# jfkirk/tensorrec

Hardware: AMD Instinct MI355X
Metric: user-item predictions/sec (higher is better)
Workload: dtype i8/bf16/fp32; 1 GPU; synthetic 1000000 users x 1000000 items, identity features, d=128, LinearRepresentation + DotProduct, biased, fused top-10 (BASELINE.json configs[2]); users=1000000, items=1000000, n_components=128, top_k=10, parallelism=items sharded x1, users replicated, topk_method=two_stage

## Files before the change

### include/tensorrec_hip.h

```cpp
#ifndef TENSORREC_HIP_H
#define TENSORREC_HIP_H
#include <stdint.h>

#ifdef __cplusplus
extern "C" {
#endif

#define TREC_OK 0
#define TREC_ERR_INVALID 1
#define TREC_ERR_LAUNCH 2
#define TREC_ERR_UNSUPPORTED 3

#define TREC_DTYPE_F32 0
#define TREC_DTYPE_BF16 1
#define TREC_MODE_DOT 0
#define TREC_MODE_EUCLIDEAN 1

int trec_abi_version(void);
const char* trec_last_error(void);
int trec_device_cu_count(void);
int trec_set_tuning(const char* name, int32_t value);
int trec_get_tuning(const char* name, int dflt);
int trec_clear_tuning(const char* name);

// ... 15 lines not shown
                        const void* packed_entries, int64_t n_rows, int64_t nnz, const float* W, int32_t d,
                        const float* own, int32_t accumulate, float* out, float* out_rowsum, void* workspace,
                        int64_t workspace_bytes, void* stream);
int trec_spmv_csr_split(const int64_t* indptr, const int32_t* indices, const float* values, const int32_t* val_perm,
                        int64_t n_rows, int64_t nnz, const float* beta, float* out, void* workspace,
                        int64_t workspace_bytes, void* stream);
int trec_csr_to_dense(const int64_t* indptr, const int32_t* indices, const float* values, int64_t n_rows,
                      int32_t n_cols, float* out, void* stream);
int trec_row_l2norm_fwd(const float* x, int64_t n_rows, int32_t d, float* y, float* inv_norm, void* stream);
int trec_row_l2norm_bwd(const float* y, const float* inv_norm, const float* dy, int64_t n_rows, int32_t d, float* dx,
                        void* stream);
int trec_relu_bwd(const float* out, const float* dout, int64_t n, float* dpre, void* stream);
int trec_colsum(const float* x, int64_t n_rows, int32_t d, float* out, float* workspace, int32_t n_slices, void* stream);
int trec_gemm_f32(int32_t trans_a, int32_t trans_b, int64_t M, int64_t N, int64_t K, const float* A, int64_t lda,
                  const float* B, int64_t ldb, float* C, int64_t ldc, int32_t accumulate, float* workspace,
                  int32_t splits, void* stream);
int trec_gemm_f32_split_bf16(int32_t trans_a, int32_t trans_b, int64_t M, int64_t N, int64_t K, const float* A, int64_t lda,
                             const float* B, int64_t ldb, float* C, int64_t ldc, int32_t accumulate, float* workspace,
                             int32_t splits, float* a_colsum_parts, void* stream);

int trec_score_kpad(int32_t d);
int trec_score_rows_per_workgroup(int32_t dtype, int32_t kpad);
int trec_score_tile_rows(int32_t dtype, int32_t kpad);
int trec_score_topk_capacity(int32_t k);
int trec_score_prep(const float* repr, int64_t n, int32_t d, int32_t kpad, int32_t normalize, int32_t dtype, void* out,
                    float* out_sqnorm, void* stream);
int trec_score_gemm_store(const void* users, const void* items, int32_t dtype, int32_t kpad, int64_t n_users,
                          int64_t n_items, const float* user_bias, const float* item_bias, int32_t mode,
                          const float* user_sqnorm, const float* item_sqnorm, float* out, int64_t ld_out,
                          int32_t variant, void* stream);
int trec_score_topk_parts(int32_t dtype, int32_t kpad, int64_t n_items, int32_t n_chunks);
int trec_score_gemm_topk(const void* users, const void* items, int32_t dtype, int32_t kpad, int64_t n_users,
                         int64_t n_items, int32_t item_index_base, const float* user_bias, const float* item_bias,
                         int32_t mode, const float* user_sqnorm, const float* item_sqnorm, int32_t n_chunks,
                         int32_t capacity, float* part_vals, int32_t* part_idx, int32_t variant, void* stream);
int trec_score_gemm_blockmax(const void* users, const void* items, int32_t dtype, int32_t kpad, int64_t n_users,
                             int64_t n_items, const float* user_bias, const float* item_bias, int32_t mode,
                             const float* user_sqnorm, const float* item_sqnorm, int32_t sb_rows, int32_t n_chunks,
                             float* blockmax, int64_t bm_stride, int32_t variant, void* stream);
int trec_topk_select_blocks(const float* blockmax, int32_t n_sb, int64_t n_users, int64_t stride, int32_t k, int32_t* sel,
                            float* sel_max, float* tau, void* stream);
int trec_topk_group_keys(const int32_t* sel, const float* sel_max, const float* floor, int64_t n, int32_t k, int32_t n_sb,
                         int32_t* keys, void* stream);
int trec_topk_pad_counts(const int64_t* indptr_t, int32_t n_sb, int32_t rows_wg, int32_t* cnt_pad, void* stream);
int trec_exclusive_scan_i32(const int32_t* counts, int64_t n, int64_t* workspace_i64, int64_t* out, void* stream);
int trec_topk_fill_groups(const int64_t* pstart, const int64_t* indptr_t, const int32_t* users_t, const int32_t* perm_t,
                          int32_t n_sb, int32_t rows_wg, int64_t max_rows, const void* users_op, int32_t row_bytes,
                          const float* user_bias, const float* user_sq, const float* user_tau, void* G, float* g_bias,
                          float* g_sq, float* g_tau, int32_t* row_pair, int32_t* rblock_chunk, void* stream);
int trec_score_gemm_topk_grouped(const void* users_g, const void* items, int32_t dtype, int32_t kpad, int64_t n_rows_g,
                                 int64_t n_items, int32_t item_index_base, const float* user_bias_g,
                                 const float* item_bias, int32_t mode, const float* user_sqnorm_g,
                                 const float* item_sqnorm, int32_t sb_rows, const int32_t* rblock_chunk,
                                 const int32_t* row_pair, const float* row_floor, int32_t capacity, float* part_vals,
                                 int32_t* part_idx, int32_t variant, const int32_t* row_index, void* stream);
int trec_topk_fill_groups_index(const int64_t* pstart, const int64_t* indptr_t, const int32_t* users_t,
                                const int32_t* perm_t, int32_t n_sb, int32_t rows_wg, int64_t max_rows, int32_t* row_user,
                                int32_t* row_pair, int32_t* rblock_chunk, void* stream);

int trec_topk_select_blocks_ex(const float* blockmax, int32_t n_sb, int64_t n_users, int64_t stride, int32_t k,
                               int32_t k_tau, int32_t* sel, float* sel_max, float* tau, void* stream);

int trec_score_prep_filter(const float* repr, int64_t n, int32_t d, int32_t kpad, int32_t normalize, const float* bias,
                           float* out_f32, void* out_bf16, float* row_stats, float* gstats, void* stream);
int trec_score_prep_i8(const float* repr, int64_t n, int32_t d, int32_t kpad, int32_t side, float clip_sigmas,
                       int32_t sb_rows, const float* bias, float* scales, double* workspace, void* out_q,
                       float* row_stats, int32_t* bias_q, float* sb_stats, float* gstats, void* stream);
int trec_score_row_scale_i8(const float* repr, int64_t n, int32_t d, float* nat, float* gmax, void* stream);
int trec_score_prep_i8_users(const float* repr, int64_t n, int32_t d, int32_t kpad, const float* wg_scale, int32_t wg_rows,
                             void* out_q, float* row_stats, void* stream);
int trec_score_bias_i8_classes(const float* bias, int64_t n, int32_t sb_rows, const float* ladder, const int32_t* class_used,
                               int32_t n_classes, float* sb_stats, int32_t* bias_q, float* gstats, void* stream);
int32_t trec_score_blockmax_i8_rows_per_workgroup(int32_t top_k);
int trec_score_user_err_i8(const float* user_stats, const float* user_bias, const float* gstats, int32_t kdim,
                           int64_t n_users, const float* scales, const float* wg_scale, int32_t wg_rows, float* r_err,
                           void* stream);
int trec_score_gemm_blockmax_i8(const void* users_q, const void* items_q, int32_t kpad, int64_t n_users, int64_t n_items,
                                const float* user_bias, const int32_t* item_bias_q, const float* scales,
                                const float* sb_stats, int32_t sb_rows, int32_t n_chunks, float* blockmax,
                                int64_t bm_stride, const float* user_err, float* chunk_top, int32_t top_k,
                                const float* wg_scale, const int32_t* wg_class, int32_t wg_rows, void* stream);
int64_t trec_user_prep_alloc_rows(int64_t n, int32_t wg_rows);
int64_t trec_user_prep_workspace_bytes(int64_t n);
int trec_user_prep_sorted(const float* repr, int64_t n, int32_t d, int32_t kpad, int32_t normalize, const float* user_bias,
                          int32_t wg_rows, int64_t n_alloc, void* workspace, int64_t workspace_bytes, int32_t* src,
                          int32_t* pos, float* wg_scale, int32_t* wg_class, float* ladder, int32_t* class_used, float* gmax,
                          int32_t* meta, float* out_f32, void* out_bf16, float* row_stats, void* out_q, float* row_stats8,
                          float* bias_sorted, void* stream);
int trec_fill_zero(void* p, int64_t nbytes, void* stream);
int trec_topk_rows_collect(const float* table, int32_t n_sb, int64_t n_users, int64_t stride, const float* thr,
                           const float* user_err, const float* sb_stats, int32_t kdim, int32_t rcap, int32_t* row_count,
                           int32_t* row_user, int64_t* status, void* stream);
int trec_score_gemm_blockmax_grouped(const void* users_bf16, const void* items_bf16, int32_t kpad, int64_t n_rows_g,
                                     int64_t n_items, const float* user_bias, const float* item_bias, int32_t sb_rows,
                                     const int32_t* rblock_chunk, const int32_t* row_user, float* blockmax,
                                     int64_t bm_stride, int32_t wgs_per_row, void* stream);
int trec_topk_rows_hot(int32_t* row_count, int32_t n_sb, int32_t rcap, int64_t n_users, int32_t* hot_list, int32_t hot_cap,
                       int64_t max_pairs, int64_t* status, void* stream);
int trec_score_gemm_blockmax_hot(const void* users_bf16, const void* items_bf16, int32_t kpad, int64_t n_users,
                                 int64_t n_items, const float* user_bias, const float* item_bias, int32_t sb_rows,
                                 const int32_t* hot_list, int32_t hot_cap, float* blockmax, int64_t bm_stride, void* stream);
int trec_topk_dense_users(const float* table, int32_t n_sb, int64_t n_users, int64_t stride, const float* thr,
                          const float* user_err, const float* sb_stats, int32_t kdim, int32_t limit, float* cand_floor,
                          int32_t* flag, int32_t* n_flagged, void* stream);
int trec_score_gemm_refine_candidates(const void* users_bf16, const void* items_bf16, int32_t kpad, int64_t n_rows_g,
                                      int64_t n_items, const float* user_bias, const float* item_bias, int32_t sb_rows,
                                      const int32_t* row_count, const int32_t* row_user, float* blockmax, int64_t bm_stride,
                                      int32_t wgs_per_row, const float* cand_floor, int32_t* cand_n, void* cand,
                                      int32_t cand_cap, int32_t item_index_base, const int32_t* wg_map, int32_t n_wgs,
                                      void* stream);
int trec_topk_rows_wg_map(const int32_t* row_count, int32_t n_sb, int32_t wgs_per_row, int32_t* wg_start, int32_t* wg_map,
                          int64_t map_cap, void* stream);
int trec_score_gemm_refine_candidates_hot(const void* users_bf16, const void* items_bf16, int32_t kpad, int64_t n_users,
                                          int64_t n_items, const float* user_bias, const float* item_bias, int32_t sb_rows,
                                          const int32_t* hot_list, int32_t hot_cap, float* blockmax, int64_t bm_stride,
                                          const float* cand_floor, int32_t* cand_n, void* cand, int32_t cand_cap,
                                          int32_t item_index_base, void* stream);
int trec_topk_candidates_finish(const int32_t* cand_n, const void* cand, int32_t cand_cap, const float* cand_floor,
                                const float* user_stats, const float* item_gstats, const float* users_f32,
                                const float* items_f32, int64_t ld_users, int64_t ld_items, int32_t kdim,
                                const float* user_bias, const float* item_bias, int32_t item_index_base, int64_t n_users,
                                int32_t k, float* out_vals, int32_t* out_idx, int32_t* flag, int32_t* n_flagged,
                                const int32_t* out_index, int32_t lanes_per_user, void* stream);
int trec_topk_candidates_finish_mixed(const int32_t* cand_n, const void* cand, int32_t cand_cap, const float* cand_floor,
                                      const float* user_stats, const float* item_gstats, const float* users_f32,
                                      const float* items_f32, int64_t ld_users, int64_t ld_items, int32_t kdim,
                                      const float* user_bias, const float* item_bias, int32_t item_index_base, int64_t n_users,
                                      int32_t k, float* out_vals, int32_t* out_idx, int32_t* flag, int32_t* n_flagged,
                                      const int32_t* out_index, int32_t cands_per_lane, int32_t* over_list, int32_t* over_count,
                                      void* stream);
int trec_topk_candidates_finish_wide(const int32_t* cand_n, const void* cand, int32_t cand_cap, const float* cand_floor,
                                     const float* users_f32, const float* items_f32, int64_t ld_users, int64_t ld_items,
                                     int32_t kdim, const float* user_bias, const float* item_bias, int32_t item_index_base,
                                     int64_t n_users, int32_t k, float* out_vals, int32_t* out_idx, int32_t* flag, int32_t* n_flagged,
                                     const int32_t* out_index, void* stream);
int trec_topk_cascade_floor(float* tau, const int32_t* src, const float* user_stats, const float* user_bias,
                            const float* item_gstats, int32_t kdim, int64_t n_users, float* floor0, int32_t* flag,
                            int32_t* n_flagged, int32_t* cand_n, void* stream);

int32_t trec_topk_prerefine_max_superblocks(void);
int trec_topk_prerefine_rows_pos(const int32_t* sel, const float* sel_val, int32_t k, int32_t top_k, int32_t sb_per_chunk,
                                 int32_t n_sb, int64_t n_users, const int32_t* src, int32_t rcap, int32_t* sel_sb,
                                 int32_t* row_count, int32_t* row_user, int32_t* ok, int32_t* sel_pos, void* stream);
int trec_topk_prerefine_tau_listed(const int32_t* sel_sb, const int32_t* sel_pos, const int32_t* ok, int32_t k, const float* pre_max,
                                   int32_t rcap, int64_t n_users, const int32_t* src, const float* user_stats,
                                   const float* user_bias, const float* item_gstats, int32_t kdim, float* tau, float* vals,
                                   float* cand_floor, void* stream);
int trec_score_gemm_refine_candidates_marked(const void* users_bf16, const void* items_bf16, int32_t kpad, int64_t n_rows_g,
                                             int64_t n_items, const float* user_bias, const float* item_bias, int32_t sb_rows,
                                             const int32_t* row_count, const int32_t* row_user, float* blockmax, int64_t bm_stride,
                                             int32_t wgs_per_row, const float* cand_floor, int32_t* cand_n, void* cand,
                                             int32_t cand_cap, int32_t item_index_base, const int32_t* wg_map, int32_t n_wgs,
                                             float* pre_max, void* stream);
int trec_topk_euclid_certify(const int32_t* cand_idx, const float* cand_g, const float* exact, int32_t kc, int32_t k,
                             const float* user_sq, const float* user_bias, const float* item_gstats, const float* bias_max,
                             int32_t kdim, int64_t n_users, float* out_vals, int32_t* out_idx, int32_t* flag,
                             int32_t* n_flagged, const float* lambda_, const float* bias_min, void* stream);
int trec_topk_filter_floor(const float* tau, const float* user_stats, const float* user_bias, const float* item_gstats,
                           int32_t kdim, int64_t n_users, float* floor, int32_t* flag, int32_t* n_flagged, void* stream);
int trec_topk_collect_blocks(const float* blockmax, int32_t n_sb, int64_t n_users, int64_t stride, const float* floor,
                             int32_t ksel, int32_t* keys, int32_t* count, int32_t* flag, int32_t* n_flagged, void* stream);
int trec_topk_filter_floor_ex(const float* tau, const float* user_stats, const float* user_bias, const float* item_gstats,
                              int32_t kdim, int64_t n_users, float mult, float* floor, int32_t* flag, int32_t* n_flagged,
                              void* stream);
int trec_topk_scan_blocks(const float* blockmax, int32_t n_sb, int64_t n_users, int64_t stride, int32_t k, const float* floor0,
                          int32_t cand_cap, float* sel_max, float* tau, int32_t* cand_s, float* cand_v, int32_t* cand_n,
                          void* stream);
int trec_topk_prune_candidates(const int32_t* cand_s, const float* cand_v, const int32_t* cand_n, int32_t cand_cap,
                               const float* floor, int32_t ksel, int64_t n_users, int32_t* keys, int32_t* count, int32_t* flag,
                               int32_t* n_flagged, int32_t* redo, void* stream);
int trec_topk_collect_blocks_masked(const float* blockmax, int32_t n_sb, int64_t n_users, int64_t stride, const float* floor,
                                    int32_t ksel, int32_t* keys, int32_t* count, int32_t* flag, int32_t* n_flagged,
                                    const int32_t* redo, void* stream);
int trec_topk_filter_finish(const int32_t* part_idx, int32_t capacity, int32_t ksel, const int32_t* count,
                            const float* users_f32, const float* items_f32, int64_t ld_users, int64_t ld_items,
                            int32_t kdim, const float* user_bias, const float* item_bias, int32_t item_index_base,
                            int64_t n_users, int32_t k, float* out_vals, int32_t* out_idx, int32_t* flag,
                            int32_t* n_flagged, void* stream);
int trec_topk_filter_finish_wide(const int32_t* part_idx, int32_t capacity, int32_t ksel, const int32_t* count,
                                 const float* users_f32, const float* items_f32, int64_t ld_users, int64_t ld_items,
                                 int32_t kdim, const float* user_bias, const float* item_bias, int32_t item_index_base,
                                 int64_t n_users, int32_t k, float* out_vals, int32_t* out_idx, int32_t* flag,
                                 int32_t* n_flagged, void* stream);

int trec_topk_merge(const float* part_vals, const int32_t* part_idx, int64_t n_users, int32_t n_cand, int32_t k,
                    float* out_vals, int32_t* out_idx, void* stream);

int trec_pair_score_fwd(const float* U, const float* V, const int32_t* xu, const int32_t* xi, int64_t n_pairs,
                        int32_t pairs_per_user, int32_t d, int32_t mode, const float* user_bias,
                        const float* item_bias, float* out, float* out_sqdist, void* stream);
int trec_pair_score_bwd(const float* U, const float* V, const int32_t* xu, const int32_t* xi, const float* grad,
                        int64_t n_pairs, int32_t pairs_per_user, int32_t d, int32_t mode, float* dU, float* dV,
                        float* d_user_bias, float* d_item_bias, void* stream);

int trec_pair_euclid_coef(const float* U, const float* V, const int32_t* xu, const int32_t* xi, const float* grad,
                          const float* sqdist, int64_t n_pairs, int32_t pairs_per_user, int32_t d, float* coef,
                          void* stream);

int trec_group_pairs_by_item(const int32_t* xu, const int32_t* xi, int64_t n_pairs, int32_t pairs_per_user,
                             int64_t n_items, int32_t* workspace_i32, int64_t* workspace_i64, int64_t* indptr_t,
                             int32_t* users_t, int32_t* perm_t, int32_t counts_given, const int32_t* ranks,
                             const float* values_in, float* values_out, void* stream);
int32_t trec_group_pairs_lds_runs(int64_t n_pairs, int64_t n_items);
int trec_group_pairs_by_item_lds(const int32_t* xu, const int32_t* xi, int64_t n_pairs, int32_t pairs_per_user, int64_t n_items,
                                 int32_t* workspace_i32, int64_t* workspace_i64, int32_t* run_counts, int64_t* indptr_t,
                                 int32_t* users_t, int32_t* perm_t, void* stream);
int64_t trec_group_pairs_staged_bytes(int64_t n_pairs, int32_t window_log2);
int trec_group_pairs_by_item_staged(const int32_t* xu, const int32_t* xi, int64_t n_pairs, int32_t pairs_per_user, int64_t n_items,
                                    int32_t* workspace_i32, int64_t* workspace_i64, int64_t* indptr_t, int32_t* entries,
                                    const int32_t* ranks, const float* values_in, void* staging, int64_t staging_bytes,
                                    int32_t window_log2, void* stream);

int64_t trec_group_pairs_binned_bytes(int64_t n_pairs, int64_t n_items);
int trec_group_pairs_by_item_binned(const int32_t* xu, const int32_t* xi, const float* values, int64_t n_pairs, int32_t pairs_per_user,
                                    int64_t n_items, int32_t drop_zero_values, void* workspace, int64_t workspace_bytes,
                                    int64_t* indptr_t, int32_t* entries, void* stream);

int trec_rank_rows(const float* scores, int64_t n_users, int64_t n_items, int64_t ld_scores, int32_t* ranks,
                   int64_t ld_ranks, void* stream);
int64_t trec_rank_rows_workspace_bytes(int64_t n_users, int64_t n_items);
int trec_rank_rows_chunked(const float* scores, int64_t n_users, int64_t n_items, int64_t ld_scores, int32_t* ranks,
                           int64_t ld_ranks, void* workspace, int64_t workspace_bytes, void* stream);
int trec_score_rankcount_max_targets(void);
int trec_pair_score_exact(const float* users_f32, const float* items_f32, int64_t ld, int32_t kdim, const int32_t* xu,
                          const int32_t* xi, int64_t n_pairs, const float* user_bias, const float* item_bias,
                          int32_t mode, const float* user_sqnorm, const float* item_sqnorm, int32_t item_index_base,
                          float* out, void* stream);
int trec_score_gemm_rankcount(const float* users_f32, const float* items_f32, int32_t kpad, int64_t n_rows,
                              int64_t n_items, int32_t item_index_base, const float* user_bias, const float* item_bias,
                              int32_t mode, const float* user_sqnorm, const float* item_sqnorm, const int32_t* row_user,
                              const int32_t* row_t0, const int32_t* row_tn, const int32_t* tgt_item,
                              const float* tgt_score, int32_t n_chunks, int32_t* counts, void* stream);
int trec_rank_of_pairs(const float* scores, int64_t ld_scores, int64_t col_offset, int64_t begin, int64_t end,
                       const int32_t* xu, const int32_t* xi, const float* target_scores, int64_t n_pairs,
                       int32_t add_one, int32_t* out, void* stream);
int trec_rank_of_pairs_by_user(const float* scores, int64_t ld_scores, int64_t col_offset, int64_t begin, int64_t end,
                               const int64_t* pair_indptr, const int32_t* xi, const float* target_scores,
                               int64_t n_users, int64_t n_pairs, int32_t add_one, int32_t* out, void* stream);

int trec_wmrb_fwd(const int64_t* indptr, const int32_t* pos_slot, const float* pos_weight, const float* pred_serial,
                  const float* sample_pred, int64_t n_users, int64_t n_items, int32_t n_sampled, float* loss,
                  float* smr, void* stream);
int trec_wmrb_bwd(const int64_t* indptr, const int32_t* pos_slot, const float* pos_weight, const float* pred_serial,
                  const float* sample_pred, const float* smr, const float* grad_loss, int64_t n_users,
                  int64_t n_items, int32_t n_sampled, float* d_pred_serial, float* d_sample_pred, void* stream);
int trec_sampled_softmax_fwd(const int64_t* indptr, const int32_t* pos_slot, const float* pred_serial,
                             const float* sample_pred, int64_t n_users, int32_t n_sampled, float inv_temperature,
                             float* loss, float* row_max, float* row_sum, void* stream);
int trec_sampled_softmax_bwd(const int64_t* indptr, const int32_t* pos_slot, const float* pred_serial,
                             const float* sample_pred, const float* row_max, const float* row_sum,
                             const float* grad_loss, int64_t n_users, int32_t n_sampled, float inv_temperature,
                             float* d_pred_serial, float* d_sample_pred, void* stream);
int trec_bpr_fwd(const int64_t* indptr, const int32_t* pos_slot, const float* pred_serial, const float* sample_pred,
                 int64_t n_users, int32_t n_sampled, float* loss, void* stream);
int trec_bpr_bwd(const int64_t* indptr, const int32_t* pos_slot, const float* pred_serial, const float* sample_pred,
                 const float* grad_loss, int64_t n_users, int32_t n_sampled, float* d_pred_serial,
                 float* d_sample_pred, void* stream);
int trec_sampled_softmax_adj_fwd(const int64_t* indptr, const int32_t* x_item, const int32_t* pos_slot,
                                 const float* pred_serial, const float* sample_pred, const int32_t* samples, const float* log_q,
                                 float log_q_uniform, int64_t n_users, int64_t n_items, int32_t n_sampled, float inv_temperature,
                                 int32_t log_q_correction, int32_t remove_hits, float* loss, float* row_ref, float* row_max,
                                 float* row_sum, void* stream);
int trec_sampled_softmax_adj_bwd(const int64_t* indptr, const int32_t* x_item, const int32_t* pos_slot,
                                 const float* pred_serial, const float* sample_pred, const int32_t* samples, const float* log_q,
                                 float log_q_uniform, const float* row_ref, const float* row_max, const float* row_sum,
                                 const float* grad_loss, int64_t n_users, int64_t n_items, int32_t n_sampled,
                                 float inv_temperature, int32_t log_q_correction, int32_t remove_hits, float* d_pred_serial,
                                 float* d_sample_pred, void* stream);
int trec_bpr_adj_fwd(const int64_t* indptr, const int32_t* x_item, const int32_t* pos_slot, const float* pred_serial,
                     const float* sample_pred, const int32_t* samples, int64_t n_users, int32_t n_sampled, int32_t remove_hits,
                     float* loss, void* stream);
int trec_bpr_adj_bwd(const int64_t* indptr, const int32_t* x_item, const int32_t* pos_slot, const float* pred_serial,
                     const float* sample_pred, const int32_t* samples, const float* grad_loss, int64_t n_users, int32_t n_sampled,
                     int32_t remove_hits, float* d_pred_serial, float* d_sample_pred, void* stream);
int trec_warp_fwd(const int64_t* indptr, const int32_t* x_item, const int32_t* pos_slot, const float* pred_serial,
                  const float* sample_pred, const int32_t* samples, int64_t n_users, int64_t n_items, int32_t n_sampled,
                  int32_t remove_hits, float* loss, int32_t* first, float* weight, void* stream);
int trec_warp_bwd(const int64_t* indptr, const int32_t* pos_slot, const int32_t* first, const float* weight,
                  const float* grad_loss, int64_t n_users, int32_t n_sampled, float* d_pred_serial, float* d_sample_pred,
                  void* stream);
int trec_wmrb_fused_lds_bytes(int32_t n_sampled, int32_t max_interactions_per_user, int32_t d);
int trec_wmrb_fused_step(const float* U, const float* V, const float* user_bias, const float* item_bias,
                         const int64_t* indptr, const int32_t* x_item, const int32_t* pos_slot, const float* pos_weight,
                         const int32_t* samples, int64_t n_users, int64_t n_items, int32_t n_sampled, int32_t d,
                         int32_t max_interactions_per_user, float* loss, float* pred_serial, float* dU,
                         float* d_user_bias, float* coef_samples, float* coef_pairs, int32_t* sample_hist,
                         int32_t* sample_rank, void* stream);
int trec_softmax_fused_lds_bytes(int32_t n_sampled, int32_t max_interactions_per_user, int32_t d);
int trec_softmax_fused_step(const float* U, const float* V, const float* user_bias, const float* item_bias,
                            const int64_t* indptr, const int32_t* x_item, const int32_t* pos_slot, const int32_t* samples,
                            int64_t n_users, int64_t n_items, int32_t n_sampled, int32_t d,
                            int32_t max_interactions_per_user, float inv_temperature, const float* log_q, float log_uniform,
                            int32_t log_q_correction, int32_t remove_hits, float* loss, float* pred_serial, float* dU,
                            float* d_user_bias, float* coef_samples, float* coef_pairs, int32_t* sample_hist,
                            int32_t* sample_rank, void* stream);
int trec_warp_fused_lds_bytes(int32_t n_sampled, int32_t max_interactions_per_user, int32_t d);
int trec_warp_fused_step(const float* U, const float* V, const float* user_bias, const float* item_bias,
                         const int64_t* indptr, const int32_t* x_item, const int32_t* pos_slot, const int32_t* samples,
                         int64_t n_users, int64_t n_items, int32_t n_sampled, int32_t d, int32_t max_interactions_per_user,
                         int32_t remove_hits, float* loss, float* pred_serial, float* dU, float* d_user_bias,
                         float* coef_samples, float* coef_pairs, int32_t* first, int32_t* sample_hist, int32_t* sample_rank,
                         void* stream);
int trec_softmax_shared_supported(int32_t n_sampled, int32_t d);
int trec_softmax_shared_slices(int64_t n_users, int32_t n_sampled, int32_t d);
int trec_softmax_shared_stats(const float* U, const float* Vs, const float* user_bias, const float* sample_bias,
                              const float* sample_c, int64_t n_users, int32_t n_sampled, int32_t d, float inv_temperature,
// ... 116 lines not shown
```

### tensorrec_amd/_native.py

```python
from __future__ import annotations

import ctypes
import os

import torch

_HERE = os.path.dirname(os.path.abspath(__file__))
LIB_PATH = os.environ.get("TREC_HIP_LIB") or os.path.join(_HERE, "libtensorrec_hip.so")

_vp, _i32, _i64, _u32, _u64, _f = (ctypes.c_void_p, ctypes.c_int32, ctypes.c_int64, ctypes.c_uint32,
                                   ctypes.c_uint64, ctypes.c_float)

_RETURNS_I64 = ("trec_csr_split_workspace_bytes", "trec_rank_rows_workspace_bytes", "trec_user_prep_alloc_rows",
                "trec_user_prep_workspace_bytes", "trec_group_pairs_staged_bytes", "trec_group_pairs_binned_bytes",
                "trec_fit_step_coop_workspace_floats")

SIGNATURES = {
    "trec_abi_version": [],
    "trec_device_cu_count": [],
    "trec_set_tuning": [ctypes.c_char_p, _i32],
    "trec_get_tuning": [ctypes.c_char_p, ctypes.c_int],
    "trec_clear_tuning": [ctypes.c_char_p],
    "trec_spmm_csr": [_vp, _vp, _vp, _vp, _i64, _i64, _vp, _i32, _vp, _i32, _i32, _vp, _vp, _vp],
    "trec_spmm_one_per_row": [_vp, _vp, _i64, _vp, _i32, _vp, _vp],
    "trec_spmm_csr_filter": [_vp, _vp, _vp, _i64, _i64, _vp, _i32, _vp, _vp, _vp, _vp, _vp],
    "trec_absmax": [_vp, _i64, _vp, _vp],
    "trec_spmm_csr_packed": [_vp, _vp, _i64, _vp, _i32, _i32, _i32, _vp, _vp, _vp],
    "trec_spmv_csr": [_vp, _vp, _vp, _vp, _i64, _vp, _vp, _vp],
    "trec_csr_split_workspace_bytes": [_i64, _i32],
    "trec_spmm_csr_split": [_vp, _vp, _vp, _vp, _vp, _i64, _i64, _vp, _i32, _vp, _i32, _vp, _vp, _vp, _i64, _vp],
    "trec_spmv_csr_split": [_vp, _vp, _vp, _vp, _i64, _i64, _vp, _vp, _vp, _i64, _vp],
    "trec_pair_euclid_coef": [_vp, _vp, _vp, _vp, _vp, _vp, _i64, _i32, _i32, _vp, _vp],
    "trec_csr_to_dense": [_vp, _vp, _vp, _i64, _i32, _vp, _vp],
    "trec_row_l2norm_fwd": [_vp, _i64, _i32, _vp, _vp, _vp],
    "trec_row_l2norm_bwd": [_vp, _vp, _vp, _i64, _i32, _vp, _vp],
    "trec_relu_bwd": [_vp, _vp, _i64, _vp, _vp],
    "trec_colsum": [_vp, _i64, _i32, _vp, _vp, _i32, _vp],
    "trec_gemm_f32": [_i32, _i32, _i64, _i64, _i64, _vp, _i64, _vp, _i64, _vp, _i64, _i32, _vp, _i32, _vp],
    "trec_gemm_f32_split_bf16": [_i32, _i32, _i64, _i64, _i64, _vp, _i64, _vp, _i64, _vp, _i64, _i32, _vp, _i32, _vp, _vp],
    "trec_score_kpad": [_i32],
    "trec_score_rows_per_workgroup": [_i32, _i32],
    "trec_score_tile_rows": [_i32, _i32],
    "trec_score_topk_capacity": [_i32],
    "trec_score_prep": [_vp, _i64, _i32, _i32, _i32, _i32, _vp, _vp, _vp],
    "trec_score_gemm_store": [_vp, _vp, _i32, _i32, _i64, _i64, _vp, _vp, _i32, _vp, _vp, _vp, _i64, _i32, _vp],
    "trec_score_topk_parts": [_i32, _i32, _i64, _i32],
    "trec_score_gemm_topk": [_vp, _vp, _i32, _i32, _i64, _i64, _i32, _vp, _vp, _i32, _vp, _vp, _i32, _i32, _vp, _vp,
                             _i32, _vp],
    "trec_score_gemm_blockmax": [_vp, _vp, _i32, _i32, _i64, _i64, _vp, _vp, _i32, _vp, _vp, _i32, _i32, _vp, _i64, _i32,
                                 _vp],
    "trec_topk_select_blocks": [_vp, _i32, _i64, _i64, _i32, _vp, _vp, _vp, _vp],
    "trec_topk_select_blocks_ex": [_vp, _i32, _i64, _i64, _i32, _i32, _vp, _vp, _vp, _vp],
    "trec_score_prep_filter": [_vp, _i64, _i32, _i32, _i32, _vp, _vp, _vp, _vp, _vp, _vp],
    "trec_score_prep_i8": [_vp, _i64, _i32, _i32, _i32, _f, _i32, _vp, _vp, _vp, _vp, _vp, _vp, _vp, _vp, _vp],
    "trec_score_row_scale_i8": [_vp, _i64, _i32, _vp, _vp, _vp],
    "trec_score_prep_i8_users": [_vp, _i64, _i32, _i32, _vp, _i32, _vp, _vp, _vp],
    "trec_score_bias_i8_classes": [_vp, _i64, _i32, _vp, _vp, _i32, _vp, _vp, _vp, _vp],
    "trec_score_blockmax_i8_rows_per_workgroup": [_i32],
    "trec_score_user_err_i8": [_vp, _vp, _vp, _i32, _i64, _vp, _vp, _i32, _vp, _vp],
    "trec_score_gemm_blockmax_i8": [_vp, _vp, _i32, _i64, _i64, _vp, _vp, _vp, _vp, _i32, _i32, _vp, _i64, _vp, _vp, _i32,
                                    _vp, _vp, _i32, _vp],
    "trec_user_prep_alloc_rows": [_i64, _i32],
    "trec_user_prep_workspace_bytes": [_i64],
    "trec_user_prep_sorted": [_vp, _i64, _i32, _i32, _i32, _vp, _i32, _i64, _vp, _i64, _vp, _vp, _vp, _vp, _vp, _vp, _vp, _vp,
                              _vp, _vp, _vp, _vp, _vp, _vp, _vp],
    "trec_fill_zero": [_vp, _i64, _vp],
    "trec_topk_cascade_floor": [_vp, _vp, _vp, _vp, _vp, _i32, _i64, _vp, _vp, _vp, _vp, _vp],
    "trec_topk_prerefine_max_superblocks": [],
    "trec_topk_prerefine_rows_pos": [_vp, _vp, _i32, _i32, _i32, _i32, _i64, _vp, _i32, _vp, _vp, _vp, _vp, _vp, _vp],
    "trec_topk_prerefine_tau_listed": [_vp, _vp, _vp, _i32, _vp, _i32, _i64, _vp, _vp, _vp, _vp, _i32, _vp, _vp, _vp, _vp],
    "trec_score_gemm_refine_candidates_marked": [_vp, _vp, _i32, _i64, _i64, _vp, _vp, _i32, _vp, _vp, _vp, _i64, _i32, _vp, _vp, _vp,
                                                 _i32, _i32, _vp, _i32, _vp, _vp],
    "trec_topk_rows_collect": [_vp, _i32, _i64, _i64, _vp, _vp, _vp, _i32, _i32, _vp, _vp, _vp, _vp],
    "trec_score_gemm_blockmax_grouped": [_vp, _vp, _i32, _i64, _i64, _vp, _vp, _i32, _vp, _vp, _vp, _i64, _i32, _vp],
    "trec_topk_rows_hot": [_vp, _i32, _i32, _i64, _vp, _i32, _i64, _vp, _vp],
    "trec_score_gemm_blockmax_hot": [_vp, _vp, _i32, _i64, _i64, _vp, _vp, _i32, _vp, _i32, _vp, _i64, _vp],
    "trec_topk_dense_users": [_vp, _i32, _i64, _i64, _vp, _vp, _vp, _i32, _i32, _vp, _vp, _vp, _vp],
    "trec_score_gemm_refine_candidates": [_vp, _vp, _i32, _i64, _i64, _vp, _vp, _i32, _vp, _vp, _vp, _i64, _i32, _vp, _vp, _vp,
                                          _i32, _i32, _vp, _i32, _vp],
    "trec_topk_rows_wg_map": [_vp, _i32, _i32, _vp, _vp, _i64, _vp],
    "trec_score_gemm_refine_candidates_hot": [_vp, _vp, _i32, _i64, _i64, _vp, _vp, _i32, _vp, _i32, _vp, _i64, _vp, _vp, _vp,
                                              _i32, _i32, _vp],
    "trec_topk_candidates_finish": [_vp, _vp, _i32, _vp, _vp, _vp, _vp, _vp, _i64, _i64, _i32, _vp, _vp, _i32, _i64, _i32, _vp,
                                    _vp, _vp, _vp, _vp, _i32, _vp],
    "trec_topk_candidates_finish_mixed": [_vp, _vp, _i32, _vp, _vp, _vp, _vp, _vp, _i64, _i64, _i32, _vp, _vp, _i32, _i64, _i32,
                                          _vp, _vp, _vp, _vp, _vp, _i32, _vp, _vp, _vp],
    "trec_topk_candidates_finish_wide": [_vp, _vp, _i32, _vp, _vp, _vp, _i64, _i64, _i32, _vp, _vp, _i32, _i64, _i32, _vp, _vp, _vp, _vp,
                                         _vp, _vp],
    "trec_topk_euclid_certify": [_vp, _vp, _vp, _i32, _i32, _vp, _vp, _vp, _vp, _i32, _i64, _vp, _vp, _vp, _vp, _vp, _vp, _vp],
    "trec_topk_filter_floor": [_vp, _vp, _vp, _vp, _i32, _i64, _vp, _vp, _vp, _vp],
    "trec_topk_collect_blocks": [_vp, _i32, _i64, _i64, _vp, _i32, _vp, _vp, _vp, _vp, _vp],
    "trec_topk_filter_floor_ex": [_vp, _vp, _vp, _vp, _i32, _i64, _f, _vp, _vp, _vp, _vp],
    "trec_topk_scan_blocks": [_vp, _i32, _i64, _i64, _i32, _vp, _i32, _vp, _vp, _vp, _vp, _vp, _vp],
    "trec_topk_prune_candidates": [_vp, _vp, _vp, _i32, _vp, _i32, _i64, _vp, _vp, _vp, _vp, _vp, _vp],
    "trec_topk_collect_blocks_masked": [_vp, _i32, _i64, _i64, _vp, _i32, _vp, _vp, _vp, _vp, _vp, _vp],
    "trec_topk_filter_finish": [_vp, _i32, _i32, _vp, _vp, _vp, _i64, _i64, _i32, _vp, _vp, _i32, _i64, _i32, _vp, _vp,
                                _vp, _vp, _vp],
    "trec_topk_filter_finish_wide": [_vp, _i32, _i32, _vp, _vp, _vp, _i64, _i64, _i32, _vp, _vp, _i32, _i64, _i32, _vp, _vp,
                                     _vp, _vp, _vp],
    "trec_topk_group_keys": [_vp, _vp, _vp, _i64, _i32, _i32, _vp, _vp],
    "trec_topk_pad_counts": [_vp, _i32, _i32, _vp, _vp],
    "trec_exclusive_scan_i32": [_vp, _i64, _vp, _vp, _vp],
    "trec_topk_fill_groups": [_vp, _vp, _vp, _vp, _i32, _i32, _i64, _vp, _i32, _vp, _vp, _vp, _vp, _vp, _vp, _vp, _vp, _vp,
                              _vp],
    "trec_score_gemm_topk_grouped": [_vp, _vp, _i32, _i32, _i64, _i64, _i32, _vp, _vp, _i32, _vp, _vp, _i32, _vp, _vp,
                                     _vp, _i32, _vp, _vp, _i32, _vp, _vp],
    "trec_topk_fill_groups_index": [_vp, _vp, _vp, _vp, _i32, _i32, _i64, _vp, _vp, _vp, _vp],
    "trec_topk_merge": [_vp, _vp, _i64, _i32, _i32, _vp, _vp, _vp],
    "trec_pair_score_fwd": [_vp, _vp, _vp, _vp, _i64, _i32, _i32, _i32, _vp, _vp, _vp, _vp, _vp],
    "trec_pair_score_bwd": [_vp, _vp, _vp, _vp, _vp, _i64, _i32, _i32, _i32, _vp, _vp, _vp, _vp, _vp],
    "trec_group_pairs_by_item": [_vp, _vp, _i64, _i32, _i64, _vp, _vp, _vp, _vp, _vp, _i32, _vp, _vp, _vp, _vp],
    "trec_group_pairs_lds_runs": [_i64, _i64],
    "trec_group_pairs_by_item_lds": [_vp, _vp, _i64, _i32, _i64, _vp, _vp, _vp, _vp, _vp, _vp, _vp],
    "trec_group_pairs_staged_bytes": [_i64, _i32],
    "trec_group_pairs_binned_bytes": [_i64, _i64],
    "trec_group_pairs_by_item_binned": [_vp, _vp, _vp, _i64, _i32, _i64, _i32, _vp, _i64, _vp, _vp, _vp],
    "trec_group_pairs_by_item_staged": [_vp, _vp, _i64, _i32, _i64, _vp, _vp, _vp, _vp, _vp, _vp, _vp, _i64, _i32, _vp],
    "trec_rank_rows": [_vp, _i64, _i64, _i64, _vp, _i64, _vp],
    "trec_rank_rows_workspace_bytes": [_i64, _i64],
    "trec_rank_rows_chunked": [_vp, _i64, _i64, _i64, _vp, _i64, _vp, _i64, _vp],
    "trec_score_rankcount_max_targets": [],
    "trec_pair_score_exact": [_vp, _vp, _i64, _i32, _vp, _vp, _i64, _vp, _vp, _i32, _vp, _vp, _i32, _vp, _vp],
    "trec_score_gemm_rankcount": [_vp, _vp, _i32, _i64, _i64, _i32, _vp, _vp, _i32, _vp, _vp, _vp, _vp, _vp, _vp, _vp,
                                  _i32, _vp, _vp],
    "trec_rank_of_pairs": [_vp, _i64, _i64, _i64, _i64, _vp, _vp, _vp, _i64, _i32, _vp, _vp],
    "trec_rank_of_pairs_by_user": [_vp, _i64, _i64, _i64, _i64, _vp, _vp, _vp, _i64, _i64, _i32, _vp, _vp],
    "trec_wmrb_fwd": [_vp, _vp, _vp, _vp, _vp, _i64, _i64, _i32, _vp, _vp, _vp],
    "trec_wmrb_bwd": [_vp, _vp, _vp, _vp, _vp, _vp, _vp, _i64, _i64, _i32, _vp, _vp, _vp],
    "trec_sampled_softmax_fwd": [_vp, _vp, _vp, _vp, _i64, _i32, _f, _vp, _vp, _vp, _vp],
    "trec_sampled_softmax_bwd": [_vp, _vp, _vp, _vp, _vp, _vp, _vp, _i64, _i32, _f, _vp, _vp, _vp],
    "trec_bpr_fwd": [_vp, _vp, _vp, _vp, _i64, _i32, _vp, _vp],
    "trec_bpr_bwd": [_vp, _vp, _vp, _vp, _vp, _i64, _i32, _vp, _vp, _vp],
    "trec_sampled_softmax_adj_fwd": [_vp, _vp, _vp, _vp, _vp, _vp, _vp, _f, _i64, _i64, _i32, _f, _i32, _i32, _vp, _vp, _vp, _vp, _vp],
    "trec_sampled_softmax_adj_bwd": [_vp, _vp, _vp, _vp, _vp, _vp, _vp, _f, _vp, _vp, _vp, _vp, _i64, _i64, _i32, _f, _i32, _i32,
                                     _vp, _vp, _vp],
    "trec_bpr_adj_fwd": [_vp, _vp, _vp, _vp, _vp, _vp, _i64, _i32, _i32, _vp, _vp],
    "trec_bpr_adj_bwd": [_vp, _vp, _vp, _vp, _vp, _vp, _vp, _i64, _i32, _i32, _vp, _vp, _vp],
    "trec_warp_fwd": [_vp, _vp, _vp, _vp, _vp, _vp, _i64, _i64, _i32, _i32, _vp, _vp, _vp, _vp],
    "trec_warp_bwd": [_vp, _vp, _vp, _vp, _vp, _i64, _i32, _vp, _vp, _vp],
    "trec_wmrb_fused_lds_bytes": [_i32, _i32, _i32],
    "trec_wmrb_fused_step": [_vp, _vp, _vp, _vp, _vp, _vp, _vp, _vp, _vp, _i64, _i64, _i32, _i32, _i32, _vp, _vp, _vp, _vp,
                             _vp, _vp, _vp, _vp, _vp],
    "trec_warp_fused_lds_bytes": [_i32, _i32, _i32],
    "trec_warp_fused_step": [_vp, _vp, _vp, _vp, _vp, _vp, _vp, _vp, _i64, _i64, _i32, _i32, _i32, _i32, _vp, _vp, _vp, _vp, _vp, _vp,
                             _vp, _vp, _vp, _vp],
    "trec_softmax_fused_lds_bytes": [_i32, _i32, _i32],
    "trec_softmax_fused_step": [_vp, _vp, _vp, _vp, _vp, _vp, _vp, _vp, _i64, _i64, _i32, _i32, _i32, _f, _vp, _f, _i32, _i32,
                                _vp, _vp, _vp, _vp, _vp, _vp, _vp, _vp, _vp],
    "trec_softmax_shared_supported": [_i32, _i32],
    "trec_softmax_shared_slices": [_i64, _i32, _i32],
    "trec_softmax_shared_stats": [_vp, _vp, _vp, _vp, _vp, _i64, _i32, _i32, _f, _vp, _vp, _vp],
    "trec_softmax_shared_positives": [_vp, _vp, _vp, _vp, _vp, _i64, _f, _vp, _vp, _vp, _vp, _vp],
    "trec_softmax_shared_grads": [_vp, _vp, _vp, _vp, _vp, _vp, _vp, _i64, _i32, _i32, _f, _i32, _vp, _vp, _vp, _vp, _vp],
    "trec_softmax_shared_scatter": [_vp, _vp, _vp, _vp, _i32, _i32, _i64, _vp, _vp, _vp],
    "trec_softmax_full_positives": [_vp, _vp, _vp, _vp, _vp, _i64, _f, _vp, _vp, _vp, _vp, _vp],
    "trec_wmrb_tiled_lds_bytes": [_i32, _i32, _i32],
    "trec_wmrb_tiled_step": [_vp, _vp, _vp, _vp, _vp, _vp, _vp, _vp, _vp, _i64, _i64, _i32, _i32, _i32, _i32, _vp, _vp, _vp,
                             _vp, _vp, _vp, _vp, _vp, _vp, _i64, _vp, _vp],
    "trec_softmax_tiled_lds_bytes": [_i32, _i32, _i32],
    "trec_softmax_tiled_step": [_vp, _vp, _vp, _vp, _vp, _vp, _vp, _vp, _i64, _i64, _i32, _i32, _i32, _i32, _f, _vp, _f, _i32, _i32,
                                _vp, _vp, _vp, _vp, _vp, _vp, _vp, _vp, _vp, _i64, _vp, _vp],
    "trec_fit_step_coop_workspace_floats": [_i64, _i64, _i32, _i32, _i32],
    "trec_fit_step_coop": [_vp] * 12 + [_vp] * 6 + [_vp] * 5 + [_i64, _i64, _i64, _i32, _i32, _i32, _i64, _u64, _u32, _f, _f, _f, _f, _f,
                                                            _vp, _i64, _vp, _vp, _vp],
    "trec_item_weighted_hist": [_vp, _vp, _i64, _vp, _vp, _i64, _i32, _vp, _vp],
    "trec_dense_loss_fwd": [_i32, _vp, _i64, _i64, _vp, _vp, _vp, _i64, _vp, _vp, _vp],
    "trec_dense_loss_fwd_phase": [_i32, _i32, _vp, _i64, _i64, _vp, _vp, _vp, _i64, _i64, _vp, _vp, _vp],
    "trec_dense_loss_bwd": [_i32, _vp, _i64, _i64, _vp, _vp, _vp, _i64, _vp, _vp, _vp, _vp],
    "trec_softmax_dense_fwd": [_vp, _i64, _vp, _vp, _vp, _i64, _i64, _f, _vp, _vp, _vp, _vp],
    "trec_softmax_dense_bwd": [_vp, _i64, _vp, _vp, _vp, _vp, _vp, _vp, _i64, _i64, _f, _vp, _vp],
    "trec_gram_f64": [_vp, _i64, _i32, _i64, _vp, _vp],
    "trec_dense_loss_factored_phase": [_i32, _i32, _vp, _vp, _vp, _i64, _i64, _i64, _vp, _vp, _vp],
    "trec_dense_loss_factored_bwd": [_i32, _vp, _vp, _i64, _vp, _vp, _vp, _vp, _vp],
    "trec_rmse_fwd": [_vp, _vp, _i64, _vp, _i32, _vp, _vp],
    "trec_rmse_bwd": [_vp, _vp, _vp, _vp, _i64, _vp, _vp],
    "trec_sample_items": [_i64, _i64, _i32, _i32, _i32, _u64, _u32, _vp, _vp],
    "trec_sample_items_alias": [_i64, _i64, _i32, _i32, _vp, _vp, _u64, _u32, _vp, _vp],
    "trec_hard_negatives_supported": [_i32, _i32, _i32],
    "trec_select_hard_negatives": [_vp, _vp, _vp, _vp, _vp, _vp, _vp, _i64, _i64, _i32, _i32, _i32, _i32, _i32, _vp, _vp, _vp],
    "trec_crc32c": [_vp, _u64, _u32],
    "trec_collapse_tastes_fwd": [_vp, _vp, _i32, _i64, _i32, _vp, _vp, _vp, _vp, _i64, _vp, _vp],
    "trec_collapse_tastes_bwd": [_vp, _vp, _vp, _i32, _i64, _vp, _vp, _vp],
    "trec_adam_tf_step": [_vp, _vp, _vp, _vp, _i64, _f, _f, _f, _f, _f, _vp],
    "trec_adam_schedule_advance": [_vp, _f, _f, _f, _i32, _vp],
    "trec_adam_tf_step_dev": [_vp, _vp, _vp, _vp, _i64, _vp, _f, _f, _f, _f, _vp],
    "trec_sample_items_dev": [_i64, _i64, _i32, _i32, _i32, _u64, _vp, _vp, _vp],
    "trec_exclude_filter_topk": [_vp, _vp, _i32, _i64, _i32, _vp, _vp, _vp, _vp, _vp, _vp, _vp, _vp],
    "trec_topk_rows_excluded": [_vp, _i64, _i64, _i64, _i32, _vp, _vp, _vp, _vp, _vp, _vp],
    "trec_exclude_rank_adjust": [_vp, _vp, _vp, _vp, _vp, _vp, _i64, _vp, _vp],
    "trec_topk_drop_self": [_vp, _vp, _i32, _i64, _vp, _vp, _vp, _vp],
    "trec_candset_scores": [_vp, _vp, _i64, _i32, _vp, _vp, _vp, _i64, _i64, _i64, _vp, _vp, _i32, _vp, _vp, _vp, _vp],
    "trec_candset_topk": [_vp, _vp, _vp, _vp, _i64, _i32, _vp, _i64, _vp, _vp, _vp],
    "trec_candset_rank_count": [_vp, _vp, _vp, _vp, _vp, _vp, _i64, _vp, _vp],
}

_lib = None


class NativeLibraryError(RuntimeError):
    pass


def load():
    global _lib
    if _lib is not None:
        return _lib
    if not os.path.exists(LIB_PATH):
        raise NativeLibraryError(
            "%s not found: build it with `python -c 'import __graft_entry__ as g; g.build()'` or "
            "`make -C tensorrec_amd/csrc`.  tensorrec_amd has no CPU fallback." % LIB_PATH)
    try:
        lib = ctypes.CDLL(LIB_PATH)
    except OSError as exc:
        raise NativeLibraryError("cannot load %s: %s" % (LIB_PATH, exc))
    for name, argtypes in SIGNATURES.items():
        try:
            fn = getattr(lib, name)
        except AttributeError:
            raise NativeLibraryError("%s does not export %s (stale build?)" % (LIB_PATH, name))
        fn.argtypes = argtypes
        fn.restype = ctypes.c_int64 if name in _RETURNS_I64 else ctypes.c_int
    lib.trec_last_error.argtypes = []
    lib.trec_last_error.restype = ctypes.c_char_p
    _lib = lib
    return lib
# ... 44 lines not shown
```

### tensorrec_amd/csrc/score_blockmax.hip

```cpp
#include "score_common.hpp"
#include <math.h>
#include <type_traits>

namespace {

constexpr int BN = 64;

__device__ __forceinline__ int swz16(int row, int ch) {
    return ch >= 16 ? (row & 15) : ((row >> 1) & 7);
}

template <int KT, bool BIAS>
__global__ __launch_bounds__(256, 2) void blockmax_pipe_kernel(ScoreParams p)
{
    constexpr int NCB = 4;
    constexpr int NBUF = 2;
    constexpr int RB = KT * 2;
    constexpr int CH = RB / 16;
    constexpr int KS = KT / 16;
    constexpr int TILE_BYTES = BN * RB;
    constexpr int NSLOT = BN * CH / 256;
    constexpr int NSTEP = 2 * KS;
    static_assert(KT == 64 || KT == 128, "pipelined BLOCKMAX covers K = 64 / 128");

// ... 366 lines not shown
    float bm[NUB];
#pragma unroll
    for (int ub = 0; ub < NUB; ++ub) bm[ub] = -INFINITY;

    int tile_now = 0;
    int64_t sb_first = t_begin;
    auto queue_entry = [&](int i, int n) __attribute__((always_inline)) {
        const bool in = i < n;
        const int32_t code = in ? qc[i] : 0;
        const f32x4 a = in ? qv[i] : (f32x4){0.f, 0.f, 0.f, 0.f};
        const int ul = code >> 16;
        const int32_t uid = in ? q_id[ul] : -1;
        const float fl = q_fl[ul], bu = q_bu[ul];
        const int64_t item0 = sb_first + (int64_t)(code & 0xffff) * 4;
        float v[4];
        int32_t slot[4];
#pragma unroll
        for (int e = 0; e < 4; ++e) {
            v[e] = BIAS ? a[e] + bu : a[e];
            slot[e] = 0x7fffffff;
            if (uid >= 0 && v[e] >= fl && item0 + e < p.n_t) slot[e] = atomicAdd(p.cand_n + uid, 1);
        }
#pragma unroll
        for (int e = 0; e < 4; ++e) {
#ifdef TREC_CAND_DIAG
            if ((p.cand_diag & 3) == 2) continue;
#endif
            if (slot[e] < p.cand_cap)
                p.cand[(int64_t)uid * p.cand_cap + slot[e]] = make_int2((int32_t)(item0 + e) + p.t_index_base, __float_as_int(v[e]));
        }
    };
    auto queue_flush = [&](auto unrc) __attribute__((always_inline)) {
        constexpr int UNR = decltype(unrc)::value;
#ifdef TREC_CAND_DIAG
        const int n = (p.cand_diag & 3) == 1 ? 0 : qn;
#else
        const int n = qn;
#endif
#pragma unroll 1
        for (int i0 = 0; i0 < n; i0 += 64 * UNR) {
#pragma unroll
            for (int j = 0; j < UNR; ++j) queue_entry(i0 + j * 64 + lane, n);
        }
        qn = 0;
    };

    auto tile_body = [&](auto bufc) __attribute__((always_inline)) {
        constexpr int buf = decltype(bufc)::value;
        const char* tb = smem + buf * TILE_BYTES;
        const float* sd = side + buf * BN + 4 * g;
        bf16x8 tf[3];
        f32x4 c0 = {0.f, 0.f, 0.f, 0.f};
        if (BIAS) c0 = *(const f32x4*)sd;
        tf[0] = *(const bf16x8*)(tb + koff[0]);
        tf[1] = *(const bf16x8*)(tb + koff[1 % KS]);
        __builtin_amdgcn_sched_barrier(0);
#pragma unroll
        for (int s = 0; s < NSTEP; ++s) {
            const int blk = s / KS, ks = s % KS;
            if (s + 2 < NSTEP)
                tf[(s + 2) % 3] = *(const bf16x8*)(tb + ((s + 2) / KS) * 16 * RB + koff[(s + 2) % KS]);
            if (ks == 0) {
#pragma unroll
                for (int ub = 0; ub < NUB; ++ub)
                    acc[ub] = __builtin_amdgcn_mfma_f32_16x16x32_bf16(tf[s % 3], rfb[ub][0], c0, 0, 0, 0);
                if (BIAS && blk + 1 < NBLK) c0 = *(const f32x4*)(sd + 16 * (blk + 1));
            } else {
#pragma unroll
                for (int ub = 0; ub < NUB; ++ub)
                    acc[ub] = __builtin_amdgcn_mfma_f32_16x16x32_bf16(tf[s % 3], rfb[ub][ks], acc[ub], 0, 0, 0);
            }
            if (ks == KS - 1 && !LIST) {
#pragma unroll
                for (int ub = 0; ub < NUB; ++ub) {
                    bm[ub] = fmaxf(fmaxf(bm[ub], acc[ub][0]), acc[ub][1]);
                    bm[ub] = fmaxf(fmaxf(bm[ub], acc[ub][2]), acc[ub][3]);
                }
            }
            if (ks == KS - 1 && LIST) {
#pragma unroll
                for (int ub = 0; ub < NUB; ++ub) {
                    if ((ub % (NUB / 2)) == 0 && __builtin_expect(qn > LQ_FLUSH, 0)) queue_flush(std::integral_constant<int, 1>{});
                    const float m4 = fmaxf(fmaxf(fmaxf(acc[ub][0], acc[ub][1]), acc[ub][2]), acc[ub][3]);
                    bm[ub] = fmaxf(bm[ub], m4);
                    const bool hit = m4 >= thr_a[ub];
                    const unsigned long long hm = __builtin_amdgcn_ballot_w64(hit);
                    if (hm != 0ull) {
                        const int pos = qn + (int)__builtin_amdgcn_mbcnt_hi((unsigned int)(hm >> 32),
                                                                            __builtin_amdgcn_mbcnt_lo((unsigned int)hm, 0u));
                        if (hit) {
                            int lo = lane;
                            asm volatile("" : "+v"(lo));
                            qv[pos] = acc[ub];
                            qc[pos] = (((ub * 16) + (lo & 15)) << 16) | (((tile_now + blk) << 2) + (lo >> 4));
                        }
                        qn += __builtin_popcountll(hm);
                    }
                }
            }
            __builtin_amdgcn_sched_barrier(0);
        }
    };

    if (!GRP) stage_issue(0, 0);
    asm volatile("s_waitcnt vmcnt(0)" ::: "memory");
    __syncthreads();
#ifdef TREC_CAND_DIAG
    dg_t1 = wall_clock64();
#endif

    for (int t = 0; t < n_tiles; ++t) {
        const int buf = t & 1;
        if (t + 1 < n_tiles) stage_issue(t + 1, buf ^ 1);
        if (LIST) tile_now = (t % p.sb_tiles) * NBLK;
        if (buf == 0) tile_body(std::integral_constant<int, 0>{});
        else tile_body(std::integral_constant<int, 1>{});

        if (((t + 1) % p.sb_tiles) == 0 || t + 1 == n_tiles) {
#ifdef TREC_CAND_DIAG
            const unsigned long long dg_b = wall_clock64();
#endif
            if (LIST) { queue_flush(std::integral_constant<int, 3>{}); sb_first = t_begin + (int64_t)(t + 1) * BN; }
            const int64_t sb = GRP ? (int64_t)chunk : t_begin / ((int64_t)p.sb_tiles * BN) + t / p.sb_tiles;
            float m[NUB];
#pragma unroll
            for (int ub = 0; ub < NUB; ++ub) {
                float x = bm[ub];
                x = fmaxf(x, __shfl_xor(x, 16, 64));
                m[ub] = fmaxf(x, __shfl_xor(x, 32, 64));
                bm[ub] = -INFINITY;
            }
            if (LIST) {
                if (g == 0) {
#pragma unroll
                    for (int ub = 0; ub < NUB; ++ub) q_ta[ub * 16 + lu] = m[ub];
                }
                __builtin_amdgcn_fence(__ATOMIC_RELEASE, "wavefront");
                __builtin_amdgcn_wave_barrier();
                __builtin_amdgcn_fence(__ATOMIC_ACQUIRE, "wavefront");
#pragma unroll
                for (int o = 0; o < OW; ++o) {
                    const int slot = (OW * g + o) * 16 + lu;
                    float v = q_ta[slot];
                    const int32_t ou = q_id[slot];
                    if (BIAS) v = v + q_bu[slot];
#ifdef TREC_CAND_DIAG
                    if (p.cand_diag & 8) continue;
#endif
                    if (GRP && p.pre_max) {
                        if (ou >= 0) {
                            const int64_t rb = ((int64_t)__builtin_amdgcn_readfirstlane(rblock) * 4 + wave) * (NUB * 16);
                            p.pre_max[rb + slot] = v;
                            p.blockmax[sb * p.bm_stride + ou] = -INFINITY;
                        }
                    } else if (ou >= 0) p.blockmax[sb * p.bm_stride + ou] = v;
                }
                __builtin_amdgcn_fence(__ATOMIC_RELEASE, "wavefront");
                __builtin_amdgcn_wave_barrier();
            } else {
#pragma unroll
                for (int o = 0; o < OW; ++o) {
                    float v = g == 0 ? m[o] : (g == 1 ? m[OW + o] : (g == 2 ? m[2 * OW + o] : m[3 * OW + o]));
                    if (BIAS) v = v + own_bias[o];
                    if (own_u[o] >= 0) p.blockmax[sb * p.bm_stride + own_u[o]] = v;
                }
            }
#ifdef TREC_CAND_DIAG
            dg_flush += wall_clock64() - dg_b;
#endif
        }
        if (t + 1 < n_tiles) asm volatile("s_waitcnt vmcnt(0)" ::: "memory");
        __syncthreads();
    }
#ifdef TREC_CAND_DIAG
    if (GRP && LIST && tid == 0 && blockIdx.x < REFINE_DIAG_WGS) {
        const unsigned long long dg_e = wall_clock64();
        unsigned long long* row = g_refine_clk + (size_t)blockIdx.x * 4;
        row[0] = dg_t1 - dg_t0;
        row[1] = dg_e - dg_t1 - dg_flush;
        row[2] = dg_flush;
        row[3] = dg_e - dg_t0;
    }
#endif
}

template <int KT, bool BIAS, bool GRP, bool LIST = false>
int launch_bf16x16(ScoreParams p, hipStream_t st)
{
    constexpr int LDS = 2 * BN * KT * 2 + 2 * BN * 4 + (LIST ? 4 * LQ_CAP * 20 + 4 * 4 * NUB * 16 * 4 : 0);
    constexpr int RW = 4 * NUB * 16;
    auto kern = blockmax_bf16x16_kernel<KT, BIAS, GRP, LIST>;
    static bool attr_set = false;
    if (!attr_set && LDS > 32 * 1024) {
        (void)hipFuncSetAttribute((const void*)kern, hipFuncAttributeMaxDynamicSharedMemorySize, LDS);
        attr_set = true;
    }
    if (GRP && p.capacity > 0) p.capacity = p.capacity * 512 / RW;
    p.n_rblocks = GRP ? (int)(p.n_r / RW) : (int)ceil_div64(p.n_r, RW);
    const unsigned blocks = GRP ? (p.wg_map ? (unsigned)p.n_wgs : (unsigned)p.n_rblocks) : (unsigned)p.n_rblocks * (unsigned)p.n_chunks;
    if (blocks == 0) return TREC_OK;
    hipLaunchKernelGGL(kern, dim3(blocks), dim3(256), LDS, st, p);
    return trec_check_launch(GRP ? "trec_score_gemm_blockmax_grouped (16x16x32)" : "trec_score_gemm_blockmax (16x16x32)");
}

template <int KT, bool BIAS>
__global__ __launch_bounds__(256, 2) void blockmax_pipe_f32_kernel(ScoreParams p)
{
    constexpr int NCB = 2;
    constexpr int RB = KT * 4;
    constexpr int CH = RB / 16;
    constexpr int KS = KT / 2;
    constexpr int G = 8;
    constexpr int TILE_BYTES = BN * RB;
    constexpr int NSLOT = BN * CH / 256;
    static_assert(KT == 64 || KT == 128, "pipelined fp32 BLOCKMAX covers K = 64 / 128");

    extern __shared__ __attribute__((aligned(16))) char smem[];
    float* side = (float*)(smem + 2 * TILE_BYTES);

    const int tid = threadIdx.x;
    const int lane = tid & 63;
    const int wave = __builtin_amdgcn_readfirstlane(tid >> 6);
    const int half = lane >> 5, l31 = lane & 31;
    const int rblock = blockIdx.x % p.n_rblocks;
    const int chunk = blockIdx.x / p.n_rblocks;
    const int64_t r_base = ((int64_t)rblock * 4 + wave) * (NCB * 32);
    const int64_t t_begin = (int64_t)chunk * p.chunk_len;
    const int64_t t_end = (t_begin + p.chunk_len < p.n_t) ? t_begin + p.chunk_len : p.n_t;
    const int n_tiles = (int)((t_end - t_begin + BN - 1) / BN);

    float rff[NCB][KS];
    float r_bias[NCB];
#pragma unroll
    for (int cb = 0; cb < NCB; ++cb) {
        int64_t row = r_base + cb * 32 + l31;
        if (row >= p.n_r) row = p.n_r - 1;
        const float* src = (const float*)p.R + row * (int64_t)KT;
#pragma unroll
        for (int ks = 0; ks < KS; ++ks) rff[cb][ks] = src[2 * ks + half];
        r_bias[cb] = (BIAS && p.r_bias) ? p.r_bias[row] : 0.f;
    }

    int slot_off[NSLOT];
#pragma unroll
    for (int i = 0; i < NSLOT; ++i) {
        const int q = i * 256 + tid;
        const int row = q / CH, pc = q % CH;
        slot_off[i] = row * RB + ((pc ^ (row & 15)) * 16);
    }
    const char* t_chunk = (const char*)p.T + t_begin * (int64_t)RB;
    float side_b = 0.f;
    auto stage_issue = [&](int tile, int buf) {
        const int64_t row0 = t_begin + (int64_t)tile * BN;
        const bool clamp = row0 + BN > p.n_t;
        if (BIAS && tid < BN) {
            int64_t g = row0 + tid;
            if (g >= p.n_t) g = p.n_t - 1;
            side_b = p.t_bias ? p.t_bias[g] : 0.f;
        }
        const char* tile_base = t_chunk + (int64_t)tile * (BN * RB);
#pragma unroll
        for (int i = 0; i < NSLOT; ++i) {
            int off = slot_off[i];
            if (clamp) {
                const int last = (int)(p.n_t - 1 - row0);
                const int row = (i * 256 + tid) / CH;
                if (row > last) off -= (row - last) * RB;
            }
            char* dst = smem + buf * TILE_BYTES + (i * 256 + wave * 64) * 16;
            __builtin_amdgcn_global_load_lds((const __attribute__((address_space(1))) void*)(tile_base + off),
                                             (__attribute__((address_space(3))) void*)dst, 16, 0, 0);
        }
    };
    auto stage_commit = [&](int buf) {
        if (BIAS && tid < BN) side[buf * BN + tid] = side_b;
        asm volatile("s_waitcnt vmcnt(0)" ::: "memory");
    };

    const int sw = l31 & 15;
    const int row_off = l31 * RB + half * 4;
    auto tf_addr = [&](int ks) { return row_off + (((ks >> 1) ^ sw) * 16) + (ks & 1) * 8; };

    float bm[NCB];
#pragma unroll
    for (int cb = 0; cb < NCB; ++cb) bm[cb] = -INFINITY;

    stage_issue(0, 0);
    stage_commit(0);
    __syncthreads();

    for (int t = 0; t < n_tiles; ++t) {
        const int buf = t & 1;
        if (t + 1 < n_tiles) stage_issue(t + 1, buf ^ 1);
        const char* tb = smem + buf * TILE_BYTES;
        const float* sd = side + buf * BN + 4 * half;
#pragma unroll 1
        for (int rb = 0; rb < BN / 32; ++rb) {
            const char* blk = tb + rb * 32 * RB;
            f32x16 acc[NCB];
#pragma unroll
            for (int cb = 0; cb < NCB; ++cb)
#pragma unroll
                for (int r = 0; r < 16; ++r) acc[cb][r] = 0.f;
            float cur[G], nxt[G];
#pragma unroll
            for (int g = 0; g < G; ++g) cur[g] = *(const float*)(blk + tf_addr(g));
// ... 135 lines not shown
```

### tensorrec_amd/csrc/score_blockmax_i8.hip

```cpp
#include "score_common.hpp"
#include <math.h>
#include <limits.h>
#include <type_traits>

namespace {

typedef int v4i32 __attribute__((ext_vector_type(4)));

constexpr int BNQ = 128;
constexpr int NWQ = 4;

template <int KT, bool BIAS, int TK, int NUB>
__global__ __launch_bounds__(NWQ * 64, 8 / NWQ) void blockmax_i8x16_kernel(ScoreParams p)
{
    constexpr int NT = NWQ * 64;
    constexpr int OW = NUB / 4;
    static_assert(NUB % 4 == 0, "user blocks per wave must split over the four row-groups");
    constexpr int RB = KT;
    constexpr int CH = RB / 16;
    constexpr int KS = KT / 64;
    constexpr int TILE_BYTES = BNQ * RB;
    constexpr int NSLOT = BNQ * CH / NT;
    constexpr int NBLK = BNQ / 16;
    constexpr int NSTEP = NBLK * KS;
    static_assert(KT == 64 || KT == 128, "int8 16x16x64 BLOCKMAX covers K = 64 / 128");

    extern __shared__ __attribute__((aligned(16))) char smem[];
    int* side = (int*)(smem + 2 * TILE_BYTES);

    const int tid = threadIdx.x;
    const int lane = tid & 63;
    const int wave = __builtin_amdgcn_readfirstlane(tid >> 6);
    const int g = lane >> 4, lu = lane & 15;
    const int rblock = blockIdx.x % p.n_rblocks;
    const int chunk = blockIdx.x / p.n_rblocks;
    if (p.wg_scale && p.wg_scale[rblock] == 0.f) return;
    const int64_t r_base = ((int64_t)rblock * NWQ + wave) * (NUB * 16);
    const int64_t t_begin = (int64_t)chunk * p.chunk_len;
    const int64_t t_end = (t_begin + p.chunk_len < p.n_t) ? t_begin + p.chunk_len : p.n_t;
    const int n_tiles = (int)((t_end - t_begin + BNQ - 1) / BNQ);
    auto swz = [](int row) { return CH == 8 ? (row & 7) : ((row >> 1) & 3); };

    v4i32 rfq[NUB][KS];
#pragma unroll
    for (int ub = 0; ub < NUB; ++ub) {
        int64_t row = r_base + ub * 16 + lu;
        if (row >= p.n_r) row = p.n_r - 1;
        const char* src = (const char*)p.R + row * (int64_t)RB;
#pragma unroll
        for (int ks = 0; ks < KS; ++ks) rfq[ub][ks] = *(const v4i32*)(src + (ks * 4 + g) * 16);
    }
    int64_t own_u[OW];
    float own_bias[OW], e_nx[OW], e_ex[OW], e_cu[OW];
    float top[TK ? OW : 1][TK ? TK : 1];
#pragma unroll
    for (int o = 0; o < OW; ++o) {
        own_u[o] = r_base + (OW * g + o) * 16 + lu;
        const int64_t row = own_u[o] < p.n_r ? own_u[o] : p.n_r - 1;
        own_bias[o] = (BIAS && p.r_bias) ? p.r_bias[row] : 0.f;
        if (TK) {
            e_nx[o] = p.r_err[row * 4]; e_ex[o] = p.r_err[row * 4 + 1]; e_cu[o] = p.r_err[row * 4 + 2];
#pragma unroll
            for (int j = 0; j < TK; ++j) top[o][j] = -INFINITY;
        }
    }

    int slot_off[NSLOT];
#pragma unroll
    for (int i = 0; i < NSLOT; ++i) {
        const int q = i * NT + tid;
        const int row = q / CH, pc = q % CH;
        slot_off[i] = row * RB + ((pc ^ swz(row)) * 16);
    }
    const char* t_chunk = (const char*)p.T + t_begin * (int64_t)RB;
    const int* t_bias_q = p.t_bias ? (const int*)p.t_bias + (p.wg_class ? (int64_t)p.wg_class[rblock] * p.bias_stride : 0) : nullptr;
    auto stage_issue = [&](int tile, int buf) {
        const int64_t row0 = t_begin + (int64_t)tile * BNQ;
        const bool clamp = row0 + BNQ > p.n_t;
        if (BIAS && wave < BNQ / 64) {
            int64_t gi = row0 + wave * 64 + lane;
            if (gi >= p.n_t) gi = p.n_t - 1;
            if (t_bias_q) {
                __builtin_amdgcn_global_load_lds((const __attribute__((address_space(1))) void*)(t_bias_q + gi),
                                                 (__attribute__((address_space(3))) void*)(side + buf * BNQ + wave * 64), 4, 0, 0);
            } else {
                side[buf * BNQ + wave * 64 + lane] = 0;
            }
        }
        const char* tile_base = t_chunk + (int64_t)tile * (BNQ * RB);
#pragma unroll
        for (int i = 0; i < NSLOT; ++i) {
            int off = slot_off[i];
            if (clamp) {
                const int last = (int)(p.n_t - 1 - row0);
                const int row = (i * NT + tid) / CH;
                if (row > last) off -= (row - last) * RB;
            }
            char* dst = smem + buf * TILE_BYTES + (i * NT + wave * 64) * 16;
            __builtin_amdgcn_global_load_lds((const __attribute__((address_space(1))) void*)(tile_base + off),
                                             (__attribute__((address_space(3))) void*)dst, 16, 0, 0);
        }
    };

    int koff[KS];
#pragma unroll
    for (int ks = 0; ks < KS; ++ks) koff[ks] = lu * RB + (((ks * 4 + g) ^ swz(lu)) * 16);

    v4i32 acc[NUB];
    int bm[NUB];
#pragma unroll
    for (int ub = 0; ub < NUB; ++ub) bm[ub] = INT_MIN;

    auto tile_body = [&](auto bufc) __attribute__((always_inline)) {
        constexpr int buf = decltype(bufc)::value;
        const char* tb = smem + buf * TILE_BYTES;
        const int* sd = side + buf * BNQ + 4 * g;
        v4i32 tf[3];
        v4i32 c0 = {0, 0, 0, 0};
        if (BIAS) c0 = *(const v4i32*)sd;
        tf[0] = *(const v4i32*)(tb + koff[0]);
        tf[1] = *(const v4i32*)(tb + (KS > 1 ? koff[1 % KS] : 16 * RB + koff[0]));
        __builtin_amdgcn_sched_barrier(0);
#pragma unroll
        for (int s = 0; s < NSTEP; ++s) {
            const int blk = s / KS, ks = s % KS;
            if (ks == 0) {
#pragma unroll
                for (int ub = 0; ub < NUB; ++ub)
                    acc[ub] = __builtin_amdgcn_mfma_i32_16x16x64_i8(tf[s % 3], rfq[ub][0], c0, 0, 0, 0);
                __builtin_amdgcn_sched_barrier(0);
                if (BIAS && blk + 1 < NBLK) c0 = *(const v4i32*)(sd + 16 * (blk + 1));
            } else {
#pragma unroll
                for (int ub = 0; ub < NUB; ++ub)
                    acc[ub] = __builtin_amdgcn_mfma_i32_16x16x64_i8(tf[s % 3], rfq[ub][ks], acc[ub], 0, 0, 0);
                __builtin_amdgcn_sched_barrier(0);
            }
            if (s + 2 < NSTEP) tf[(s + 2) % 3] = *(const v4i32*)(tb + ((s + 2) / KS) * 16 * RB + koff[(s + 2) % KS]);
            if (ks == KS - 1) {
#pragma unroll
                for (int ub = 0; ub < NUB; ++ub) {
                    bm[ub] = max(max(bm[ub], acc[ub][0]), acc[ub][1]);
                    bm[ub] = max(max(bm[ub], acc[ub][2]), acc[ub][3]);
                }
            }
            __builtin_amdgcn_sched_barrier(0);
        }
    };

    stage_issue(0, 0);
    asm volatile("s_waitcnt vmcnt(0)" ::: "memory");
    __syncthreads();

    const float a_user = p.wg_scale ? p.wg_scale[rblock] : p.scales[0];
    const int64_t sb0 = t_begin / ((int64_t)p.sb_tiles * BNQ);
    f32x4 ss_cur = *(const f32x4*)(p.sb_stats + sb0 * 4), ss_next = ss_cur;
    for (int t = 0; t < n_tiles; ++t) {
        const int buf = t & 1;
        if (t + 1 < n_tiles) stage_issue(t + 1, buf ^ 1);
        if ((t % p.sb_tiles) == 0 && t + p.sb_tiles < n_tiles)
            ss_next = *(const f32x4*)(p.sb_stats + (sb0 + t / p.sb_tiles + 1) * 4);
        if (buf == 0) tile_body(std::integral_constant<int, 0>{});
        else tile_body(std::integral_constant<int, 1>{});

        if (((t + 1) % p.sb_tiles) == 0 || t + 1 == n_tiles) {
            const int64_t sb = sb0 + t / p.sb_tiles;
            const float scale = a_user * ss_cur[0];
            const float yh = TK ? ss_cur[1] : 0.f, dy = TK ? ss_cur[2] : 0.f, db = TK ? a_user * ss_cur[3] : 0.f;
            ss_cur = ss_next;
            int m[NUB];
#pragma unroll
            for (int ub = 0; ub < NUB; ++ub) {
                int x = bm[ub];
                const int o1 = __shfl_xor(x, 16, 64);
                x = x > o1 ? x : o1;
                const int o2 = __shfl_xor(x, 32, 64);
                m[ub] = x > o2 ? x : o2;
                bm[ub] = INT_MIN;
            }
#pragma unroll
            for (int o = 0; o < OW; ++o) {
                const int mo = g == 0 ? m[o] : (g == 1 ? m[OW + o] : (g == 2 ? m[2 * OW + o] : m[3 * OW + o]));
                float v = (float)mo * scale;
                if (BIAS) v = v + own_bias[o];
                if (own_u[o] < p.n_r) p.blockmax[sb * p.bm_stride + own_u[o]] = v;
                if (TK) {
                    float lb = v - i8_pair_err(e_nx[o], e_ex[o], e_cu[o], yh, dy, db, KT);
                    lb = (lb == lb) ? lb : -INFINITY;
                    if (p.top_tag) lb = lb_tag(lb, t / p.sb_tiles);
#pragma unroll
                    for (int j = TK - 1; j >= 1; --j) top[o][j] = __builtin_amdgcn_fmed3f(top[o][j], top[o][j - 1], lb);
                    top[o][0] = fmaxf(top[o][0], lb);
                }
            }
        }
        if (t + 1 < n_tiles) asm volatile("s_waitcnt vmcnt(0)" ::: "memory");
        __syncthreads();
    }
    if (TK) {
#pragma unroll
        for (int o = 0; o < OW; ++o)
            if (own_u[o] < p.n_r) {
#pragma unroll
                for (int j = 0; j < TK; ++j) p.chunk_top[((int64_t)chunk * TK + j) * p.bm_stride + own_u[o]] = top[o][j];
            }
    }
}

template <int KT, bool BIAS, int TK, int NUB>
int launch_i8x16(ScoreParams p, int sb_rows, hipStream_t st)
{
    constexpr int LDS = 2 * BNQ * KT + 2 * BNQ * 4;
    auto kern = blockmax_i8x16_kernel<KT, BIAS, TK, NUB>;
    static bool attr_set = false;
    if (!attr_set && LDS > 32 * 1024) {
        (void)hipFuncSetAttribute((const void*)kern, hipFuncAttributeMaxDynamicSharedMemorySize, LDS);
        attr_set = true;
    }
    p.n_rblocks = (int)ceil_div64(p.n_r, NWQ * NUB * 16);
    p.sb_tiles = sb_rows / BNQ;
    const unsigned blocks = (unsigned)p.n_rblocks * (unsigned)p.n_chunks;
    hipLaunchKernelGGL(kern, dim3(blocks), dim3(NWQ * 64), LDS, st, p);
    return trec_check_launch("trec_score_gemm_blockmax_i8 (16x16x64)");
}

template <int KT, bool BIAS>
int launch_i8x16_lists(const ScoreParams& p, int sb_rows, hipStream_t st)
{
    if (p.top_k == 0) return launch_i8x16<KT, BIAS, 0, 12>(p, sb_rows, st);
    if (p.top_k == 10) return launch_i8x16<KT, BIAS, 10, 12>(p, sb_rows, st);
    return launch_i8x16<KT, BIAS, 16, 8>(p, sb_rows, st);
}

template <int G>
__global__ __launch_bounds__(256) void prep_i8_kernel(const float* __restrict__ x, int64_t n, int d, int kt,
                                                     const float* __restrict__ scale_ptr, int sb_rows,
                                                     float* __restrict__ sb_stats, signed char* __restrict__ out_q,
                                                     float2* __restrict__ row_stats, int wg_rows)
{
    const int64_t row = ((int64_t)blockIdx.x * blockDim.x + threadIdx.x) / G;
    const bool ok = row < n;
    const int sub = threadIdx.x % G;
    const int64_t sb = sb_rows ? (ok ? row : n - 1) / sb_rows : 0;
    const float scale = sb_rows ? sb_stats[sb * 4] : (wg_rows > 0 ? scale_ptr[(ok ? row : n - 1) / wg_rows] : *scale_ptr);
    const float inv = 1.0f / scale;
    const float* xr = x + (ok ? row : 0) * (int64_t)d;
    float sw = 0.f, se = 0.f;
#pragma unroll
    for (int it = 0; it < 2; ++it) {
        const int c = (it * G + sub) * 4;
        f32x4 v = {0.f, 0.f, 0.f, 0.f};
        if (ok && c < d) {
            if ((d & 3) == 0) v = *(const f32x4*)(xr + c);
            else {
#pragma unroll
                for (int e = 0; e < 4; ++e) if (c + e < d) v[e] = xr[c + e];
            }
        }
        unsigned int pk = 0;
#pragma unroll
        for (int e = 0; e < 4; ++e) {
            float q = rintf(v[e] * inv);
            if (!(q == q)) q = 0.f;
            q = fminf(fmaxf(q, -127.f), 127.f);
            const float err = v[e] - q * scale;
            sw = fmaf(v[e], v[e], sw);
            se = fmaf(err, err, se);
            pk |= ((unsigned int)(int)q & 0xffu) << (8 * e);
        }
        if (ok && c < kt) *(unsigned int*)(out_q + row * (int64_t)kt + c) = pk;
    }
    for (int off = G / 2; off > 0; off >>= 1) { sw += __shfl_xor(sw, off, 64); se += __shfl_xor(se, off, 64); }
    float nw = sqrtf(sw), ne = sqrtf(se);
    if (sub == 0 && ok) row_stats[row] = make_float2(nw, ne);
}

__global__ __launch_bounds__(256) void sb_reduce_kernel(const float2* __restrict__ row_stats, int64_t n, int sb_rows,
                                                       float* __restrict__ sb_stats)
{
    const int64_t s = blockIdx.x;
    const int64_t r0 = s * sb_rows, r1 = (r0 + sb_rows < n) ? r0 + sb_rows : n;
    float g0 = 0.f, g1 = 0.f;
    for (int64_t r = r0 + threadIdx.x; r < r1; r += 256) {
        const float2 st = row_stats[r];
        float a = st.x + st.y, b = st.y;
        if (a != a) a = INFINITY;
        if (b != b) b = INFINITY;
        g0 = fmaxf(g0, a); g1 = fmaxf(g1, b);
    }
    for (int off = 32; off > 0; off >>= 1) { g0 = fmaxf(g0, __shfl_xor(g0, off, 64)); g1 = fmaxf(g1, __shfl_xor(g1, off, 64)); }
    __shared__ float w0[4], w1[4];
    if ((threadIdx.x & 63) == 0) { w0[threadIdx.x >> 6] = g0; w1[threadIdx.x >> 6] = g1; }
    __syncthreads();
    if (threadIdx.x == 0) {
        sb_stats[s * 4 + 1] = fmaxf(fmaxf(w0[0], w0[1]), fmaxf(w0[2], w0[3]));
        sb_stats[s * 4 + 2] = fmaxf(fmaxf(w1[0], w1[1]), fmaxf(w1[2], w1[3]));
    }
}

__global__ __launch_bounds__(1024) void sb_scale_kernel(const float* __restrict__ x, int64_t n, int d, int sb_rows,
                                                       float* __restrict__ sb_stats)
{
    const int64_t s = blockIdx.x;
    const int64_t r0 = s * sb_rows;
    const int64_t r1 = (r0 + sb_rows < n) ? r0 + sb_rows : n;
    const int64_t n_elem = (r1 - r0) * d;
    const float* xs = x + r0 * (int64_t)d;
    float am = 0.f;
    if ((d & 3) == 0) {
        for (int64_t i = (int64_t)threadIdx.x * 4; i < n_elem; i += 4096) {
            const f32x4 v = *(const f32x4*)(xs + i);
#pragma unroll
            for (int e = 0; e < 4; ++e) { const float a = fabsf(v[e]); am = (a > am || a != a) ? a : am; }
        }
    } else {
        for (int64_t i = threadIdx.x; i < n_elem; i += 1024) { const float a = fabsf(xs[i]); am = (a > am || a != a) ? a : am; }
    }
    if (am != am) am = INFINITY;
    for (int off = 32; off > 0; off >>= 1) am = fmaxf(am, __shfl_xor(am, off, 64));
    __shared__ float wmax[16];
    if ((threadIdx.x & 63) == 0) wmax[threadIdx.x >> 6] = am;
    __syncthreads();
    if (threadIdx.x == 0) {
        am = 0.f;
        for (int w = 0; w < 16; ++w) am = fmaxf(am, wmax[w]);
        float sc = am / 127.0f;
        if (!(sc > 0.f) || !(sc < INFINITY)) sc = 1.0f;
        sb_stats[s * 4] = sc;
    }
}

__global__ __launch_bounds__(256) void bias_i8_kernel(const float* __restrict__ bias, int64_t n, const float* __restrict__ ladder,
                                                     const int32_t* __restrict__ class_used, int sb_rows,
                                                     float* __restrict__ sb_stats, int* __restrict__ bias_q,
                                                     float* __restrict__ gstats)
{
    const int64_t s = blockIdx.x;
    const int c = blockIdx.y;
    if (class_used && class_used[c] == 0) return;
    const int64_t r0 = s * sb_rows, r1 = (r0 + sb_rows < n) ? r0 + sb_rows : n;
// ... 90 lines not shown
    if (u >= n_users) return;
    const float2 st = ustats[u];
    const float bu = user_bias ? fabsf(user_bias[u]) : 0.f;
    const float ck = (float)(kdim + 6) * 2.98023224e-07f;
    *(f32x4*)(r_err + u * 4) = (f32x4){st.x, st.y, ck * (bu + gstats[2]), wg_scale ? wg_scale[u / wg_rows] : scales[0]};
}

__global__ __launch_bounds__(256) void sumsq_absmax_kernel(const float* __restrict__ x, int64_t n_elem, double* __restrict__ ws)
{
    double acc = 0.0;
    float am = 0.f;
    for (int64_t i = ((int64_t)blockIdx.x * 256 + threadIdx.x) * 4; i + 3 < n_elem; i += (int64_t)gridDim.x * 1024) {
        const f32x4 v = *(const f32x4*)(x + i);
        acc += (double)v[0] * v[0] + (double)v[1] * v[1] + (double)v[2] * v[2] + (double)v[3] * v[3];
#pragma unroll
        for (int e = 0; e < 4; ++e) { const float a = fabsf(v[e]); am = (a > am || a != a) ? a : am; }
    }
    if (blockIdx.x == 0 && threadIdx.x == 0)
        for (int64_t i = n_elem & ~(int64_t)3; i < n_elem; ++i) {
            acc += (double)x[i] * x[i];
            const float a = fabsf(x[i]);
            am = (a > am || a != a) ? a : am;
        }
    if (am != am) am = INFINITY;
    for (int off = 32; off > 0; off >>= 1) { acc += __shfl_xor(acc, off, 64); am = fmaxf(am, __shfl_xor(am, off, 64)); }
    if ((threadIdx.x & 63) == 0) {
        atomicAdd(ws, acc);
        atomicMax((unsigned int*)(ws + 1), __float_as_uint(am));
    }
}

__global__ void scale_from_stats_kernel(const double* __restrict__ ws, double n_elem, float clip_sigmas, float* __restrict__ scales)
{
    const double rms = sqrt(ws[0] / n_elem);
    const float am = __uint_as_float(*(const unsigned int*)(ws + 1));
    float top = am;
    if (clip_sigmas > 0.f && (float)(clip_sigmas * rms) < top) top = (float)(clip_sigmas * rms);
    float s = top / 127.0f;
    if (!(s > 0.f) || !(s < INFINITY)) s = 1.0f;
    scales[0] = s;
}

}

extern "C" int trec_score_prep_i8(const float* repr, int64_t n, int32_t d, int32_t kpad, int32_t side, float clip_sigmas,
                                  int32_t sb_rows, const float* bias, float* scales, double* workspace, void* out_q,
                                  float* row_stats, int32_t* bias_q, float* sb_stats, float* gstats, void* stream)
{
    TREC_REQUIRE(scales && (side == 0 || side == 1 || side == 2), "trec_score_prep_i8: side must be 0 (users), 1 (items) or 2 (item biases)");
    TREC_REQUIRE(!bias || (bias_q && gstats && side >= 1), "trec_score_prep_i8: a bias needs bias_q, gstats and side 1 / 2");
    TREC_REQUIRE(side == 0 || (sb_stats && sb_rows >= 1), "trec_score_prep_i8: the item side needs sb_stats and sb_rows");
    if (n == 0) return TREC_OK;
    hipStream_t st = (hipStream_t)stream;
    if (side != 2) {
        TREC_REQUIRE(repr && out_q && row_stats, "trec_score_prep_i8: null pointer");
        TREC_REQUIRE(d >= 1 && kpad >= d && kpad % 4 == 0 && (kpad <= 64 || kpad == 128),
                     "trec_score_prep_i8: need d <= kpad, kpad % 4 == 0, kpad <= 64 or kpad == 128");
        TREC_REQUIRE(((uintptr_t)repr % 16) == 0, "trec_score_prep_i8: repr must be 16-byte aligned");
        if (side == 0) {
            TREC_REQUIRE(workspace, "trec_score_prep_i8: the user side needs the 16-byte workspace");
            if (hipMemsetAsync(workspace, 0, 2 * sizeof(double), st) != hipSuccess) {
                trec_set_last_error("trec_score_prep_i8: memset failed");
                return TREC_ERR_LAUNCH;
            }
            const int64_t n_elem = n * (int64_t)d;
            unsigned sb = (unsigned)ceil_div64(n_elem, 1024 * 8);
            if (sb > 4096) sb = 4096;
            if (sb < 1) sb = 1;
            hipLaunchKernelGGL(sumsq_absmax_kernel, dim3(sb), dim3(256), 0, st, repr, n_elem, workspace);
            hipLaunchKernelGGL(scale_from_stats_kernel, dim3(1), dim3(1), 0, st, workspace, (double)n_elem, clip_sigmas, scales);
        } else {
            hipLaunchKernelGGL(sb_scale_kernel, dim3((unsigned)ceil_div64(n, sb_rows)), dim3(1024), 0, st, repr, n, d, sb_rows, sb_stats);
        }
        const int g = kpad == 128 ? 32 : (kpad == 64 ? 16 : 8);
        const unsigned blocks = (unsigned)ceil_div64(n * g, 256);
#define TREC_PQ(GV) hipLaunchKernelGGL(prep_i8_kernel<GV>, dim3(blocks), dim3(256), 0, st, repr, n, d, kpad, scales, side == 1 ? sb_rows : 0, sb_stats, (signed char*)out_q, (float2*)row_stats, 0)
        if (g == 32) TREC_PQ(32);
        else if (g == 16) TREC_PQ(16);
        else TREC_PQ(8);
#undef TREC_PQ
        if (side == 1)
            hipLaunchKernelGGL(sb_reduce_kernel, dim3((unsigned)ceil_div64(n, sb_rows)), dim3(256), 0, st, (const float2*)row_stats, n, sb_rows, sb_stats);
    }
    if (side >= 1 && bias)
        hipLaunchKernelGGL(bias_i8_kernel, dim3((unsigned)ceil_div64(n, sb_rows), 1), dim3(256), 0, st, bias, n, scales, (const int32_t*)nullptr, sb_rows, sb_stats, bias_q, gstats);
    return trec_check_launch("trec_score_prep_i8");
}


extern "C" int trec_score_row_scale_i8(const float* repr, int64_t n, int32_t d, float* nat, float* gmax, void* stream)
{
    TREC_REQUIRE(repr && nat && gmax, "trec_score_row_scale_i8: null pointer");
    TREC_REQUIRE(d >= 1 && d <= 256 && ((uintptr_t)repr % 16) == 0, "trec_score_row_scale_i8: need d <= 256 and 16-byte aligned rows");
    if (n == 0) return TREC_OK;
    const int kp = (d + 3) / 4 * 4;
    const int g = kp > 64 ? 32 : (kp > 32 ? 16 : 8);
    const unsigned blocks = (unsigned)ceil_div64(n * g, 256);
    hipStream_t st = (hipStream_t)stream;
    if (g == 32) hipLaunchKernelGGL(row_natscale_kernel<32>, dim3(blocks), dim3(256), 0, st, repr, n, d, nat, gmax);
    else if (g == 16) hipLaunchKernelGGL(row_natscale_kernel<16>, dim3(blocks), dim3(256), 0, st, repr, n, d, nat, gmax);
    else hipLaunchKernelGGL(row_natscale_kernel<8>, dim3(blocks), dim3(256), 0, st, repr, n, d, nat, gmax);
    return trec_check_launch("trec_score_row_scale_i8");
}

extern "C" int trec_score_prep_i8_users(const float* repr, int64_t n, int32_t d, int32_t kpad, const float* wg_scale,
                                        int32_t wg_rows, void* out_q, float* row_stats, void* stream)
{
    TREC_REQUIRE(repr && wg_scale && out_q && row_stats && wg_rows >= 1, "trec_score_prep_i8_users: bad arguments");
    TREC_REQUIRE(d >= 1 && kpad >= d && kpad % 4 == 0 && (kpad <= 64 || kpad == 128),
                 "trec_score_prep_i8_users: need d <= kpad, kpad % 4 == 0, kpad <= 64 or kpad == 128");
    TREC_REQUIRE(((uintptr_t)repr % 16) == 0, "trec_score_prep_i8_users: repr must be 16-byte aligned");
    if (n == 0) return TREC_OK;
    hipStream_t st = (hipStream_t)stream;
    const int g = kpad == 128 ? 32 : (kpad == 64 ? 16 : 8);
    const unsigned blocks = (unsigned)ceil_div64(n * g, 256);
#define TREC_PQU(GV) hipLaunchKernelGGL(prep_i8_kernel<GV>, dim3(blocks), dim3(256), 0, st, repr, n, d, kpad, wg_scale, 0, (float*)nullptr, (signed char*)out_q, (float2*)row_stats, wg_rows)
    if (g == 32) TREC_PQU(32);
    else if (g == 16) TREC_PQU(16);
    else TREC_PQU(8);
#undef TREC_PQU
    return trec_check_launch("trec_score_prep_i8_users");
}

extern "C" int trec_score_bias_i8_classes(const float* bias, int64_t n, int32_t sb_rows, const float* ladder,
                                          const int32_t* class_used, int32_t n_classes, float* sb_stats, int32_t* bias_q,
                                          float* gstats, void* stream)
{
    TREC_REQUIRE(bias && ladder && sb_stats && bias_q && gstats, "trec_score_bias_i8_classes: null pointer");
    TREC_REQUIRE(sb_rows >= 1 && n_classes >= 1 && n_classes <= 65535, "trec_score_bias_i8_classes: bad sizes");
    if (n == 0) return TREC_OK;
    hipLaunchKernelGGL(bias_i8_kernel, dim3((unsigned)ceil_div64(n, sb_rows), (unsigned)n_classes), dim3(256), 0, (hipStream_t)stream,
                       bias, n, ladder, class_used, sb_rows, sb_stats, bias_q, gstats);
    return trec_check_launch("trec_score_bias_i8_classes");
}

extern "C" int32_t trec_score_blockmax_i8_rows_per_workgroup(int32_t top_k)
{
    return top_k <= 10 ? NWQ * 12 * 16 : NWQ * 8 * 16;
}

extern "C" int trec_score_user_err_i8(const float* user_stats, const float* user_bias, const float* gstats, int32_t kdim,
                                      int64_t n_users, const float* scales, const float* wg_scale, int32_t wg_rows,
                                      float* r_err, void* stream)
{
    TREC_REQUIRE(user_stats && gstats && r_err && kdim >= 1, "trec_score_user_err_i8: bad arguments");
    TREC_REQUIRE((wg_scale && wg_rows >= 1) || scales, "trec_score_user_err_i8: need wg_scale + wg_rows or scales");
    TREC_REQUIRE(((uintptr_t)r_err % 16) == 0, "trec_score_user_err_i8: r_err must be 16-byte aligned");
    if (n_users == 0) return TREC_OK;
    hipLaunchKernelGGL(user_err_i8_kernel, dim3((unsigned)ceil_div64(n_users, 256)), dim3(256), 0, (hipStream_t)stream,
                       (const float2*)user_stats, user_bias, gstats, kdim, n_users, scales, wg_scale, wg_rows, r_err);
    return trec_check_launch("trec_score_user_err_i8");
}

extern "C" int trec_score_gemm_blockmax_i8(const void* users_q, const void* items_q, int32_t kpad, int64_t n_users,
                                           int64_t n_items, const float* user_bias, const int32_t* item_bias_q,
                                           const float* scales, const float* sb_stats, int32_t sb_rows, int32_t n_chunks,
                                           float* blockmax, int64_t bm_stride, const float* user_err, float* chunk_top,
                                           int32_t top_k, const float* wg_scale, const int32_t* wg_class, int32_t wg_rows,
                                           void* stream)
{
    const int top_tag = (top_k & 0x100) ? 1 : 0;
    top_k &= 0xff;
    TREC_REQUIRE(!wg_scale || wg_rows == trec_score_blockmax_i8_rows_per_workgroup(top_k),
                 "trec_score_gemm_blockmax_i8: the user operand was laid out for another workgroup height (prepared for the other top_k?)");
    TREC_REQUIRE(users_q && items_q && (scales || wg_scale) && sb_stats && blockmax && bm_stride >= n_users, "trec_score_gemm_blockmax_i8: bad arguments");
    TREC_REQUIRE(!wg_class || wg_scale, "trec_score_gemm_blockmax_i8: wg_class comes with wg_scale");
    TREC_REQUIRE(kpad == 64 || kpad == 128, "trec_score_gemm_blockmax_i8: kpad must be 64 or 128");
    TREC_REQUIRE(sb_rows >= BNQ && sb_rows % BNQ == 0, "trec_score_gemm_blockmax_i8: sb_rows must be a multiple of 128");
    TREC_REQUIRE(n_users >= 1 && n_items >= 1 && n_chunks >= 1, "trec_score_gemm_blockmax_i8: empty operand");
    TREC_REQUIRE(n_items < (int64_t)1 << 31 && n_users < (int64_t)1 << 31, "trec_score_gemm_blockmax_i8: sizes must fit int32");
    TREC_REQUIRE((chunk_top != nullptr) == (user_err != nullptr) && (chunk_top ? (top_k == 10 || top_k == 16) : top_k == 0),
                 "trec_score_gemm_blockmax_i8: user_err, chunk_top and top_k (10 or 16) come together");
    ScoreParams p = {};
    p.R = users_q; p.T = items_q; p.n_r = n_users; p.n_t = n_items;
    p.chunk_len = ceil_div64(ceil_div64(n_items, n_chunks), sb_rows) * sb_rows;
    p.n_chunks = (int)ceil_div64(n_items, p.chunk_len);
    p.r_bias = user_bias; p.t_bias = (const float*)item_bias_q;
    p.blockmax = blockmax; p.bm_stride = bm_stride;
    p.scales = scales; p.sb_stats = sb_stats; p.r_err = user_err; p.chunk_top = chunk_top; p.top_k = top_k;
    p.top_tag = top_tag;
    TREC_REQUIRE(!top_tag || (top_k && p.chunk_len / sb_rows <= (1 << TREC_LB_TAG_BITS)),
                 "trec_score_gemm_blockmax_i8: tagged lower bounds need the lists and chunks of at most 4096 superblocks");
    p.wg_scale = wg_scale; p.wg_class = item_bias_q ? wg_class : nullptr; p.bias_stride = n_items;
    hipStream_t st = (hipStream_t)stream;
    const bool bias = user_bias || item_bias_q;
    if (kpad == 128) return bias ? launch_i8x16_lists<128, true>(p, sb_rows, st) : launch_i8x16_lists<128, false>(p, sb_rows, st);
    return bias ? launch_i8x16_lists<64, true>(p, sb_rows, st) : launch_i8x16_lists<64, false>(p, sb_rows, st);
}
```

### tensorrec_amd/csrc/score_common.hpp

```cpp
#pragma once
#include "common.hpp"

struct ScoreParams {
    const void* R;
    const void* T;
    int64_t n_r, n_t;
    int64_t chunk_len;
    int n_chunks;
    int n_rblocks;
    const float* r_bias;
    const float* t_bias;
    const float* r_sqnorm;
    const float* t_sqnorm;
    int euclid;
    float* out;
    int64_t ld_out;
    float* part_vals;
    int32_t* part_idx;
    int capacity;
    int n_parts;
    int32_t t_index_base;
    float* blockmax;
    int64_t bm_stride;
    int sb_tiles;
    const int32_t* rblock_chunk;
    const int32_t* row_pair;
    const float* row_floor;
    const int32_t* row_index;
    int independent_lists;
    const float* scales;
    const float* sb_stats;
    const float* r_err;
    const float* wg_scale;
    const int32_t* wg_class;
    int64_t bias_stride;
    int grp_band_major;
    const float* cand_floor;
    int32_t* cand_n;
    int2* cand;
    int32_t cand_cap;
    const int32_t* wg_map;
    int32_t n_wgs;
    float* pre_max;
    int cand_diag;
    float* chunk_top;
    int top_k;
    int top_tag;
};

#define TREC_LB_TAG_BITS 12
__device__ __forceinline__ int lb_key(float x)
{
    const int b = __float_as_int(x);
    return b >= 0 ? b : (int)(0x80000000u - (unsigned int)b);
}
__device__ __forceinline__ float lb_tag(float lb, int idx)
{
    if (!(fabsf(lb) < 1e37f)) return -INFINITY;
    const int k2 = ((lb_key(lb) >> TREC_LB_TAG_BITS) - 1) * (1 << TREC_LB_TAG_BITS) + idx;
    const int b2 = k2 >= 0 ? k2 : (int)(0x80000000u - (unsigned int)k2);
    return __int_as_float(b2);
}
__device__ __forceinline__ int lb_tag_index(float tagged) { return lb_key(tagged) & ((1 << TREC_LB_TAG_BITS) - 1); }

__device__ __forceinline__ float i8_pair_err(float nx, float ex, float cu, float yh, float dy, float db, int kdim)
{
    const float ck = (float)(kdim + 6) * 2.98023224e-07f;
    const float e = nx * (dy + ck * yh) + ex * yh + db + cu;
    return e * 1.001953125f + 1e-30f;
}

int launch_blockmax_pipelined(const ScoreParams& p, int kt, hipStream_t stream);
int launch_blockmax_filter16(const ScoreParams& p, int kt, hipStream_t stream);
int launch_blockmax_pipelined_grouped(const ScoreParams& p, int kt, hipStream_t stream);
int launch_blockmax_pipelined_f32(const ScoreParams& p, int kt, int sb_rows, hipStream_t stream);
```

### tensorrec_amd/csrc/topk_cascade.hip

```cpp
#include "score_common.hpp"
#include "topk_common.hpp"

namespace {

constexpr int CROWS = 8;
constexpr int CGROUPS = 4;
constexpr int CUSERS = 1024;
constexpr int GROUP_ROWS = 512;

struct UserConsts { float f[4], nx[4], ex[4], au[4]; unsigned int valid; };

__device__ __forceinline__ UserConsts load_user_consts(const float* __restrict__ thr, const float* __restrict__ user_err,
                                                       int64_t n_users, int64_t u)
{
    const float infl = 1.0029296875f;
    UserConsts c;
    c.valid = 0u;
    float thv[4];
    f32x4 uvv[4];
#pragma unroll
    for (int e = 0; e < 4; ++e) {
        const int64_t ue_i = u + e < n_users ? u + e : n_users - 1;
        thv[e] = thr[ue_i];
        uvv[e] = *(const f32x4*)(user_err + ue_i * 4);
// ... 23 lines not shown
{
    const float infl = 1.0029296875f;
    const float ck = (float)(kdim + 6) * 2.98023224e-07f;
    const bool vec = (stride % 4 == 0) && (((uintptr_t)table % 16) == 0) && (u + 3 < stride);
    unsigned int bits = 0;
    f32x4 v[CROWS], ss[CROWS];
#pragma unroll
    for (int r = 0; r < CROWS; ++r) {
        const int32_t s = s0 + r < n_sb ? s0 + r : n_sb - 1;
        const float* src = table + (int64_t)s * stride + u;
        if (vec) v[r] = __builtin_nontemporal_load((const f32x4*)src);
        else {
            v[r] = (f32x4){-INFINITY, -INFINITY, -INFINITY, -INFINITY};
#pragma unroll
            for (int e = 0; e < 4; ++e) if (u + e < n_users) v[r][e] = src[e];
        }
        ss[r] = *(const f32x4*)(sb_stats + (int64_t)s * 4);
    }
#pragma unroll
    for (int r = 0; r < CROWS; ++r) {
        const int32_t s = s0 + r;
        const float A = (ss[r][2] + ck * ss[r][1]) * infl, B = ss[r][1] * infl, C = ss[r][3] * infl;
#pragma unroll
        for (int e = 0; e < 4; ++e)
            if (s < n_sb && ((c.valid >> e) & 1u) && !(__fmaf_rn(c.nx[e], A, __fmaf_rn(c.ex[e], B, __fmaf_rn(c.au[e], C, v[r][e]))) < c.f[e]))
                bits |= 1u << (4 * r + e);
    }
    return bits;
}

__global__ __launch_bounds__(256) void rows_collect_kernel(const float* __restrict__ table, int32_t n_sb, int64_t n_users,
                                                          int64_t stride, const float* __restrict__ thr,
                                                          const float* __restrict__ user_err,
                                                          const float* __restrict__ sb_stats, int kdim, int32_t rcap,
                                                          int32_t* __restrict__ row_count, int32_t* __restrict__ row_user, int rows_fast)
{
    __shared__ int wsum[2][CROWS][4];
    __shared__ int base_s[2][CROWS];
    const unsigned ublk = rows_fast ? blockIdx.y : blockIdx.x, rgrp = rows_fast ? blockIdx.x : blockIdx.y;
    const int64_t u = (int64_t)ublk * CUSERS + threadIdx.x * 4;
    const int lane = threadIdx.x & 63, wave = threadIdx.x >> 6;
    const UserConsts c = load_user_consts(thr, user_err, n_users, u);
    for (int g = 0; g < CGROUPS; ++g) {
        const int32_t s0 = (rgrp * CGROUPS + g) * CROWS;
        if (s0 >= n_sb) break;
        const unsigned int bits = tile_bits(table, n_sb, n_users, stride, c, sb_stats, kdim, s0, u);
        int pre[CROWS];
#pragma unroll
        for (int r = 0; r < CROWS; ++r) {
            const int k = __builtin_popcount((bits >> (4 * r)) & 15u);
            int inc = k;
            for (int off = 1; off < 64; off <<= 1) {
                const int t = __shfl_up(inc, off, 64);
                if (lane >= off) inc += t;
            }
            pre[r] = inc - k;
            if (lane == 63) wsum[g & 1][r][wave] = inc;
        }
        __syncthreads();
        if (threadIdx.x < CROWS && s0 + threadIdx.x < n_sb) {
            const int total = wsum[g & 1][threadIdx.x][0] + wsum[g & 1][threadIdx.x][1] + wsum[g & 1][threadIdx.x][2] +
                              wsum[g & 1][threadIdx.x][3];
            base_s[g & 1][threadIdx.x] = total ? atomicAdd(&row_count[s0 + threadIdx.x], total) : 0;
        }
        __syncthreads();
#pragma unroll
        for (int r = 0; r < CROWS; ++r) {
            const int32_t s = s0 + r;
            if (s >= n_sb) break;
            const unsigned int m = (bits >> (4 * r)) & 15u;
            if (m) {
                int idx = base_s[g & 1][r] + pre[r];
                for (int w = 0; w < wave; ++w) idx += wsum[g & 1][r][w];
#pragma unroll
                for (int e = 0; e < 4; ++e)
                    if ((m >> e) & 1u) {
                        if (idx < rcap) row_user[(int64_t)s * rcap + idx] = (int32_t)(u + e);
                        ++idx;
                    }
            }
        }
    }
}

__global__ __launch_bounds__(256) void rows_collect_wave_kernel(const float* __restrict__ table, int32_t n_sb, int64_t n_users,
                                                               int64_t stride, const float* __restrict__ thr,
                                                               const float* __restrict__ user_err,
                                                               const float* __restrict__ sb_stats, int kdim, int32_t rcap,
                                                               int32_t* __restrict__ row_count, int32_t* __restrict__ row_user)
{
    const int64_t u = (int64_t)blockIdx.y * CUSERS + threadIdx.x * 4;
    const int lane = threadIdx.x & 63;
    const UserConsts c = load_user_consts(thr, user_err, n_users, u);
    for (int g = 0; g < CGROUPS; ++g) {
        const int32_t s0 = (blockIdx.x * CGROUPS + g) * CROWS;
        if (s0 >= n_sb) break;
        const unsigned int bits = tile_bits(table, n_sb, n_users, stride, c, sb_stats, kdim, s0, u);
        if (__builtin_amdgcn_ballot_w64(bits != 0u) == 0ull) continue;
        int pre[CROWS];
        int mine = 0;
#pragma unroll
        for (int r = 0; r < CROWS; ++r) {
            const int k = __builtin_popcount((bits >> (4 * r)) & 15u);
            int inc = k;
            for (int off = 1; off < 64; off <<= 1) {
                const int t = __shfl_up(inc, off, 64);
                if (lane >= off) inc += t;
            }
            pre[r] = inc - k;
            const int tot = __shfl(inc, 63, 64);
            if (lane == r) mine = tot;
        }
        int base = 0;
        if (lane < CROWS && mine > 0 && s0 + lane < n_sb) base = atomicAdd(&row_count[s0 + lane], mine);
#pragma unroll
        for (int r = 0; r < CROWS; ++r) {
            const int32_t s = s0 + r;
            const int b = __shfl(base, r, 64);
            if (s >= n_sb) break;
            const unsigned int m = (bits >> (4 * r)) & 15u;
            if (m) {
                int idx = b + pre[r];
#pragma unroll
                for (int e = 0; e < 4; ++e)
                    if ((m >> e) & 1u) {
                        if (idx < rcap) row_user[(int64_t)s * rcap + idx] = (int32_t)(u + e);
                        ++idx;
                    }
            }
        }
    }
}

__global__ __launch_bounds__(256) void dense_users_kernel(const float* __restrict__ table, int32_t n_sb, int64_t n_users,
                                                         int64_t stride, const float* __restrict__ thr,
                                                         const float* __restrict__ user_err,
                                                         const float* __restrict__ sb_stats, int kdim, int32_t limit,
                                                         float* __restrict__ cand_floor, int32_t* __restrict__ flag,
                                                         int32_t* __restrict__ n_flagged)
{
    const int64_t u = ((int64_t)blockIdx.x * 256 + threadIdx.x) * 4;
    if (u >= n_users) return;
    const UserConsts c = load_user_consts(thr, user_err, n_users, u);
    int cnt[4] = {0, 0, 0, 0};
    const int32_t groups = n_sb / CROWS;
    for (int j = 0; j < 4; ++j) {
        const int32_t s0 = (int32_t)(((int64_t)groups * j) / 4) * CROWS;
        const unsigned int bits = tile_bits(table, n_sb, n_users, stride, c, sb_stats, kdim, s0, u);
#pragma unroll
        for (int e = 0; e < 4; ++e) cnt[e] += __builtin_popcount(bits & (0x11111111u << e));
    }
#pragma unroll
    for (int e = 0; e < 4; ++e)
        if (u + e < n_users && cnt[e] >= limit && cand_floor[u + e] < INFINITY) {
            cand_floor[u + e] = INFINITY;
            if (flag[u + e] == 0) { flag[u + e] = 1; atomicAdd(n_flagged, 1); }
        }
}

__global__ __launch_bounds__(256) void rows_status_kernel(const int32_t* __restrict__ row_count, int32_t n_sb, int32_t rcap,
                                                         int64_t* __restrict__ status)
{
    __shared__ long long tot[4];
    __shared__ int over[4];
    long long t = 0;
    int o = 0;
    for (int s = threadIdx.x; s < n_sb; s += 256) {
        const int c = row_count[s];
        o |= c > rcap;
        t += ((c < rcap ? c : rcap) + GROUP_ROWS - 1) / GROUP_ROWS * GROUP_ROWS;
    }
    for (int off = 32; off > 0; off >>= 1) { t += __shfl_xor(t, off, 64); o |= __shfl_xor(o, off, 64); }
    if ((threadIdx.x & 63) == 0) { tot[threadIdx.x >> 6] = t; over[threadIdx.x >> 6] = o; }
    __syncthreads();
    if (threadIdx.x == 0) {
        status[0] = tot[0] + tot[1] + tot[2] + tot[3];
        status[1] = (over[0] | over[1] | over[2] | over[3]) ? 1 : 0;
    }
}

__global__ __launch_bounds__(256) void rows_hot_kernel(int32_t* __restrict__ row_count, int32_t n_sb, int32_t rcap,
                                                      int64_t n_users, int32_t* __restrict__ hot_list, int32_t hot_cap,
                                                      int64_t max_pairs, int64_t* __restrict__ status)
{
    __shared__ int wcnt[4];
    __shared__ int base_s;
    __shared__ long long tot[4], totp[4];
    if (threadIdx.x == 0) base_s = 0;
    long long t = 0, tp = 0;
    __syncthreads();
    for (int s0 = 0; s0 < n_sb; s0 += 256) {
        const int s = s0 + threadIdx.x;
        const int c = s < n_sb ? row_count[s] : 0;
        const bool hot = c > rcap;
        const unsigned long long m = __builtin_amdgcn_ballot_w64(hot);
        const int lane = threadIdx.x & 63, wave = threadIdx.x >> 6;
        if (lane == 0) wcnt[wave] = __builtin_popcountll(m);
        __syncthreads();
        int idx = base_s + __builtin_popcountll(m & ((1ull << lane) - 1ull));
        for (int w = 0; w < wave; ++w) idx += wcnt[w];
        if (hot) {
            if (idx < hot_cap) hot_list[idx] = s;
            row_count[s] = 0;
        } else {
            t += (c + GROUP_ROWS - 1) / GROUP_ROWS * GROUP_ROWS;
            tp += c;
        }
        __syncthreads();
        if (threadIdx.x == 0) base_s += wcnt[0] + wcnt[1] + wcnt[2] + wcnt[3];
        __syncthreads();
    }
    for (int off = 32; off > 0; off >>= 1) { t += __shfl_xor(t, off, 64); tp += __shfl_xor(tp, off, 64); }
    if ((threadIdx.x & 63) == 0) { tot[threadIdx.x >> 6] = t; totp[threadIdx.x >> 6] = tp; }
    __syncthreads();
    const int n_hot = base_s;
    for (int j = n_hot + threadIdx.x; j < hot_cap; j += 256) hot_list[j] = -1;
    if (threadIdx.x == 0) {
        const long long per_hot = (n_users + GROUP_ROWS - 1) / GROUP_ROWS * GROUP_ROWS;
        const long long nh = n_hot < hot_cap ? n_hot : hot_cap;
        status[0] = tot[0] + tot[1] + tot[2] + tot[3] + nh * per_hot;
        const long long pairs = totp[0] + totp[1] + totp[2] + totp[3] + (long long)n_hot * n_users;
        status[1] = (n_hot > hot_cap || pairs > max_pairs) ? 1 : 0;
        status[2] = n_hot;
    }
}

}

extern "C" int trec_topk_rows_collect(const float* table, int32_t n_sb, int64_t n_users, int64_t stride, const float* thr,
                                      const float* user_err, const float* sb_stats, int32_t kdim, int32_t rcap,
                                      int32_t* row_count, int32_t* row_user, int64_t* status, void* stream)
{
    TREC_REQUIRE(table && thr && user_err && sb_stats && row_count && row_user && status, "trec_topk_rows_collect: null pointer");
    TREC_REQUIRE(n_sb >= 1 && n_users >= 1 && stride >= n_users, "trec_topk_rows_collect: bad sizes");
    TREC_REQUIRE(rcap >= GROUP_ROWS && rcap % GROUP_ROWS == 0, "trec_topk_rows_collect: rcap must be a multiple of 512");
    hipStream_t st = (hipStream_t)stream;
    const int n_ublk = (int)ceil_div64(n_users, CUSERS);
    const unsigned n_rgrp = (unsigned)((n_sb + CROWS * CGROUPS - 1) / (CROWS * CGROUPS));
    const int rows_fast = trec_get_tuning("rows_collect_rows_fast", 1) != 0 && n_ublk <= 65535;
    if (rows_fast && trec_get_tuning("rows_collect_per_wave", 1) != 0)
        hipLaunchKernelGGL(rows_collect_wave_kernel, dim3(n_rgrp, (unsigned)n_ublk), dim3(256), 0, st, table, n_sb, n_users, stride, thr,
                           user_err, sb_stats, kdim, rcap, row_count, row_user);
    else
    hipLaunchKernelGGL(rows_collect_kernel, rows_fast ? dim3(n_rgrp, (unsigned)n_ublk) : dim3((unsigned)n_ublk, n_rgrp),
                       dim3(256), 0, st, table, n_sb, n_users, stride, thr, user_err, sb_stats, kdim, rcap, row_count, row_user, rows_fast);
    hipLaunchKernelGGL(rows_status_kernel, dim3(1), dim3(256), 0, st, row_count, n_sb, rcap, status);
    return trec_check_launch("trec_topk_rows_collect");
}

extern "C" int trec_topk_rows_hot(int32_t* row_count, int32_t n_sb, int32_t rcap, int64_t n_users, int32_t* hot_list,
                                  int32_t hot_cap, int64_t max_pairs, int64_t* status, void* stream)
{
    TREC_REQUIRE(row_count && hot_list && status, "trec_topk_rows_hot: null pointer");
    TREC_REQUIRE(n_sb >= 1 && rcap >= 1 && hot_cap >= 1 && n_users >= 1, "trec_topk_rows_hot: bad sizes");
    hipLaunchKernelGGL(rows_hot_kernel, dim3(1), dim3(256), 0, (hipStream_t)stream, row_count, n_sb, rcap, n_users, hot_list,
                       hot_cap, max_pairs, status);
    return trec_check_launch("trec_topk_rows_hot");
}

extern "C" int trec_score_gemm_blockmax_hot(const void* users_bf16, const void* items_bf16, int32_t kpad, int64_t n_users,
                                            int64_t n_items, const float* user_bias, const float* item_bias, int32_t sb_rows,
                                            const int32_t* hot_list, int32_t hot_cap, float* blockmax, int64_t bm_stride,
                                            void* stream)
{
    TREC_REQUIRE(users_bf16 && items_bf16 && hot_list && blockmax, "trec_score_gemm_blockmax_hot: null pointer");
    TREC_REQUIRE(kpad == 64 || kpad == 128, "trec_score_gemm_blockmax_hot: kpad must be 64 or 128");
    TREC_REQUIRE(sb_rows >= 64 && sb_rows % 64 == 0 && hot_cap >= 1 && bm_stride >= n_users, "trec_score_gemm_blockmax_hot: bad sizes");
    if (n_users == 0 || n_items == 0) return TREC_OK;
    ScoreParams p = {};
    p.R = users_bf16; p.T = items_bf16; p.n_r = n_users; p.n_t = n_items;
    p.chunk_len = sb_rows; p.n_chunks = hot_cap;
    p.r_bias = user_bias; p.t_bias = item_bias;
    p.blockmax = blockmax; p.bm_stride = bm_stride; p.sb_tiles = sb_rows / 64;
    p.rblock_chunk = hot_list;
    return launch_blockmax_filter16(p, kpad, (hipStream_t)stream);
}

extern "C" int trec_score_gemm_blockmax_grouped(const void* users_bf16, const void* items_bf16, int32_t kpad, int64_t n_rows_g,
                                                int64_t n_items, const float* user_bias, const float* item_bias,
                                                int32_t sb_rows, const int32_t* rblock_chunk, const int32_t* row_user,
                                                float* blockmax, int64_t bm_stride, int32_t wgs_per_row, void* stream)
{
    TREC_REQUIRE(wgs_per_row >= 0, "trec_score_gemm_blockmax_grouped: wgs_per_row < 0");
    TREC_REQUIRE(users_bf16 && items_bf16 && rblock_chunk && row_user && blockmax, "trec_score_gemm_blockmax_grouped: null pointer");
    TREC_REQUIRE(kpad == 64 || kpad == 128, "trec_score_gemm_blockmax_grouped: kpad must be 64 or 128");
    TREC_REQUIRE(n_rows_g % GROUP_ROWS == 0 && n_rows_g < ((int64_t)1 << 40), "trec_score_gemm_blockmax_grouped: n_rows_g % 512 != 0");
    TREC_REQUIRE(sb_rows >= 64 && sb_rows % 64 == 0, "trec_score_gemm_blockmax_grouped: sb_rows must be a multiple of 64");
    if (n_rows_g == 0) return TREC_OK;
    TREC_REQUIRE(n_rows_g / GROUP_ROWS < ((int64_t)1 << 31), "trec_score_gemm_blockmax_grouped: too many workgroups");
    ScoreParams p = {};
    p.R = users_bf16; p.T = items_bf16; p.n_r = n_rows_g; p.n_t = n_items;
    p.chunk_len = sb_rows; p.n_chunks = 1;
    p.r_bias = user_bias; p.t_bias = item_bias;
    p.blockmax = blockmax; p.bm_stride = bm_stride; p.sb_tiles = sb_rows / 64;
    p.rblock_chunk = rblock_chunk; p.row_index = row_user; p.capacity = wgs_per_row;
    p.grp_band_major = trec_get_tuning("cascade_band_major", 0);
    return launch_blockmax_pipelined_grouped(p, kpad, (hipStream_t)stream);
}

extern "C" int trec_score_gemm_refine_candidates(const void* users_bf16, const void* items_bf16, int32_t kpad, int64_t n_rows_g,
                                                 int64_t n_items, const float* user_bias, const float* item_bias,
                                                 int32_t sb_rows, const int32_t* row_count, const int32_t* row_user,
                                                 float* blockmax, int64_t bm_stride, int32_t wgs_per_row,
                                                 const float* cand_floor, int32_t* cand_n, void* cand, int32_t cand_cap,
                                                 int32_t item_index_base, const int32_t* wg_map, int32_t n_wgs, void* stream)
{
    TREC_REQUIRE(users_bf16 && items_bf16 && row_count && row_user && blockmax && cand_floor && cand_n && cand,
                 "trec_score_gemm_refine_candidates: null pointer");
    TREC_REQUIRE(n_wgs >= 0 && (wg_map || n_wgs == 0), "trec_score_gemm_refine_candidates: n_wgs without wg_map");
    if (wg_map && n_wgs == 0) return TREC_OK;
    TREC_REQUIRE(wgs_per_row > 0 && cand_cap >= 1, "trec_score_gemm_refine_candidates: needs the fixed-capacity layout (wgs_per_row > 0)");
    TREC_REQUIRE(kpad == 64 || kpad == 128, "trec_score_gemm_refine_candidates: kpad must be 64 or 128");
    TREC_REQUIRE(n_rows_g % GROUP_ROWS == 0 && n_rows_g < ((int64_t)1 << 40), "trec_score_gemm_refine_candidates: n_rows_g % 512 != 0");
    TREC_REQUIRE(sb_rows >= 64 && sb_rows % 64 == 0 && sb_rows <= 65536, "trec_score_gemm_refine_candidates: sb_rows must be a multiple of 64, <= 65536");
    if (n_rows_g == 0) return TREC_OK;
    TREC_REQUIRE(n_rows_g / GROUP_ROWS < ((int64_t)1 << 31), "trec_score_gemm_refine_candidates: too many workgroups");
    ScoreParams p = {};
    p.R = users_bf16; p.T = items_bf16; p.n_r = n_rows_g; p.n_t = n_items;
    p.chunk_len = sb_rows; p.n_chunks = 1;
    p.r_bias = user_bias; p.t_bias = item_bias;
    p.blockmax = blockmax; p.bm_stride = bm_stride; p.sb_tiles = sb_rows / 64;
    p.rblock_chunk = row_count; p.row_index = row_user; p.capacity = wgs_per_row;
    p.cand_floor = cand_floor; p.cand_n = cand_n; p.cand = (int2*)cand; p.cand_cap = cand_cap; p.t_index_base = item_index_base;
    p.cand_diag = trec_get_tuning("cascade_cand_diag", 0);
    p.wg_map = wg_map; p.n_wgs = n_wgs;
    return launch_blockmax_pipelined_grouped(p, kpad, (hipStream_t)stream);
}

extern "C" int trec_score_gemm_refine_candidates_marked(const void* users_bf16, const void* items_bf16, int32_t kpad, int64_t n_rows_g,
                                                        int64_t n_items, const float* user_bias, const float* item_bias,
                                                        int32_t sb_rows, const int32_t* row_count, const int32_t* row_user,
                                                        float* blockmax, int64_t bm_stride, int32_t wgs_per_row,
                                                        const float* cand_floor, int32_t* cand_n, void* cand, int32_t cand_cap,
                                                        int32_t item_index_base, const int32_t* wg_map, int32_t n_wgs, float* pre_max,
                                                        void* stream)
{
    TREC_REQUIRE(users_bf16 && items_bf16 && row_count && row_user && blockmax && cand_floor && cand_n && cand && pre_max,
                 "trec_score_gemm_refine_candidates_marked: null pointer");
    TREC_REQUIRE(n_wgs >= 0 && (wg_map || n_wgs == 0), "trec_score_gemm_refine_candidates_marked: n_wgs without wg_map");
    if (wg_map && n_wgs == 0) return TREC_OK;
    TREC_REQUIRE(wgs_per_row > 0 && cand_cap >= 1, "trec_score_gemm_refine_candidates_marked: needs the fixed-capacity layout (wgs_per_row > 0)");
    TREC_REQUIRE(kpad == 64 || kpad == 128, "trec_score_gemm_refine_candidates_marked: kpad must be 64 or 128");
    TREC_REQUIRE(n_rows_g % GROUP_ROWS == 0 && n_rows_g < ((int64_t)1 << 40), "trec_score_gemm_refine_candidates_marked: n_rows_g % 512 != 0");
    TREC_REQUIRE(sb_rows >= 64 && sb_rows % 64 == 0 && sb_rows <= 65536, "trec_score_gemm_refine_candidates_marked: sb_rows must be a multiple of 64, <= 65536");
    if (n_rows_g == 0) return TREC_OK;
    TREC_REQUIRE(n_rows_g / GROUP_ROWS < ((int64_t)1 << 31), "trec_score_gemm_refine_candidates_marked: too many workgroups");
    ScoreParams p = {};
    p.R = users_bf16; p.T = items_bf16; p.n_r = n_rows_g; p.n_t = n_items;
    p.chunk_len = sb_rows; p.n_chunks = 1;
    p.r_bias = user_bias; p.t_bias = item_bias;
    p.blockmax = blockmax; p.bm_stride = bm_stride; p.sb_tiles = sb_rows / 64;
    p.rblock_chunk = row_count; p.row_index = row_user; p.capacity = wgs_per_row;
    p.cand_floor = cand_floor; p.cand_n = cand_n; p.cand = (int2*)cand; p.cand_cap = cand_cap; p.t_index_base = item_index_base;
    p.cand_diag = trec_get_tuning("cascade_cand_diag", 0);
    p.wg_map = wg_map; p.n_wgs = n_wgs;
    p.pre_max = pre_max;
    return launch_blockmax_pipelined_grouped(p, kpad, (hipStream_t)stream);
}

extern "C" int trec_score_gemm_refine_candidates_hot(const void* users_bf16, const void* items_bf16, int32_t kpad, int64_t n_users,
                                                     int64_t n_items, const float* user_bias, const float* item_bias,
                                                     int32_t sb_rows, const int32_t* hot_list, int32_t hot_cap, float* blockmax,
                                                     int64_t bm_stride, const float* cand_floor, int32_t* cand_n, void* cand,
                                                     int32_t cand_cap, int32_t item_index_base, void* stream)
{
    TREC_REQUIRE(users_bf16 && items_bf16 && hot_list && blockmax && cand_floor && cand_n && cand,
                 "trec_score_gemm_refine_candidates_hot: null pointer");
    TREC_REQUIRE(kpad == 64 || kpad == 128, "trec_score_gemm_refine_candidates_hot: kpad must be 64 or 128");
    TREC_REQUIRE(sb_rows >= 64 && sb_rows % 64 == 0 && sb_rows <= 65536 && hot_cap >= 1 && bm_stride >= n_users && cand_cap >= 1,
                 "trec_score_gemm_refine_candidates_hot: bad sizes");
    if (n_users == 0 || n_items == 0) return TREC_OK;
    ScoreParams p = {};
    p.R = users_bf16; p.T = items_bf16; p.n_r = n_users; p.n_t = n_items;
    p.chunk_len = sb_rows; p.n_chunks = hot_cap;
    p.r_bias = user_bias; p.t_bias = item_bias;
    p.blockmax = blockmax; p.bm_stride = bm_stride; p.sb_tiles = sb_rows / 64;
    p.rblock_chunk = hot_list;
    p.cand_floor = cand_floor; p.cand_n = cand_n; p.cand = (int2*)cand; p.cand_cap = cand_cap; p.t_index_base = item_index_base;
    return launch_blockmax_filter16(p, kpad, (hipStream_t)stream);
}

extern "C" int trec_topk_dense_users(const float* table, int32_t n_sb, int64_t n_users, int64_t stride, const float* thr,
                                     const float* user_err, const float* sb_stats, int32_t kdim, int32_t limit,
                                     float* cand_floor, int32_t* flag, int32_t* n_flagged, void* stream)
{
    TREC_REQUIRE(table && thr && user_err && sb_stats && cand_floor && flag && n_flagged, "trec_topk_dense_users: null pointer");
    TREC_REQUIRE(n_sb >= 32 && stride >= n_users && limit >= 1 && limit <= 32, "trec_topk_dense_users: need n_sb >= 32, 1 <= limit <= 32");
    if (n_users == 0) return TREC_OK;
    hipLaunchKernelGGL(dense_users_kernel, dim3((unsigned)ceil_div64(n_users, 1024)), dim3(256), 0, (hipStream_t)stream, table, n_sb,
                       n_users, stride, thr, user_err, sb_stats, kdim, limit, cand_floor, flag, n_flagged);
    return trec_check_launch("trec_topk_dense_users");
}

namespace {
__global__ __launch_bounds__(256) void wg_start_kernel(const int32_t* __restrict__ row_count, int32_t n_sb, int32_t wgs_per_row,
                                                      int32_t* __restrict__ wg_start, int32_t group_rows)
{
    __shared__ int wsum[4];
    __shared__ int base_s;
    if (threadIdx.x == 0) base_s = 0;
    __syncthreads();
    const int lane = threadIdx.x & 63, wave = threadIdx.x >> 6;
    for (int s0 = 0; s0 < n_sb; s0 += 256) {
        const int s = s0 + threadIdx.x;
        int c = s < n_sb ? (row_count[s] + group_rows - 1) / group_rows : 0;
        if (c > wgs_per_row) c = wgs_per_row;
        int inc = c;
        for (int off = 1; off < 64; off <<= 1) {
            const int t = __shfl_up(inc, off, 64);
            if (lane >= off) inc += t;
        }
        if (lane == 63) wsum[wave] = inc;
        __syncthreads();
        int excl = base_s + inc - c;
        for (int w = 0; w < wave; ++w) excl += wsum[w];
        if (s < n_sb) wg_start[s] = excl;
        __syncthreads();
        if (threadIdx.x == 0) base_s += wsum[0] + wsum[1] + wsum[2] + wsum[3];
        __syncthreads();
    }
    if (threadIdx.x == 0) wg_start[n_sb] = base_s;
}

__global__ __launch_bounds__(256) void wg_map_kernel(const int32_t* __restrict__ wg_start, int32_t wgs_per_row, int64_t map_cap,
                                                    int32_t* __restrict__ wg_map)
{
    const int s = blockIdx.x;
    const int b = wg_start[s], e = wg_start[s + 1];
    for (int j = threadIdx.x; j < e - b; j += 256)
        if ((int64_t)b + j < map_cap) wg_map[b + j] = s * wgs_per_row + j;
}
}

extern "C" int trec_topk_rows_wg_map(const int32_t* row_count, int32_t n_sb, int32_t wgs_per_row, int32_t* wg_start,
                                     int32_t* wg_map, int64_t map_cap, void* stream)
{
    TREC_REQUIRE(row_count && wg_start && wg_map, "trec_topk_rows_wg_map: null pointer");
    TREC_REQUIRE(n_sb >= 1 && wgs_per_row >= 1 && map_cap >= 0 && (int64_t)n_sb * wgs_per_row < ((int64_t)1 << 31),
                 "trec_topk_rows_wg_map: bad sizes");
    hipStream_t st = (hipStream_t)stream;
    hipLaunchKernelGGL(wg_start_kernel, dim3(1), dim3(256), 0, st, row_count, n_sb, wgs_per_row, wg_start, GROUP_ROWS);
    hipLaunchKernelGGL(wg_map_kernel, dim3((unsigned)n_sb), dim3(256), 0, st, wg_start, wgs_per_row, map_cap, wg_map);
    return trec_check_launch("trec_topk_rows_wg_map");
}
```

### tensorrec_amd/ops_topk.py

```python
from .ops_base import (DTYPE_BF16, DTYPE_F32, MODE_DOT, MODE_EUCLIDEAN, N, _f32c, _timed, gemm_raw, group_pairs_by_item,
                       l2_normalize_rows, pair_scores_exact, rank_rows, torch)

def score_kpad(d):
    k = N.query("trec_score_kpad", int(d))
    if k < 0:
        raise ValueError("n_components = %d is beyond the MFMA score kernel's limit of 256" % d)
    return k


def score_prep(repr_, dtype=DTYPE_F32, normalize=False, want_sqnorm=False):
    x = _f32c(repr_.detach())
    n, d = x.shape
    kpad = score_kpad(d)
    if dtype == DTYPE_F32 and kpad == d and not normalize and not want_sqnorm:
        return x, None, kpad
    out = torch.empty((n, kpad), dtype=torch.float32 if dtype == DTYPE_F32 else torch.bfloat16, device=x.device)
    sq = torch.empty((n,), dtype=torch.float32, device=x.device) if want_sqnorm else None
    N.call("trec_score_prep", N.ptr(x), n, d, kpad, 1 if normalize else 0, dtype, N.ptr(out), N.ptr(sq))
    return out, sq, kpad


SCORE_KMAX = 256


# ... 303 lines not shown
def score_prep_filter(repr_, normalize=False, bias=None, want_gstats=False, sort_users=False, k=10, user_bias=None):
    x = _f32c(repr_.detach())
    n, d = x.shape
    kpad = score_kpad(d)
    if sort_users and kpad <= 128 and n > 0 and i8_user_classes_enabled():
        return _prep_users_sorted(x, normalize, k, user_bias)
    op = FilterOperand()
    op.n, op.d, op.kpad = n, d, kpad
    own_f32 = normalize or kpad != d
    op.f32 = torch.empty((n, kpad), dtype=torch.float32, device=x.device) if own_f32 else x
    op.bf16 = torch.empty((n, kpad), dtype=torch.bfloat16, device=x.device)
    op.stats = torch.empty((n, 2), dtype=torch.float32, device=x.device)
    op.gstats = zero_block(4, x.device)[:3].view(torch.float32) if want_gstats else None
    with _timed("score_prep_filter"):
        N.call("trec_score_prep_filter", N.ptr(x), n, d, kpad, 1 if normalize else 0, N.ptr(bias),
               N.ptr(op.f32) if own_f32 else None, N.ptr(op.bf16), N.ptr(op.stats), N.ptr(op.gstats))
    return op


def spmm_filter_operand(features, w, bias=None, want_gstats=False):
    w = _f32c(w)
    d = w.shape[1]
    n = features.shape[0]
    op = FilterOperand()
    op.n, op.d, op.kpad = n, d, d
    op.f32 = torch.empty((n, d), dtype=torch.float32, device=w.device)
    op.bf16 = torch.empty((n, d), dtype=torch.bfloat16, device=w.device)
    op.stats = torch.empty((n, 2), dtype=torch.float32, device=w.device)
    op.gstats = torch.zeros((3,), dtype=torch.float32, device=w.device) if want_gstats else None
    with _timed("spmm_csr"):
        N.call("trec_spmm_csr_filter", N.ptr(features.indptr), N.ptr(features.indices), N.ptr(features.values), n,
               features.nnz, N.ptr(w), d, N.ptr(op.f32), N.ptr(op.bf16), N.ptr(op.stats), N.ptr(op.gstats))
    if want_gstats and bias is not None:
        import ctypes
        N.call("trec_absmax", N.ptr(bias), bias.numel(), ctypes.c_void_p(op.gstats.data_ptr() + 8))
    return op


I8_USER_CLIP_SIGMAS = 4.0
CASCADE_MAX_REFINED = 0.45
CASCADE_ROW_CAPACITY = 0.50
CASCADE_MAX_HOT = 1 << 20
CASCADE_CANDIDATES = 256
CASCADE_DENSE_USER_LIMIT = 16
CASCADE_MAX_CHUNKS = 128
CASCADE_PREREFINE_MIN_SB = 32
CASCADE_MIN_ITEMS = 262144


TOPK_USER_BATCH_MAX = 4_194_304


def topk_user_batch(n_users, n_items, n_components, device, fraction=0.6, route="cascade", k=10):
    n_sb = (int(n_items) + SUPERBLOCK_ROWS - 1) // SUPERBLOCK_ROWS
    kpad = max(32, (int(n_components) + 31) // 32 * 32)
    if route == "cascade":
        per_user = 1.3 * (n_sb * (4 + 12 * CASCADE_ROW_CAPACITY) + 8 * kpad + 1024 + 8 * CASCADE_CANDIDATES + 256 + 16 * int(k))
    elif route == "wide":
        per_user = 1.3 * (n_sb * (4 + 12 * CASCADE_ROW_CAPACITY) + 8 * kpad + 1024 + 8 * WIDE_CANDIDATES + 32 * int(k))
    else:
        cap = max(16, int(N.query("trec_score_topk_capacity", min(16, int(k)))))
        lists = 2 * (2 * int(k)) * cap * 8 if int(k) <= 16 else max(2 * (2 * int(k)) * cap * 8, 2 * 4 * SUPERBLOCK_ROWS * int(k))
        per_user = 1.3 * (n_sb * 4 + 6 * kpad + int(k) * kpad * 4 + lists + 1024)
    try:
        free, _total = torch.cuda.mem_get_info(device)
    except Exception:
        free = 16 << 30
    return int(max(65536, min(int(n_users), TOPK_USER_BATCH_MAX, fraction * free / per_user)))


def cascade_prefilter_for(n_components, n_items_total, enabled=None):
    if not (N.load().trec_get_tuning(b"topk_int8_prefilter", 1) != 0 if enabled is None else enabled):
        return None
    return "int8" if score_kpad(n_components) in (64, 128) and n_items_total >= CASCADE_MIN_ITEMS else None


def score_prep_i8_pair(uop, iop, item_bias=None, sb_rows=None, top_k=10):
    if uop.kpad > 128:
        raise ValueError("int8 pre-filter covers kpad <= 128")
    sb_rows = int(sb_rows or SUPERBLOCK_ROWS)
    dev = uop.f32.device
    classes = uop.src is not None
    with _timed("score_prep_i8"):
        fresh_items = iop.i8 is None or iop.sb_rows != sb_rows
        n_sb = (iop.n + sb_rows - 1) // sb_rows
        if fresh_items:
            zb = zero_block(8 + 4 * n_sb, dev).view(torch.float32)
            iop.scales = zb[0:3]
            iop.gstats8 = zb[4:8]
            iop.sb_stats = zb[8:].reshape(n_sb, 4)
            iop.sb_rows = sb_rows
            iop.i8 = torch.empty((iop.n, iop.kpad), dtype=torch.int8, device=dev)
            iop.stats8 = torch.empty((iop.n, 2), dtype=torch.float32, device=dev)
            N.call("trec_score_prep_i8", N.ptr(iop.f32), iop.n, iop.f32.shape[1], iop.kpad, 1, 0.0, sb_rows, None,
                   N.ptr(iop.scales), None, N.ptr(iop.i8), N.ptr(iop.stats8), None, N.ptr(iop.sb_stats), N.ptr(iop.gstats8))
        else:
            iop.gstats8[2:].zero_()
            iop.sb_stats[:, 3].zero_()
        if classes:
            wg_rows = int(N.query("trec_score_blockmax_i8_rows_per_workgroup", int(top_k)))
            if wg_rows != uop.wg_rows:
                raise ValueError("the user operand was laid out for int8 workgroups of %s rows, this call needs %d "
                                 "(score_prep_filter(sort_users=True, k=...) must be given the same k)" % (uop.wg_rows, wg_rows))
            iop.bias_q = None
            if item_bias is not None:
                iop.bias_q = torch.empty((I8_N_CLASSES, iop.n), dtype=torch.int32, device=dev)
                N.call("trec_score_bias_i8_classes", N.ptr(item_bias), iop.n, sb_rows, N.ptr(uop.ladder), N.ptr(uop.class_used),
                       I8_N_CLASSES, N.ptr(iop.sb_stats), N.ptr(iop.bias_q), N.ptr(iop.gstats8))
        else:
            uop.i8 = torch.empty((uop.n, uop.kpad), dtype=torch.int8, device=dev)
            uop.stats8 = torch.empty((uop.n, 2), dtype=torch.float32, device=dev)
            uop.wg_class = uop.wg_scale = None
            ws = torch.empty((2,), dtype=torch.float64, device=dev)
            clip = N.load().trec_get_tuning(b"i8_user_clip_x10", int(I8_USER_CLIP_SIGMAS * 10)) / 10.0
            N.call("trec_score_prep_i8", N.ptr(uop.f32), uop.n, uop.f32.shape[1], uop.kpad, 0, float(clip), 0, None,
                   N.ptr(iop.scales), N.ptr(ws), N.ptr(uop.i8), N.ptr(uop.stats8), None, None, None)
            iop.bias_q = torch.empty((iop.n,), dtype=torch.int32, device=dev) if item_bias is not None else None
            if item_bias is not None:
                N.call("trec_score_prep_i8", None, iop.n, iop.f32.shape[1], iop.kpad, 2, 0.0, sb_rows, N.ptr(item_bias),
                       N.ptr(iop.scales), None, None, None, N.ptr(iop.bias_q), N.ptr(iop.sb_stats), N.ptr(iop.gstats8))
    import weakref
    iop.bias_owner = weakref.ref(uop)
    return uop, iop


def blockmax_i8_chunks(n_items, n_chunks, sb_rows):
    chunk_len = -(-(-(-n_items // n_chunks)) // sb_rows) * sb_rows
    return chunk_len, -(-n_items // chunk_len)


class _Candidates(object):
    __slots__ = ("n", "items", "cap", "floor0", "flag", "n_flagged", "pre")


def cascade_lists_candidates():
    return N.load().trec_get_tuning(b"cascade_candidates", 1) != 0


def _cascade_stage1(uop, iop, k, user_bias, item_bias, sb_rows, n_sb, n_chunks, floor_exchange, stats_exchange, gstats_all=None,
                    item_index_base=0, candidates_cap=None):
    dev = uop.bf16.device
    n_u, n_i, kpad = uop.n, iop.n, uop.kpad
    kk = int(k)
    top_k = 10 if kk <= 10 else 16
    if uop.i8 is None or iop.i8 is None or iop.sb_rows != sb_rows or iop.bias_owner is None or iop.bias_owner() is not uop:
        score_prep_i8_pair(uop, iop, item_bias, sb_rows, top_k)
    gstats8 = iop.gstats8
    if stats_exchange is not None:
        gstats8 = gstats8.clone()
        gstats8[2] = gstats_all[2] if gstats_all is not None else stats_exchange(gstats8)[2]
    user_err = torch.empty((n_u, 4), dtype=torch.float32, device=dev)
    N.call("trec_score_user_err_i8", N.ptr(uop.stats8), N.ptr(user_bias), N.ptr(gstats8), kpad, n_u, N.ptr(iop.scales),
           N.ptr(uop.wg_scale), int(uop.wg_rows or 0) if uop.wg_scale is not None else 0, N.ptr(user_err))
    stride = (n_u + 3) // 4 * 4
    chunk_len, n_ch = blockmax_i8_chunks(n_i, n_chunks, sb_rows)
    table = torch.empty((n_sb, stride), dtype=torch.float32, device=dev)
    chunk_top = torch.empty((n_ch * top_k, stride), dtype=torch.float32, device=dev)
    lib = N.load()
    lists = cascade_lists_candidates() and gstats_all is not None and sb_rows <= 65536
    sb_per_chunk = chunk_len // sb_rows
    pre = (lists and floor_exchange is None and stats_exchange is None and kk <= WIDE_K_MAX
           and lib.trec_get_tuning(b"cascade_prerefine", 1) != 0 and sb_per_chunk <= 4096
           and CASCADE_PREREFINE_MIN_SB <= n_sb <= int(N.query("trec_topk_prerefine_max_superblocks")))
    if pre and kk > 16:
        pre = (lib.trec_get_tuning(b"wide_prerefine", 1) != 0
               and n_sb >= 4 * kk)
    with _timed("score_gemm_blockmax_i8"):
        N.call("trec_score_gemm_blockmax_i8", N.ptr(uop.i8), N.ptr(iop.i8), kpad, n_u, n_i, N.ptr(user_bias),
               N.ptr(iop.bias_q), N.ptr(iop.scales), N.ptr(iop.sb_stats), sb_rows, n_chunks, N.ptr(table), stride,
               N.ptr(user_err), N.ptr(chunk_top), top_k | (0x100 if pre else 0), N.ptr(uop.wg_scale), N.ptr(uop.wg_class),
               int(uop.wg_rows or 0) if uop.wg_scale is not None else 0)
    sel = torch.empty((n_u, kk), dtype=torch.int32, device=dev)
    sel_max = torch.empty((kk, n_u), dtype=torch.float32, device=dev) if (floor_exchange is not None or pre) else None
    tau = torch.empty((n_u,), dtype=torch.float32, device=dev)
    with _timed("topk_select_blocks"):
        if kk <= 16:
            N.call("trec_topk_select_blocks", N.ptr(chunk_top), n_ch * top_k, n_u, stride, kk, N.ptr(sel), N.ptr(sel_max),
                   N.ptr(tau))
        else:
            N.call("trec_topk_select_blocks_ex", N.ptr(chunk_top), n_ch * top_k, n_u, stride, kk, kk, N.ptr(sel), N.ptr(sel_max),
                   N.ptr(tau))
    if floor_exchange is not None:
        tau = floor_exchange(sel_max).contiguous()
    zb = zero_block(8 + n_sb, dev)
    status = zb[0:6].view(torch.int64)
    n_flagged0 = zb[6:7]
    row_count = zb[8:8 + n_sb]
    cands = None
    if lists:
        cands = _Candidates()
        cands.pre = None
        cands.cap = int(candidates_cap) if candidates_cap is not None else \
            int(N.load().trec_get_tuning(b"cascade_candidates_cap", CASCADE_CANDIDATES))
        cands.floor0 = torch.empty((n_u,), dtype=torch.float32, device=dev)
        cands.flag = torch.empty((n_u,), dtype=torch.int32, device=dev)
        cands.n_flagged = n_flagged0
        cands.n = torch.empty((n_u,), dtype=torch.int32, device=dev)
        N.call("trec_topk_cascade_floor", N.ptr(tau), N.ptr(uop.src), N.ptr(uop.stats), N.ptr(user_bias), N.ptr(gstats_all), kpad,
               n_u, N.ptr(cands.floor0), N.ptr(cands.flag), N.ptr(cands.n_flagged), N.ptr(cands.n))
        try:
            cands.items = torch.empty((n_u, cands.cap, 2), dtype=torch.int32, device=dev)
        except torch.cuda.OutOfMemoryError:
            cands.cap = 64
            cands.items = torch.empty((n_u, cands.cap, 2), dtype=torch.int32, device=dev)
    if pre:
        n_cap_a = int(uop.n_real or n_u)
        rcap_frac_a = lib.trec_get_tuning(b"cascade_rcap_pct", int(100 * CASCADE_ROW_CAPACITY)) / 100.0
        rcap_a = (int(rcap_frac_a * n_cap_a) + 511) // 512 * 512 + 512
        pre_ws = zero_block(n_sb + 1, dev)
        sel_sb = torch.empty((n_u, kk), dtype=torch.int32, device=dev)
        pre_ok = torch.empty((n_u,), dtype=torch.int32, device=dev)
        pre_rows = torch.empty((n_sb * rcap_a,), dtype=torch.int32, device=dev)
        pre_vals = torch.empty((n_u, kk), dtype=torch.float32, device=dev)
        if n_sb >= 32 and lib.trec_get_tuning(b"prerefine_early_dense", 1 if kk <= 16 else 0) != 0:
            N.call("trec_topk_dense_users", N.ptr(table), n_sb, n_u, stride, N.ptr(tau), N.ptr(user_err), N.ptr(iop.sb_stats),
                   kpad, CASCADE_DENSE_USER_LIMIT if n_i >= CASCADE_MIN_ITEMS else 30, N.ptr(cands.floor0), N.ptr(cands.flag),
                   N.ptr(cands.n_flagged))
        sel_pos = torch.empty((n_u, kk), dtype=torch.int32, device=dev)
        pre_max = torch.empty((n_sb * rcap_a,), dtype=torch.float32, device=dev)
        with _timed("topk_prerefine"):
            N.call("trec_topk_prerefine_rows_pos", N.ptr(sel), N.ptr(sel_max), kk, top_k, sb_per_chunk, n_sb, n_u, N.ptr(uop.src),
                   rcap_a, N.ptr(sel_sb), N.ptr(pre_ws), N.ptr(pre_rows), N.ptr(pre_ok), N.ptr(sel_pos))
        n_wgs_a = n_cap_a * kk // 512 + n_sb + 1
        wg_start_a = torch.empty((n_sb + 1,), dtype=torch.int32, device=dev)
        wg_map_a = torch.full((n_wgs_a,), n_sb * (rcap_a // 512), dtype=torch.int32, device=dev)
        N.call("trec_topk_rows_wg_map", N.ptr(pre_ws), n_sb, rcap_a // 512, N.ptr(wg_start_a), N.ptr(wg_map_a), n_wgs_a)
        with _timed("score_gemm_blockmax_pre"):
            N.call("trec_score_gemm_refine_candidates_marked", N.ptr(uop.bf16), N.ptr(iop.bf16), kpad, n_sb * rcap_a, n_i,
                   N.ptr(user_bias), N.ptr(item_bias), sb_rows, N.ptr(pre_ws), N.ptr(pre_rows), N.ptr(table), stride,
                   rcap_a // 512, N.ptr(cands.floor0), N.ptr(cands.n), N.ptr(cands.items), cands.cap, int(item_index_base),
                   N.ptr(wg_map_a), n_wgs_a, N.ptr(pre_max))
        with _timed("topk_prerefine"):
            N.call("trec_topk_prerefine_tau_listed", N.ptr(sel_sb), N.ptr(sel_pos), N.ptr(pre_ok), kk, N.ptr(pre_max), rcap_a, n_u,
                   N.ptr(uop.src), N.ptr(uop.stats), N.ptr(user_bias), N.ptr(gstats_all), kpad, N.ptr(tau), N.ptr(pre_vals),
                   N.ptr(cands.floor0))
        cands.pre = (sel_sb, pre_vals)
        if FILTER_DEBUG is not None:
            FILTER_DEBUG.update({"prerefine_users_ok": int(pre_ok.sum().item()), "prerefine_rcap": rcap_a,
                                 "prerefine_row_count_max": int(pre_ws[:n_sb].max().item()), "prerefine_listed": 1,
                                 "prerefine_pairs": int((sel_sb >= 0).sum().item())})
    if cands is None and uop.src is not None:
        tau.masked_fill_(uop.src < 0, float("inf"))
    n_cap = int(uop.n_real or n_u)
    rcap_frac = N.load().trec_get_tuning(b"cascade_rcap_pct", int(100 * CASCADE_ROW_CAPACITY)) / 100.0
    rcap = (int(rcap_frac * n_cap) + 511) // 512 * 512 + 512
    row_user = torch.empty((n_sb * rcap,), dtype=torch.int32, device=dev)
    with _timed("topk_rows_compact"):
        N.call("trec_topk_rows_collect", N.ptr(table), n_sb, n_u, stride, N.ptr(tau), N.ptr(user_err),
               N.ptr(iop.sb_stats), kpad, rcap, N.ptr(row_count), N.ptr(row_user), N.ptr(status))
    if FILTER_DEBUG is not None:
        FILTER_DEBUG.update({"int8_pairs_wanted": int(row_count.sum().item()), "int8_pairs_total": int(n_sb) * int(n_u),
                             "rcap": rcap, "row_count_max": int(row_count.max().item()),
                             "hot_superblocks": int((row_count > rcap).sum().item())})
    hot_cap = max(8, min(N.load().trec_get_tuning(b"cascade_max_hot", CASCADE_MAX_HOT), n_sb))
    hot_list = torch.empty((hot_cap,), dtype=torch.int32, device=dev)
    max_pairs = int(N.load().trec_get_tuning(b"cascade_max_refined_pct", int(100 * CASCADE_MAX_REFINED)) / 100.0 * n_sb * n_cap)
    N.call("trec_topk_rows_hot", N.ptr(row_count), n_sb, rcap, n_u, N.ptr(hot_list), hot_cap, max_pairs, N.ptr(status))
    if cands is not None:
        if n_sb >= 32:
            N.call("trec_topk_dense_users", N.ptr(table), n_sb, n_u, stride, N.ptr(tau), N.ptr(user_err), N.ptr(iop.sb_stats),
                   kpad, CASCADE_DENSE_USER_LIMIT if n_i >= CASCADE_MIN_ITEMS else 30, N.ptr(cands.floor0), N.ptr(cands.flag),
                   N.ptr(cands.n_flagged))
        wg_cap = min(n_sb * (rcap // 512), max_pairs // 512 + n_sb + 1)
        wg_start = torch.empty((n_sb + 1,), dtype=torch.int32, device=dev)
        wg_map = torch.empty((wg_cap,), dtype=torch.int32, device=dev)
        N.call("trec_topk_rows_wg_map", N.ptr(row_count), n_sb, rcap // 512, N.ptr(wg_start), N.ptr(wg_map), wg_cap)
    rows, overflow, n_hot = status.tolist()
    if stats_exchange is not None:
        overflow = float(stats_exchange(torch.tensor([float(overflow)], device=dev)).item())
    if overflow:
        return None, stride, (int(rows), True), tau, None
    n_hot = min(int(n_hot), hot_cap)
    with _timed("score_gemm_blockmax_grouped"):
        if cands is not None:
            n_wgs = min(wg_cap, (int(rows) - n_hot * ((n_u + 511) // 512 * 512)) // 512)
            N.call("trec_score_gemm_refine_candidates", N.ptr(uop.bf16), N.ptr(iop.bf16), kpad, n_sb * rcap, n_i,
                   N.ptr(user_bias), N.ptr(item_bias), sb_rows, N.ptr(row_count), N.ptr(row_user), N.ptr(table), stride,
                   rcap // 512, N.ptr(cands.floor0), N.ptr(cands.n), N.ptr(cands.items), cands.cap, int(item_index_base),
                   N.ptr(wg_map), n_wgs)
        else:
            N.call("trec_score_gemm_blockmax_grouped", N.ptr(uop.bf16), N.ptr(iop.bf16), kpad, n_sb * rcap, n_i,
                   N.ptr(user_bias), N.ptr(item_bias), sb_rows, N.ptr(row_count), N.ptr(row_user), N.ptr(table), stride,
                   rcap // 512)
    with _timed("score_gemm_blockmax_hot"):
        if n_hot == 0:
            pass
        elif cands is not None:
            N.call("trec_score_gemm_refine_candidates_hot", N.ptr(uop.bf16), N.ptr(iop.bf16), kpad, n_u, n_i,
                   N.ptr(user_bias), N.ptr(item_bias), sb_rows, N.ptr(hot_list), n_hot, N.ptr(table), stride,
                   N.ptr(cands.floor0), N.ptr(cands.n), N.ptr(cands.items), cands.cap, int(item_index_base))
        else:
            N.call("trec_score_gemm_blockmax_hot", N.ptr(uop.bf16), N.ptr(iop.bf16), kpad, n_u, n_i, N.ptr(user_bias),
                   N.ptr(item_bias), sb_rows, N.ptr(hot_list), n_hot, N.ptr(table), stride)
    return table, stride, (int(rows), False), tau, cands

def _filter_tail(uop, iop, blockmax, bm_stride, n_u, n_sb, k, user_bias, item_bias, item_index_base, sb_rows, variant, ksel,
                 cap, floor, flag, n_flagged, rows_wg, wide=False, keys_count=None):
    dev = uop.bf16.device
    n_i, kpad = iop.n, uop.kpad
    n_pairs = n_u * ksel
    if keys_count is not None:
        keys, count = keys_count
    else:
        keys = torch.empty((n_pairs,), dtype=torch.int32, device=dev)
        count = torch.empty((n_u,), dtype=torch.int32, device=dev)
        with _timed("topk_collect_blocks"):
            N.call("trec_topk_collect_blocks", N.ptr(blockmax), n_sb, n_u, bm_stride, N.ptr(floor), ksel, N.ptr(keys),
                   N.ptr(count), N.ptr(flag), N.ptr(n_flagged))
    if FILTER_DEBUG is not None and not wide:
        FILTER_DEBUG["flagged_after_collect"] = int(n_flagged.item())
        _debug_counts("kept_superblocks", count)
        true_cnt = torch.zeros((n_u,), dtype=torch.int32, device=dev)
        for s0 in range(0, n_sb, 64):
            true_cnt += (blockmax[s0:s0 + 64, :n_u] >= floor[None, :]).sum(0, dtype=torch.int32)
        _debug_counts("kept_superblocks_uncapped", true_cnt)
    indptr_t, users_t, perm_t = group_pairs_by_item(None, keys, ksel, n_sb + 1)
    cnt_pad = torch.empty((n_sb + 1,), dtype=torch.int32, device=dev)
    N.call("trec_topk_pad_counts", N.ptr(indptr_t), n_sb, rows_wg, N.ptr(cnt_pad))
    pstart = torch.empty((n_sb + 2,), dtype=torch.int64, device=dev)
    ws64 = torch.empty(((n_sb + 1 + 1023) // 1024 + 1,), dtype=torch.int64, device=dev)
    N.call("trec_exclusive_scan_i32", N.ptr(cnt_pad), n_sb + 1, N.ptr(ws64), N.ptr(pstart))
    max_rows = (n_pairs + min(n_sb, n_pairs) * (rows_wg - 1) + rows_wg - 1) // rows_wg * rows_wg
    row_user = torch.empty((max_rows,), dtype=torch.int32, device=dev)
    row_pair = torch.empty((max_rows,), dtype=torch.int32, device=dev)
    rblock_chunk = torch.empty((max_rows // rows_wg,), dtype=torch.int32, device=dev)
    with _timed("topk_fill_groups"):
        N.call("trec_topk_fill_groups_index", N.ptr(pstart), N.ptr(indptr_t), N.ptr(users_t), N.ptr(perm_t), n_sb, rows_wg,
               max_rows, N.ptr(row_user), N.ptr(row_pair), N.ptr(rblock_chunk))
    pi = torch.empty((n_pairs * 2, cap), dtype=torch.int32, device=dev)
    with _timed("score_gemm_topk_grouped"):
        N.call("trec_score_gemm_topk_grouped", N.ptr(uop.bf16), N.ptr(iop.bf16), DTYPE_BF16, kpad, max_rows, n_i,
               item_index_base, N.ptr(user_bias), N.ptr(item_bias), MODE_DOT, None, None, sb_rows, N.ptr(rblock_chunk),
               N.ptr(row_pair), N.ptr(floor), cap, None, N.ptr(pi), (variant & 1) | 16, N.ptr(row_user))
    ov = torch.empty((n_u, int(k)), dtype=torch.float32, device=dev)
    oi = torch.empty((n_u, int(k)), dtype=torch.int32, device=dev)
    with _timed("topk_filter_finish"):
        N.call("trec_topk_filter_finish_wide" if wide else "trec_topk_filter_finish", N.ptr(pi), cap, ksel, N.ptr(count),
               N.ptr(uop.f32), N.ptr(iop.f32), kpad, kpad, uop.d, N.ptr(user_bias), N.ptr(item_bias), item_index_base, n_u,
               int(k), N.ptr(ov), N.ptr(oi), N.ptr(flag), N.ptr(n_flagged))
    return ov, oi, count


WIDE_PASS_BYTES = 4 << 30


def _wide_second_pass(uop, iop, blockmax, bad, n_sb, k, user_bias, item_bias, item_index_base, sb_rows, variant, floor, rows_wg,
                      ksel_w, gstats=None):
    dev = uop.bf16.device
    per_chain = max(1024, WIDE_PASS_BYTES // (ksel_w * 2 * 16 * 4))
    out_v, out_i, out_f = [], [], []
    with _timed("topk_filter_wide_pass"):
        for s0 in range(0, int(bad.numel()), per_chain):
            b = bad[s0:s0 + per_chain]
            n_b = int(b.numel())
            sub = FilterOperand()
            sub.n, sub.d, sub.kpad = n_b, uop.d, uop.kpad
            sub.bf16 = uop.bf16.index_select(0, b)
            sub.f32 = uop.f32.index_select(0, b)
            table_b = blockmax.index_select(1, b)
            ub = user_bias.index_select(0, b) if user_bias is not None else None
            flag_b = torch.zeros((n_b,), dtype=torch.int32, device=dev)
            n_flagged_b = torch.zeros((1,), dtype=torch.int32, device=dev)
            if floor is None:
                sub.stats = uop.stats.index_select(0, b)
                sel_b = torch.empty((n_b, int(k)), dtype=torch.int32, device=dev)
                tau_b = torch.empty((n_b,), dtype=torch.float32, device=dev)
                floor_b = torch.empty((n_b,), dtype=torch.float32, device=dev)
                N.call("trec_topk_select_blocks", N.ptr(table_b), n_sb, n_b, n_b, int(k), N.ptr(sel_b), None, N.ptr(tau_b))
                N.call("trec_topk_filter_floor", N.ptr(tau_b), N.ptr(sub.stats), N.ptr(ub), N.ptr(gstats), uop.kpad, n_b,
                       N.ptr(floor_b), N.ptr(flag_b), N.ptr(n_flagged_b))
            else:
                floor_b = floor.index_select(0, b)
            wv, wi, _ = _filter_tail(sub, iop, table_b, n_b, n_b, n_sb, k, ub, item_bias, item_index_base, sb_rows, variant,
                                     ksel_w, 16, floor_b, flag_b, n_flagged_b, rows_wg, wide=True)
            out_v.append(wv); out_i.append(wi); out_f.append(flag_b)
            del table_b, sub
    return torch.cat(out_v), torch.cat(out_i), torch.cat(out_f)


def score_topk_filtered(uop, iop, k, user_bias=None, item_bias=None, item_index_base=0, sb_rows=None, variant=1,
                        n_chunks=None, floor_exchange=None, stats_exchange=None, ksel=None, prefilter=None, finish_lanes=0):
    if uop.src is None:
        return _score_topk_filtered(uop, iop, k, user_bias, item_bias, item_index_base, sb_rows, variant, n_chunks,
                                    floor_exchange, stats_exchange, ksel, prefilter, finish_lanes=finish_lanes)
    if user_bias is None:
        ub = None
    elif uop.bias_sorted is not None and uop.bias_ref is user_bias:
        ub = uop.bias_sorted
    else:
        ub = user_bias.reshape(-1).index_select(0, uop.perm).masked_fill_(uop.pad, 0.0)
    ov, oi = _score_topk_filtered(uop, iop, k, ub, item_bias, item_index_base, sb_rows, variant, n_chunks,
                                  floor_exchange, stats_exchange, ksel, prefilter, caller_order=True, finish_lanes=finish_lanes)
    LAST_FILTER_STATS["users"] = int(uop.n_real)
    LAST_FILTER_STATS["layout_rows"] = int(uop.n)
    return ov, oi


def _score_topk_filtered(uop, iop, k, user_bias=None, item_bias=None, item_index_base=0, sb_rows=None, variant=1,
                         n_chunks=None, floor_exchange=None, stats_exchange=None, ksel=None, prefilter=None,
                         caller_order=False, finish_lanes=0):
    if not 1 <= int(k) <= 16:
        raise ValueError("fused top-k supports k <= 16 (got %d)" % k)
    cap = 8
    dev = uop.bf16.device
    n_u, n_i, kpad = uop.n, iop.n, uop.kpad
    if iop.kpad != kpad or iop.gstats is None:
        raise ValueError("score_topk_filtered: operands must share kpad and the item side needs gstats")
    sb_rows = int(sb_rows or SUPERBLOCK_ROWS)
    n_sb = (n_i + sb_rows - 1) // sb_rows
    if n_sb < int(k):
        raise ValueError("score_topk_filtered needs at least k superblocks of items")
    ksel = min(int(ksel or FILTER_KSEL), n_sb)
    ksel = max(ksel, int(k))
    rows_wg = N.query("trec_score_rows_per_workgroup", DTYPE_BF16, kpad)
# ... 457 lines not shown
```

Measured before the change: 11600 billion predictions/s.

## Quantize blockmax upper bounds to 16-bit keys for cascade row collection

The int8 blockmax GEMM now also writes a uint16 key per (superblock, user) cell. The key encodes the upper bound (score plus error) on a per-workgroup grid computed by a new key_grid kernel. The downstream rows_collect and dense_users passes read these compact keys against a quantized threshold instead of the fp32 table plus per-user error stats, cutting their memory traffic and arithmetic. In exchange it adds an extra int16 table write in the GEMM, a grid kernel launch, and conservative quantization that may admit somewhat more candidate pairs.

```diff
diff --git a/include/tensorrec_hip.h b/include/tensorrec_hip.h
--- a/include/tensorrec_hip.h
+++ b/include/tensorrec_hip.h
@@ -191,6 +191,28 @@
                                              int32_t wgs_per_row, const float* cand_floor, int32_t* cand_n, void* cand,
                                              int32_t cand_cap, int32_t item_index_base, const int32_t* wg_map, int32_t n_wgs,
                                              float* pre_max, void* stream);
+int trec_score_key_grid(const float* user_err, const float* user_bias, const float* gstats, const float* sb_stats, int32_t n_sb,
+                        int32_t kdim, int64_t n_users, int32_t wg_rows, float* key_grid, void* stream);
+int trec_score_gemm_blockmax_i8_keys(const void* users_q, const void* items_q, int32_t kpad, int64_t n_users, int64_t n_items,
+                                     const float* user_bias, const int32_t* item_bias_q, const float* scales,
+                                     const float* sb_stats, int32_t sb_rows, int32_t n_chunks, float* blockmax, int64_t bm_stride,
+                                     const float* user_err, float* chunk_top, int32_t top_k, const float* wg_scale,
+                                     const int32_t* wg_class, int32_t wg_rows, void* keys, int64_t key_stride,
+                                     const float* key_grid, void* stream);
+int trec_topk_rows_collect_keys(const void* keys, int32_t n_sb, int64_t n_users, int64_t key_stride, const float* thr,
+                                const float* key_grid, int32_t wg_rows, int32_t rcap, int32_t* row_count, int32_t* row_user,
+                                int64_t* status, void* stream);
+int trec_topk_dense_users_keys(const void* keys, int32_t n_sb, int64_t n_users, int64_t key_stride, const float* thr,
+                               const float* key_grid, int32_t wg_rows, int32_t limit, float* cand_floor, int32_t* flag,
+                               int32_t* n_flagged, void* stream);
+int trec_score_gemm_refine_candidates_marked_keys(const void* users_bf16, const void* items_bf16, int32_t kpad, int64_t n_rows_g,
+                                                  int64_t n_items, const float* user_bias, const float* item_bias, int32_t sb_rows,
+                                                  const int32_t* row_count, const int32_t* row_user, float* blockmax,
+                                                  int64_t bm_stride, int32_t wgs_per_row, const float* cand_floor, int32_t* cand_n,
+                                                  void* cand, int32_t cand_cap, int32_t item_index_base, const int32_t* wg_map,
+                                                  int32_t n_wgs, float* pre_max, void* keys, int64_t key_stride, void* stream);
+int trec_cascade_keys_host(const float* ub, const float* tau, const float* r, int64_t n, uint16_t* key, int32_t* tkey,
+                           float* grid);
 int trec_topk_euclid_certify(const int32_t* cand_idx, const float* cand_g, const float* exact, int32_t kc, int32_t k,
                              const float* user_sq, const float* user_bias, const float* item_gstats, const float* bias_max,
                              int32_t kdim, int64_t n_users, float* out_vals, int32_t* out_idx, int32_t* flag,
diff --git a/tensorrec_amd/_native.py b/tensorrec_amd/_native.py
--- a/tensorrec_amd/_native.py
+++ b/tensorrec_amd/_native.py
@@ -71,6 +71,14 @@
     "trec_topk_prerefine_tau_listed": [_vp, _vp, _vp, _i32, _vp, _i32, _i64, _vp, _vp, _vp, _vp, _i32, _vp, _vp, _vp, _vp],
     "trec_score_gemm_refine_candidates_marked": [_vp, _vp, _i32, _i64, _i64, _vp, _vp, _i32, _vp, _vp, _vp, _i64, _i32, _vp, _vp, _vp,
                                                  _i32, _i32, _vp, _i32, _vp, _vp],
+    "trec_score_key_grid": [_vp, _vp, _vp, _vp, _i32, _i32, _i64, _i32, _vp, _vp],
+    "trec_score_gemm_blockmax_i8_keys": [_vp, _vp, _i32, _i64, _i64, _vp, _vp, _vp, _vp, _i32, _i32, _vp, _i64, _vp, _vp, _i32,
+                                         _vp, _vp, _i32, _vp, _i64, _vp, _vp],
+    "trec_topk_rows_collect_keys": [_vp, _i32, _i64, _i64, _vp, _vp, _i32, _i32, _vp, _vp, _vp, _vp],
+    "trec_topk_dense_users_keys": [_vp, _i32, _i64, _i64, _vp, _vp, _i32, _i32, _vp, _vp, _vp, _vp],
+    "trec_score_gemm_refine_candidates_marked_keys": [_vp, _vp, _i32, _i64, _i64, _vp, _vp, _i32, _vp, _vp, _vp, _i64, _i32, _vp,
+                                                      _vp, _vp, _i32, _i32, _vp, _i32, _vp, _vp, _i64, _vp],
+    "trec_cascade_keys_host": [_vp, _vp, _vp, _i64, _vp, _vp, _vp],
     "trec_topk_rows_collect": [_vp, _i32, _i64, _i64, _vp, _vp, _vp, _i32, _i32, _vp, _vp, _vp, _vp],
     "trec_score_gemm_blockmax_grouped": [_vp, _vp, _i32, _i64, _i64, _vp, _vp, _i32, _vp, _vp, _vp, _i64, _i32, _vp],
     "trec_topk_rows_hot": [_vp, _i32, _i32, _i64, _vp, _i32, _i64, _vp, _vp],
diff --git a/tensorrec_amd/csrc/score_blockmax.hip b/tensorrec_amd/csrc/score_blockmax.hip
--- a/tensorrec_amd/csrc/score_blockmax.hip
+++ b/tensorrec_amd/csrc/score_blockmax.hip
@@ -542,6 +542,7 @@
                             const int64_t rb = ((int64_t)__builtin_amdgcn_readfirstlane(rblock) * 4 + wave) * (NUB * 16);
                             p.pre_max[rb + slot] = v;
                             p.blockmax[sb * p.bm_stride + ou] = -INFINITY;
+                            if (p.keys) p.keys[sb * p.key_stride + ou] = 0;
                         }
                     } else if (ou >= 0) p.blockmax[sb * p.bm_stride + ou] = v;
                 }
diff --git a/tensorrec_amd/csrc/score_blockmax_i8.hip b/tensorrec_amd/csrc/score_blockmax_i8.hip
--- a/tensorrec_amd/csrc/score_blockmax_i8.hip
+++ b/tensorrec_amd/csrc/score_blockmax_i8.hip
@@ -153,6 +153,8 @@
     __syncthreads();
 
     const float a_user = p.wg_scale ? p.wg_scale[rblock] : p.scales[0];
+    const float k_inv = (TK && p.keys) ? __int_as_float(__builtin_amdgcn_readfirstlane(__float_as_int(p.key_grid[4 * rblock]))) : 0.f;
+    const float k_c0 = (TK && p.keys) ? __int_as_float(__builtin_amdgcn_readfirstlane(__float_as_int(p.key_grid[4 * rblock + 1]))) : 0.f;
     const int64_t sb0 = t_begin / ((int64_t)p.sb_tiles * BNQ);
     f32x4 ss_cur = *(const f32x4*)(p.sb_stats + sb0 * 4), ss_next = ss_cur;
     for (int t = 0; t < n_tiles; ++t) {
@@ -178,14 +180,22 @@
                 m[ub] = x > o2 ? x : o2;
                 bm[ub] = INT_MIN;
             }
+            int mo_[OW];
+#pragma unroll
+            for (int o = 0; o < OW; ++o) mo_[o] = g == 0 ? m[o] : (g == 1 ? m[OW + o] : (g == 2 ? m[2 * OW + o] : m[3 * OW + o]));
 #pragma unroll
             for (int o = 0; o < OW; ++o) {
-                const int mo = g == 0 ? m[o] : (g == 1 ? m[OW + o] : (g == 2 ? m[2 * OW + o] : m[3 * OW + o]));
+                const int mo = mo_[o];
                 float v = (float)mo * scale;
                 if (BIAS) v = v + own_bias[o];
-                if (own_u[o] < p.n_r) p.blockmax[sb * p.bm_stride + own_u[o]] = v;
+                const float e = TK ? i8_pair_err(e_nx[o], e_ex[o], e_cu[o], yh, dy, db, KT) : 0.f;
+                if (own_u[o] < p.n_r) {
+                    const int64_t cell = sb * p.bm_stride + own_u[o];
+                    p.blockmax[cell] = v;
+                    if (TK && p.keys) p.keys[cell] = (uint16_t)i8_ub_key(__builtin_fmaf(e, 1.001f, v), k_inv, k_c0);
+                }
                 if (TK) {
-                    float lb = v - i8_pair_err(e_nx[o], e_ex[o], e_cu[o], yh, dy, db, KT);
+                    float lb = v - e;
                     lb = (lb == lb) ? lb : -INFINITY;
                     if (p.top_tag) lb = lb_tag(lb, t / p.sb_tiles);
 #pragma unroll
@@ -582,12 +592,97 @@
     return trec_check_launch("trec_score_user_err_i8");
 }
 
+namespace {
+int blockmax_i8_stage(const void* users_q, const void* items_q, int32_t kpad, int64_t n_users, int64_t n_items,
+                      const float* user_bias, const int32_t* item_bias_q, const float* scales, const float* sb_stats,
+                      int32_t sb_rows, int32_t n_chunks, float* blockmax, int64_t bm_stride, const float* user_err,
+                      float* chunk_top, int32_t top_k, const float* wg_scale, const int32_t* wg_class, int32_t wg_rows,
+                      uint16_t* keys, int64_t key_stride, const float* key_grid, void* stream);
+
+__global__ __launch_bounds__(256) void key_grid_kernel(const float* __restrict__ r_err, const float* __restrict__ user_bias,
+                                                      const float* __restrict__ gstats, const float* __restrict__ sb_stats,
+                                                      int32_t n_sb, int kdim, int64_t n_users, int32_t wg_rows,
+                                                      float* __restrict__ key_grid)
+{
+    float y = 0.f, d = 0.f, c = 0.f;
+    for (int s = threadIdx.x; s < n_sb; s += 256) {
+        const f32x4 ss = *(const f32x4*)(sb_stats + (int64_t)s * 4);
+        if (ss[1] < INFINITY) y = fmaxf(y, ss[1]);
+        if (ss[2] < INFINITY) d = fmaxf(d, ss[2]);
+        if (ss[3] < INFINITY) c = fmaxf(c, ss[3]);
+    }
+    __shared__ float w[4][4];
+    for (int off = 32; off > 0; off >>= 1) {
+        y = fmaxf(y, __shfl_xor(y, off, 64)); d = fmaxf(d, __shfl_xor(d, off, 64)); c = fmaxf(c, __shfl_xor(c, off, 64));
+    }
+    if ((threadIdx.x & 63) == 0) { w[0][threadIdx.x >> 6] = y; w[1][threadIdx.x >> 6] = d; w[2][threadIdx.x >> 6] = c; }
+    __syncthreads();
+    y = fmaxf(fmaxf(w[0][0], w[0][1]), fmaxf(w[0][2], w[0][3]));
+    d = fmaxf(fmaxf(w[1][0], w[1][1]), fmaxf(w[1][2], w[1][3]));
+    c = fmaxf(fmaxf(w[2][0], w[2][1]), fmaxf(w[2][2], w[2][3]));
+    const float bmax = gstats ? gstats[2] : 0.f;
+    float r = 0.f;
+    const int64_t u0 = (int64_t)blockIdx.x * wg_rows;
+    for (int64_t u = u0 + threadIdx.x; u < u0 + wg_rows && u < n_users; u += 256) {
+        const f32x4 ue = *(const f32x4*)(r_err + u * 4);
+        const float bsum = (user_bias ? fabsf(user_bias[u]) : 0.f) + bmax;
+        const float e_max = i8_pair_err(ue[0], ue[1], ue[2], y, d, ue[3] * c, kdim);
+        const float ru = 1.002f * (ue[0] * y + bsum) + 2.01f * e_max + 1e-24f;
+        if (ru < INFINITY) r = fmaxf(r, ru);
+    }
+    for (int off = 32; off > 0; off >>= 1) r = fmaxf(r, __shfl_xor(r, off, 64));
+    if ((threadIdx.x & 63) == 0) w[3][threadIdx.x >> 6] = r;
+    __syncthreads();
+    if (threadIdx.x == 0) {
+        float r_eff, inv, c0k, c0t;
+        i8_key_grid(fmaxf(fmaxf(w[3][0], w[3][1]), fmaxf(w[3][2], w[3][3])), &r_eff, &inv, &c0k, &c0t);
+        *(f32x4*)(key_grid + (int64_t)blockIdx.x * 4) = (f32x4){inv, c0k, c0t, r_eff};
+    }
+}
+}
+
+extern "C" int trec_score_key_grid(const float* user_err, const float* user_bias, const float* gstats, const float* sb_stats,
+                                   int32_t n_sb, int32_t kdim, int64_t n_users, int32_t wg_rows, float* key_grid, void* stream)
+{
+    TREC_REQUIRE(user_err && sb_stats && key_grid && n_sb >= 1 && kdim >= 1, "trec_score_key_grid: bad arguments");
+    TREC_REQUIRE(wg_rows == NWQ * 12 * 16 || wg_rows == NWQ * 8 * 16, "trec_score_key_grid: wg_rows must be the int8 workgroup's height");
+    TREC_REQUIRE(((uintptr_t)user_err % 16) == 0 && ((uintptr_t)key_grid % 16) == 0, "trec_score_key_grid: unaligned pointer");
+    if (n_users == 0) return TREC_OK;
+    hipLaunchKernelGGL(key_grid_kernel, dim3((unsigned)ceil_div64(n_users, wg_rows)), dim3(256), 0, (hipStream_t)stream, user_err,
+                       user_bias, gstats, sb_stats, n_sb, kdim, n_users, wg_rows, key_grid);
+    return trec_check_launch("trec_score_key_grid");
+}
+
+extern "C" int trec_score_gemm_blockmax_i8_keys(const void* users_q, const void* items_q, int32_t kpad, int64_t n_users,
+                                                int64_t n_items, const float* user_bias, const int32_t* item_bias_q,
+                                                const float* scales, const float* sb_stats, int32_t sb_rows, int32_t n_chunks,
+                                                float* blockmax, int64_t bm_stride, const float* user_err, float* chunk_top,
+                                                int32_t top_k, const float* wg_scale, const int32_t* wg_class, int32_t wg_rows,
+                                                void* keys, int64_t key_stride, const float* key_grid, void* stream)
+{
+    TREC_REQUIRE(keys && key_grid, "trec_score_gemm_blockmax_i8_keys: null pointer");
+    return blockmax_i8_stage(users_q, items_q, kpad, n_users, n_items, user_bias, item_bias_q, scales, sb_stats, sb_rows, n_chunks,
+                             blockmax, bm_stride, user_err, chunk_top, top_k, wg_scale, wg_class, wg_rows, (uint16_t*)keys, key_stride,
+                             key_grid, stream);
+}
+
 extern "C" int trec_score_gemm_blockmax_i8(const void* users_q, const void* items_q, int32_t kpad, int64_t n_users,
                                            int64_t n_items, const float* user_bias, const int32_t* item_bias_q,
                                            const float* scales, const float* sb_stats, int32_t sb_rows, int32_t n_chunks,
                                            float* blockmax, int64_t bm_stride, const float* user_err, float* chunk_top,
                                            int32_t top_k, const float* wg_scale, const int32_t* wg_class, int32_t wg_rows,
                                            void* stream)
+{
+    return blockmax_i8_stage(users_q, items_q, kpad, n_users, n_items, user_bias, item_bias_q, scales, sb_stats, sb_rows, n_chunks,
+                             blockmax, bm_stride, user_err, chunk_top, top_k, wg_scale, wg_class, wg_rows, nullptr, 0, nullptr, stream);
+}
+
+namespace {
+int blockmax_i8_stage(const void* users_q, const void* items_q, int32_t kpad, int64_t n_users, int64_t n_items,
+                      const float* user_bias, const int32_t* item_bias_q, const float* scales, const float* sb_stats,
+                      int32_t sb_rows, int32_t n_chunks, float* blockmax, int64_t bm_stride, const float* user_err,
+                      float* chunk_top, int32_t top_k, const float* wg_scale, const int32_t* wg_class, int32_t wg_rows,
+                      uint16_t* keys, int64_t key_stride, const float* key_grid, void* stream)
 {
     const int top_tag = (top_k & 0x100) ? 1 : 0;
     top_k &= 0xff;
@@ -612,8 +707,12 @@
     TREC_REQUIRE(!top_tag || (top_k && p.chunk_len / sb_rows <= (1 << TREC_LB_TAG_BITS)),
                  "trec_score_gemm_blockmax_i8: tagged lower bounds need the lists and chunks of at most 4096 superblocks");
     p.wg_scale = wg_scale; p.wg_class = item_bias_q ? wg_class : nullptr; p.bias_stride = n_items;
+    TREC_REQUIRE(!keys || (chunk_top && key_grid && key_stride == bm_stride),
+                 "trec_score_gemm_blockmax_i8_keys: the keys need the lists (user_err, chunk_top), key_grid and the table's row stride");
+    p.keys = keys; p.key_stride = key_stride; p.key_grid = key_grid;
     hipStream_t st = (hipStream_t)stream;
     const bool bias = user_bias || item_bias_q;
     if (kpad == 128) return bias ? launch_i8x16_lists<128, true>(p, sb_rows, st) : launch_i8x16_lists<128, false>(p, sb_rows, st);
     return bias ? launch_i8x16_lists<64, true>(p, sb_rows, st) : launch_i8x16_lists<64, false>(p, sb_rows, st);
 }
+}
diff --git a/tensorrec_amd/csrc/score_common.hpp b/tensorrec_amd/csrc/score_common.hpp
--- a/tensorrec_amd/csrc/score_common.hpp
+++ b/tensorrec_amd/csrc/score_common.hpp
@@ -46,6 +46,9 @@
     float* chunk_top;
     int top_k;
     int top_tag;
+    uint16_t* keys;
+    int64_t key_stride;
+    const float* key_grid;
 };
 
 #define TREC_LB_TAG_BITS 12
@@ -70,6 +73,29 @@
     return e * 1.001953125f + 1e-30f;
 }
 
+__host__ __device__ __forceinline__ void i8_key_grid(float r, float* r_eff, float* inv, float* c0k, float* c0t)
+{
+    float c = r;
+    if (!(c < 1e37f)) c = 1e37f;
+    if (!(c > 1e-24f)) c = 1e-24f;
+    *r_eff = c;
+    *inv = 32766.f / c;
+    const float ri = c * *inv;
+    *c0k = (ri + 1.0625f) + 2e-30f * *inv;
+    *c0t = ri - 0.0625f;
+}
+__host__ __device__ __forceinline__ unsigned int i8_ub_key(float ub, float inv, float c0k)
+{
+    return (unsigned int)fmaxf(fminf(ceilf(__builtin_fmaf(ub, inv, c0k)), 65535.f), 1.f);
+}
+__host__ __device__ __forceinline__ unsigned int i8_thr_key(float tau, float inv, float c0t)
+{
+    if (tau != tau) return 1u;
+    if (tau == INFINITY) return 65536u;
+    const float b = ceilf(__builtin_fmaf(tau, inv, c0t));
+    return 1u + (unsigned int)(!(b > 0.f) ? 0.f : (b < 65534.f ? b : 65534.f));
+}
+
 int launch_blockmax_pipelined(const ScoreParams& p, int kt, hipStream_t stream);
 int launch_blockmax_filter16(const ScoreParams& p, int kt, hipStream_t stream);
 int launch_blockmax_pipelined_grouped(const ScoreParams& p, int kt, hipStream_t stream);
diff --git a/tensorrec_amd/csrc/topk_cascade.hip b/tensorrec_amd/csrc/topk_cascade.hip
--- a/tensorrec_amd/csrc/topk_cascade.hip
+++ b/tensorrec_amd/csrc/topk_cascade.hip
@@ -199,6 +199,128 @@
     }
 #pragma unroll
     for (int e = 0; e < 4; ++e)
+        if (u + e < n_users && cnt[e] >= limit && cand_floor[u + e] < INFINITY) {
+            cand_floor[u + e] = INFINITY;
+            if (flag[u + e] == 0) { flag[u + e] = 1; atomicAdd(n_flagged, 1); }
+        }
+}
+
+constexpr int KUSERS = 2048;
+
+struct KeyConsts { unsigned int tk[8]; };
+
+__device__ __forceinline__ KeyConsts load_key_consts(const float* __restrict__ thr, const float* __restrict__ key_grid,
+                                                     int32_t wg_rows, int64_t n_users, int64_t u)
+{
+    KeyConsts c;
+    float th[8];
+    const int64_t uc = u < n_users ? u : n_users - 1;
+    const f32x4 g = *(const f32x4*)(key_grid + 4 * (int64_t)((unsigned int)uc / (unsigned int)wg_rows));
+    if (u + 7 < n_users && ((uintptr_t)thr % 16) == 0) {
+        const f32x4 t0 = *(const f32x4*)(thr + u), t1 = *(const f32x4*)(thr + u + 4);
+#pragma unroll
+        for (int e = 0; e < 4; ++e) { th[e] = t0[e]; th[4 + e] = t1[e]; }
+    } else {
+#pragma unroll
+        for (int e = 0; e < 8; ++e) th[e] = thr[u + e < n_users ? u + e : n_users - 1];
+    }
+#pragma unroll
+    for (int e = 0; e < 8; ++e) c.tk[e] = u + e < n_users ? i8_thr_key(th[e], g[0], g[2]) : 65536u;
+    return c;
+}
+
+__device__ __forceinline__ unsigned long long key_tile_bits(const uint16_t* __restrict__ keys, int32_t n_sb, int64_t key_stride,
+                                                            const KeyConsts& c, int32_t s0, int64_t u)
+{
+    u32x4 v[CROWS];
+#pragma unroll
+    for (int r = 0; r < CROWS; ++r) {
+        const int32_t s = s0 + r < n_sb ? s0 + r : n_sb - 1;
+        v[r] = (u32x4){0u, 0u, 0u, 0u};
+        if (u < key_stride) v[r] = __builtin_nontemporal_load((const u32x4*)(keys + (int64_t)s * key_stride + u));
+    }
+    unsigned long long bits = 0ull;
+#pragma unroll
+    for (int r = 0; r < CROWS; ++r) {
+        if (s0 + r >= n_sb) break;
+        unsigned int b = 0u;
+#pragma unroll
+        for (int e = 0; e < 8; ++e) {
+            const unsigned int k = (e & 1) ? (v[r][e >> 1] >> 16) : (v[r][e >> 1] & 0xffffu);
+            if (k >= c.tk[e]) b |= 1u << e;
+        }
+        bits |= (unsigned long long)b << (8 * r);
+    }
+    return bits;
+}
+
+__global__ __launch_bounds__(256) void rows_collect_keys_kernel(const uint16_t* __restrict__ keys, int32_t n_sb, int64_t n_users,
+                                                               int64_t key_stride, const float* __restrict__ thr,
+                                                               const float* __restrict__ key_grid, int32_t wg_rows, int32_t rcap,
+                                                               int32_t* __restrict__ row_count, int32_t* __restrict__ row_user)
+{
+    const int64_t u = (int64_t)blockIdx.y * KUSERS + threadIdx.x * 8;
+    const int lane = threadIdx.x & 63;
+    const KeyConsts c = load_key_consts(thr, key_grid, wg_rows, n_users, u);
+    for (int g = 0; g < CGROUPS; ++g) {
+        const int32_t s0 = (blockIdx.x * CGROUPS + g) * CROWS;
+        if (s0 >= n_sb) break;
+        const unsigned long long bits = key_tile_bits(keys, n_sb, key_stride, c, s0, u);
+        if (__builtin_amdgcn_ballot_w64(bits != 0ull) == 0ull) continue;
+        int pre[CROWS];
+        int mine = 0;
+#pragma unroll
+        for (int r = 0; r < CROWS; ++r) {
+            const int k = __builtin_popcount((unsigned int)(bits >> (8 * r)) & 255u);
+            int inc = k;
+            for (int off = 1; off < 64; off <<= 1) {
+                const int t = __shfl_up(inc, off, 64);
+                if (lane >= off) inc += t;
+            }
+            pre[r] = inc - k;
+            const int tot = __shfl(inc, 63, 64);
+            if (lane == r) mine = tot;
+        }
+        int base = 0;
+        if (lane < CROWS && mine > 0 && s0 + lane < n_sb) base = atomicAdd(&row_count[s0 + lane], mine);
+#pragma unroll
+        for (int r = 0; r < CROWS; ++r) {
+            const int32_t s = s0 + r;
+            const int b = __shfl(base, r, 64);
+            if (s >= n_sb) break;
+            const unsigned int m = (unsigned int)(bits >> (8 * r)) & 255u;
+            if (m) {
+                int idx = b + pre[r];
+#pragma unroll
+                for (int e = 0; e < 8; ++e)
+                    if ((m >> e) & 1u) {
+                        if (idx < rcap) row_user[(int64_t)s * rcap + idx] = (int32_t)(u + e);
+                        ++idx;
+                    }
+            }
+        }
+    }
+}
+
+__global__ __launch_bounds__(256) void dense_users_keys_kernel(const uint16_t* __restrict__ keys, int32_t n_sb, int64_t n_users,
+                                                              int64_t key_stride, const float* __restrict__ thr,
+                                                              const float* __restrict__ key_grid, int32_t wg_rows, int32_t limit,
+                                                              float* __restrict__ cand_floor, int32_t* __restrict__ flag,
+                                                              int32_t* __restrict__ n_flagged)
+{
+    const int64_t u = ((int64_t)blockIdx.x * 256 + threadIdx.x) * 8;
+    if (u >= n_users) return;
+    const KeyConsts c = load_key_consts(thr, key_grid, wg_rows, n_users, u);
+    int cnt[8] = {0, 0, 0, 0, 0, 0, 0, 0};
+    const int32_t groups = n_sb / CROWS;
+    for (int j = 0; j < 4; ++j) {
+        const int32_t s0 = (int32_t)(((int64_t)groups * j) / 4) * CROWS;
+        const unsigned long long bits = key_tile_bits(keys, n_sb, key_stride, c, s0, u);
+#pragma unroll
+        for (int e = 0; e < 8; ++e) cnt[e] += __builtin_popcountll(bits & (0x0101010101010101ull << e));
+    }
+#pragma unroll
+    for (int e = 0; e < 8; ++e)
         if (u + e < n_users && cnt[e] >= limit && cand_floor[u + e] < INFINITY) {
             cand_floor[u + e] = INFINITY;
             if (flag[u + e] == 0) { flag[u + e] = 1; atomicAdd(n_flagged, 1); }
@@ -293,6 +415,39 @@
                        dim3(256), 0, st, table, n_sb, n_users, stride, thr, user_err, sb_stats, kdim, rcap, row_count, row_user, rows_fast);
     hipLaunchKernelGGL(rows_status_kernel, dim3(1), dim3(256), 0, st, row_count, n_sb, rcap, status);
     return trec_check_launch("trec_topk_rows_collect");
+}
+
+extern "C" int trec_topk_rows_collect_keys(const void* keys, int32_t n_sb, int64_t n_users, int64_t key_stride, const float* thr,
+                                           const float* key_grid, int32_t wg_rows, int32_t rcap, int32_t* row_count,
+                                           int32_t* row_user, int64_t* status, void* stream)
+{
+    TREC_REQUIRE(keys && thr && key_grid && row_count && row_user && status, "trec_topk_rows_collect_keys: null pointer");
+    TREC_REQUIRE(n_sb >= 1 && n_users >= 1 && key_stride >= n_users && key_stride % 8 == 0, "trec_topk_rows_collect_keys: bad sizes (key_stride % 8)");
+    TREC_REQUIRE(wg_rows >= 8 && wg_rows % 8 == 0 && n_users < ((int64_t)1 << 31), "trec_topk_rows_collect_keys: wg_rows must be a multiple of 8");
+    TREC_REQUIRE(((uintptr_t)keys % 16) == 0 && ((uintptr_t)key_grid % 16) == 0,
+                 "trec_topk_rows_collect_keys: keys and key_grid must be 16-byte aligned");
+    TREC_REQUIRE(rcap >= GROUP_ROWS && rcap % GROUP_ROWS == 0, "trec_topk_rows_collect_keys: rcap must be a multiple of 512");
+    hipStream_t st = (hipStream_t)stream;
+    const int64_t n_ublk = ceil_div64(n_users, KUSERS);
+    TREC_REQUIRE(n_ublk <= 65535, "trec_topk_rows_collect_keys: too many users");
+    const unsigned n_rgrp = (unsigned)((n_sb + CROWS * CGROUPS - 1) / (CROWS * CGROUPS));
+    hipLaunchKernelGGL(rows_collect_keys_kernel, dim3(n_rgrp, (unsigned)n_ublk), dim3(256), 0, st, (const uint16_t*)keys, n_sb, n_users,
+                       key_stride, thr, key_grid, wg_rows, rcap, row_count, row_user);
+    hipLaunchKernelGGL(rows_status_kernel, dim3(1), dim3(256), 0, st, row_count, n_sb, rcap, status);
+    return trec_check_launch("trec_topk_rows_collect_keys");
+}
+
+extern "C" int trec_cascade_keys_host(const float* ub, const float* tau, const float* r, int64_t n, uint16_t* key, int32_t* tkey,
+                                      float* grid)
+{
+    TREC_REQUIRE(ub && tau && r && key && tkey && grid && n >= 0, "trec_cascade_keys_host: bad arguments");
+    for (int64_t i = 0; i < n; ++i) {
+        float* g = grid + 4 * i;
+        i8_key_grid(r[i], &g[3], &g[0], &g[1], &g[2]);
+        key[i] = (uint16_t)i8_ub_key(ub[i], g[0], g[1]);
+        tkey[i] = (int32_t)i8_thr_key(tau[i], g[0], g[2]);
+    }
+    return TREC_OK;
 }
 
 extern "C" int trec_topk_rows_hot(int32_t* row_count, int32_t n_sb, int32_t rcap, int64_t n_users, int32_t* hot_list,
@@ -374,13 +529,13 @@
     return launch_blockmax_pipelined_grouped(p, kpad, (hipStream_t)stream);
 }
 
-extern "C" int trec_score_gemm_refine_candidates_marked(const void* users_bf16, const void* items_bf16, int32_t kpad, int64_t n_rows_g,
-                                                        int64_t n_items, const float* user_bias, const float* item_bias,
-                                                        int32_t sb_rows, const int32_t* row_count, const int32_t* row_user,
-                                                        float* blockmax, int64_t bm_stride, int32_t wgs_per_row,
-                                                        const float* cand_floor, int32_t* cand_n, void* cand, int32_t cand_cap,
-                                                        int32_t item_index_base, const int32_t* wg_map, int32_t n_wgs, float* pre_max,
-                                                        void* stream)
+extern "C" int trec_score_gemm_refine_candidates_marked_keys(const void* users_bf16, const void* items_bf16, int32_t kpad, int64_t n_rows_g,
+                                                             int64_t n_items, const float* user_bias, const float* item_bias,
+                                                             int32_t sb_rows, const int32_t* row_count, const int32_t* row_user,
+                                                             float* blockmax, int64_t bm_stride, int32_t wgs_per_row,
+                                                             const float* cand_floor, int32_t* cand_n, void* cand, int32_t cand_cap,
+                                                             int32_t item_index_base, const int32_t* wg_map, int32_t n_wgs, float* pre_max,
+                                                             void* keys, int64_t key_stride, void* stream)
 {
     TREC_REQUIRE(users_bf16 && items_bf16 && row_count && row_user && blockmax && cand_floor && cand_n && cand && pre_max,
                  "trec_score_gemm_refine_candidates_marked: null pointer");
@@ -402,7 +557,21 @@
     p.cand_diag = trec_get_tuning("cascade_cand_diag", 0);
     p.wg_map = wg_map; p.n_wgs = n_wgs;
     p.pre_max = pre_max;
+    p.keys = (uint16_t*)keys; p.key_stride = key_stride;
     return launch_blockmax_pipelined_grouped(p, kpad, (hipStream_t)stream);
+}
+
+extern "C" int trec_score_gemm_refine_candidates_marked(const void* users_bf16, const void* items_bf16, int32_t kpad, int64_t n_rows_g,
+                                                        int64_t n_items, const float* user_bias, const float* item_bias,
+                                                        int32_t sb_rows, const int32_t* row_count, const int32_t* row_user,
+                                                        float* blockmax, int64_t bm_stride, int32_t wgs_per_row,
+                                                        const float* cand_floor, int32_t* cand_n, void* cand, int32_t cand_cap,
+                                                        int32_t item_index_base, const int32_t* wg_map, int32_t n_wgs, float* pre_max,
+                                                        void* stream)
+{
+    return trec_score_gemm_refine_candidates_marked_keys(users_bf16, items_bf16, kpad, n_rows_g, n_items, user_bias, item_bias, sb_rows,
+                                                         row_count, row_user, blockmax, bm_stride, wgs_per_row, cand_floor, cand_n, cand,
+                                                         cand_cap, item_index_base, wg_map, n_wgs, pre_max, nullptr, 0, stream);
 }
 
 extern "C" int trec_score_gemm_refine_candidates_hot(const void* users_bf16, const void* items_bf16, int32_t kpad, int64_t n_users,
@@ -439,6 +608,22 @@
     return trec_check_launch("trec_topk_dense_users");
 }
 
+extern "C" int trec_topk_dense_users_keys(const void* keys, int32_t n_sb, int64_t n_users, int64_t key_stride, const float* thr,
+                                          const float* key_grid, int32_t wg_rows, int32_t limit, float* cand_floor, int32_t* flag,
+                                          int32_t* n_flagged, void* stream)
+{
+    TREC_REQUIRE(keys && thr && key_grid && cand_floor && flag && n_flagged, "trec_topk_dense_users_keys: null pointer");
+    TREC_REQUIRE(n_sb >= 32 && key_stride >= n_users && key_stride % 8 == 0 && limit >= 1 && limit <= 32,
+                 "trec_topk_dense_users_keys: need n_sb >= 32, key_stride % 8 == 0, 1 <= limit <= 32");
+    TREC_REQUIRE(wg_rows >= 8 && wg_rows % 8 == 0 && n_users < ((int64_t)1 << 31), "trec_topk_dense_users_keys: wg_rows must be a multiple of 8");
+    TREC_REQUIRE(((uintptr_t)keys % 16) == 0 && ((uintptr_t)key_grid % 16) == 0,
+                 "trec_topk_dense_users_keys: keys and key_grid must be 16-byte aligned");
+    if (n_users == 0) return TREC_OK;
+    hipLaunchKernelGGL(dense_users_keys_kernel, dim3((unsigned)ceil_div64(n_users, KUSERS)), dim3(256), 0, (hipStream_t)stream,
+                       (const uint16_t*)keys, n_sb, n_users, key_stride, thr, key_grid, wg_rows, limit, cand_floor, flag, n_flagged);
+    return trec_check_launch("trec_topk_dense_users_keys");
+}
+
 namespace {
 __global__ __launch_bounds__(256) void wg_start_kernel(const int32_t* __restrict__ row_count, int32_t n_sb, int32_t wgs_per_row,
                                                       int32_t* __restrict__ wg_start, int32_t group_rows)
diff --git a/tensorrec_amd/ops_topk.py b/tensorrec_amd/ops_topk.py
--- a/tensorrec_amd/ops_topk.py
+++ b/tensorrec_amd/ops_topk.py
@@ -479,10 +479,16 @@
     user_err = torch.empty((n_u, 4), dtype=torch.float32, device=dev)
     N.call("trec_score_user_err_i8", N.ptr(uop.stats8), N.ptr(user_bias), N.ptr(gstats8), kpad, n_u, N.ptr(iop.scales),
            N.ptr(uop.wg_scale), int(uop.wg_rows or 0) if uop.wg_scale is not None else 0, N.ptr(user_err))
-    stride = (n_u + 3) // 4 * 4
+    stride = (n_u + 7) // 8 * 8
     chunk_len, n_ch = blockmax_i8_chunks(n_i, n_chunks, sb_rows)
     table = torch.empty((n_sb, stride), dtype=torch.float32, device=dev)
     chunk_top = torch.empty((n_ch * top_k, stride), dtype=torch.float32, device=dev)
+    stride16 = stride
+    keys = torch.empty((n_sb, stride16), dtype=torch.int16, device=dev)
+    key_rows = int(N.query("trec_score_blockmax_i8_rows_per_workgroup", top_k))
+    key_grid = torch.empty(((n_u + key_rows - 1) // key_rows, 4), dtype=torch.float32, device=dev)
+    N.call("trec_score_key_grid", N.ptr(user_err), N.ptr(user_bias), N.ptr(gstats8), N.ptr(iop.sb_stats), n_sb, kpad, n_u, key_rows,
+           N.ptr(key_grid))
     lib = N.load()
     lists = cascade_lists_candidates() and gstats_all is not None and sb_rows <= 65536
     sb_per_chunk = chunk_len // sb_rows
@@ -493,10 +499,10 @@
         pre = (lib.trec_get_tuning(b"wide_prerefine", 1) != 0
                and n_sb >= 4 * kk)
     with _timed("score_gemm_blockmax_i8"):
-        N.call("trec_score_gemm_blockmax_i8", N.ptr(uop.i8), N.ptr(iop.i8), kpad, n_u, n_i, N.ptr(user_bias),
+        N.call("trec_score_gemm_blockmax_i8_keys", N.ptr(uop.i8), N.ptr(iop.i8), kpad, n_u, n_i, N.ptr(user_bias),
                N.ptr(iop.bias_q), N.ptr(iop.scales), N.ptr(iop.sb_stats), sb_rows, n_chunks, N.ptr(table), stride,
                N.ptr(user_err), N.ptr(chunk_top), top_k | (0x100 if pre else 0), N.ptr(uop.wg_scale), N.ptr(uop.wg_class),
-               int(uop.wg_rows or 0) if uop.wg_scale is not None else 0)
+               int(uop.wg_rows or 0) if uop.wg_scale is not None else 0, N.ptr(keys), stride16, N.ptr(key_grid))
     sel = torch.empty((n_u, kk), dtype=torch.int32, device=dev)
     sel_max = torch.empty((kk, n_u), dtype=torch.float32, device=dev) if (floor_exchange is not None or pre) else None
     tau = torch.empty((n_u,), dtype=torch.float32, device=dev)
@@ -540,8 +546,8 @@
         pre_rows = torch.empty((n_sb * rcap_a,), dtype=torch.int32, device=dev)
         pre_vals = torch.empty((n_u, kk), dtype=torch.float32, device=dev)
         if n_sb >= 32 and lib.trec_get_tuning(b"prerefine_early_dense", 1 if kk <= 16 else 0) != 0:
-            N.call("trec_topk_dense_users", N.ptr(table), n_sb, n_u, stride, N.ptr(tau), N.ptr(user_err), N.ptr(iop.sb_stats),
-                   kpad, CASCADE_DENSE_USER_LIMIT if n_i >= CASCADE_MIN_ITEMS else 30, N.ptr(cands.floor0), N.ptr(cands.flag),
+            N.call("trec_topk_dense_users_keys", N.ptr(keys), n_sb, n_u, stride16, N.ptr(tau), N.ptr(key_grid), key_rows,
+                   CASCADE_DENSE_USER_LIMIT if n_i >= CASCADE_MIN_ITEMS else 30, N.ptr(cands.floor0), N.ptr(cands.flag),
                    N.ptr(cands.n_flagged))
         sel_pos = torch.empty((n_u, kk), dtype=torch.int32, device=dev)
         pre_max = torch.empty((n_sb * rcap_a,), dtype=torch.float32, device=dev)
@@ -553,19 +559,22 @@
         wg_map_a = torch.full((n_wgs_a,), n_sb * (rcap_a // 512), dtype=torch.int32, device=dev)
         N.call("trec_topk_rows_wg_map", N.ptr(pre_ws), n_sb, rcap_a // 512, N.ptr(wg_start_a), N.ptr(wg_map_a), n_wgs_a)
         with _timed("score_gemm_blockmax_pre"):
-            N.call("trec_score_gemm_refine_candidates_marked", N.ptr(uop.bf16), N.ptr(iop.bf16), kpad, n_sb * rcap_a, n_i,
+            N.call("trec_score_gemm_refine_candidates_marked_keys", N.ptr(uop.bf16), N.ptr(iop.bf16), kpad, n_sb * rcap_a, n_i,
                    N.ptr(user_bias), N.ptr(item_bias), sb_rows, N.ptr(pre_ws), N.ptr(pre_rows), N.ptr(table), stride,
                    rcap_a // 512, N.ptr(cands.floor0), N.ptr(cands.n), N.ptr(cands.items), cands.cap, int(item_index_base),
-                   N.ptr(wg_map_a), n_wgs_a, N.ptr(pre_max))
+                   N.ptr(wg_map_a), n_wgs_a, N.ptr(pre_max), N.ptr(keys), stride16)
         with _timed("topk_prerefine"):
             N.call("trec_topk_prerefine_tau_listed", N.ptr(sel_sb), N.ptr(sel_pos), N.ptr(pre_ok), kk, N.ptr(pre_max), rcap_a, n_u,
                    N.ptr(uop.src), N.ptr(uop.stats), N.ptr(user_bias), N.ptr(gstats_all), kpad, N.ptr(tau), N.ptr(pre_vals),
                    N.ptr(cands.floor0))
         cands.pre = (sel_sb, pre_vals)
         if FILTER_DEBUG is not None:
+            real_cols = (uop.src >= 0) if uop.src is not None else torch.ones((n_u,), dtype=torch.bool, device=dev)
             FILTER_DEBUG.update({"prerefine_users_ok": int(pre_ok.sum().item()), "prerefine_rcap": rcap_a,
                                  "prerefine_row_count_max": int(pre_ws[:n_sb].max().item()), "prerefine_listed": 1,
-                                 "prerefine_pairs": int((sel_sb >= 0).sum().item())})
+                                 "prerefine_pairs": int((sel_sb >= 0).sum().item()),
+                                 "prerefine_marks": int(torch.isneginf(table[:, :n_u])[:, real_cols].sum().item()),
+                                 "prerefine_key_marks_differ": int((torch.isneginf(table[:, :n_u]) != (keys[:, :n_u] == 0))[:, real_cols].sum().item())})
     if cands is None and uop.src is not None:
         tau.masked_fill_(uop.src < 0, float("inf"))
     n_cap = int(uop.n_real or n_u)
@@ -573,8 +582,8 @@
     rcap = (int(rcap_frac * n_cap) + 511) // 512 * 512 + 512
     row_user = torch.empty((n_sb * rcap,), dtype=torch.int32, device=dev)
     with _timed("topk_rows_compact"):
-        N.call("trec_topk_rows_collect", N.ptr(table), n_sb, n_u, stride, N.ptr(tau), N.ptr(user_err),
-               N.ptr(iop.sb_stats), kpad, rcap, N.ptr(row_count), N.ptr(row_user), N.ptr(status))
+        N.call("trec_topk_rows_collect_keys", N.ptr(keys), n_sb, n_u, stride16, N.ptr(tau), N.ptr(key_grid), key_rows, rcap,
+               N.ptr(row_count), N.ptr(row_user), N.ptr(status))
     if FILTER_DEBUG is not None:
         FILTER_DEBUG.update({"int8_pairs_wanted": int(row_count.sum().item()), "int8_pairs_total": int(n_sb) * int(n_u),
                              "rcap": rcap, "row_count_max": int(row_count.max().item()),
@@ -585,8 +594,8 @@
     N.call("trec_topk_rows_hot", N.ptr(row_count), n_sb, rcap, n_u, N.ptr(hot_list), hot_cap, max_pairs, N.ptr(status))
     if cands is not None:
         if n_sb >= 32:
-            N.call("trec_topk_dense_users", N.ptr(table), n_sb, n_u, stride, N.ptr(tau), N.ptr(user_err), N.ptr(iop.sb_stats),
-                   kpad, CASCADE_DENSE_USER_LIMIT if n_i >= CASCADE_MIN_ITEMS else 30, N.ptr(cands.floor0), N.ptr(cands.flag),
+            N.call("trec_topk_dense_users_keys", N.ptr(keys), n_sb, n_u, stride16, N.ptr(tau), N.ptr(key_grid), key_rows,
+                   CASCADE_DENSE_USER_LIMIT if n_i >= CASCADE_MIN_ITEMS else 30, N.ptr(cands.floor0), N.ptr(cands.flag),
                    N.ptr(cands.n_flagged))
         wg_cap = min(n_sb * (rcap // 512), max_pairs // 512 + n_sb + 1)
         wg_start = torch.empty((n_sb + 1,), dtype=torch.int32, device=dev)
```

Result: no change. 11630 billion predictions/s (median of 6 runs) (+0.3%).
